# PaullyMac/routest

Measured on AMD Instinct MI355X. Metric: ETA preds/sec (whole node) + p50 /predict latency, 3-layer MLP bf16, higher is better.
Workload: dtype bf16

## Files before the change

csrc/bindings.cpp:

```cpp
#include <torch/extension.h>
#include <ATen/hip/impl/HIPStreamMasqueradingAsCUDA.h>
#include <c10/core/DeviceGuard.h>
#include <hip/hip_runtime.h>

#include <sys/mman.h>

#include <cstring>
#include <mutex>
#include <vector>

#include "ops.h"
#include "common.h"
#include "native_model.h"
#include "route_service.h"

namespace {

#define RT_CHECK_HIP(expr)                                                             \
  do {                                                                                 \
    hipError_t _e = (expr);                                                            \
    TORCH_CHECK(_e == hipSuccess, "HIP error in ", #expr, ": ", hipGetErrorString(_e)); \
  } while (0)

int num_cus(int dev) {
// ... 1342 lines not shown
    c.h_indices = (const int*)tptr("h_indices", false);
    c.h_length = (const float*)tptr("h_length", false);
    c.h_edge_name = (const int32_t*)tptr("h_edge_name", false);
    if (has("names")) c.names = d["names"].cast<std::vector<std::string>>();
    c.N = d["N"].cast<int>();
    c.snap_c = d["snap_c"].cast<double>();
    c.max_path = d["max_path"].cast<int>();
    TORCH_CHECK(c.glat && c.glon && c.h_indptr && c.h_indices && c.h_length && c.N == c.cch->topo().N &&
                    c.max_path > 0,
                "CCH route config incomplete");
  } else if (c.provider == 1) {
    c.glat = (const double*)tptr("glat", false);
    c.glon = (const double*)tptr("glon", false);
    c.h_indptr = (const int*)tptr("h_indptr", false);
    c.h_indices = (const int*)tptr("h_indices", false);
    c.h_cost = (const float*)tptr("h_cost", false);
    c.indptr = (const int*)tptr("indptr", true);
    c.indices = (const int*)tptr("indices", true);
    c.cost = (const float*)tptr("cost", true);
    c.lat32 = (const float*)tptr("lat32", true);
    c.lon32 = (const float*)tptr("lon32", true);
    c.lm = (const float*)tptr("lm", true);
    const torch::Device dev(torch::kCUDA, device);
    ws_from(d.contains("lane_ws") ? py::object(d["lane_ws"]) : py::object(py::none()), c.lane_ws, dev);
    ws_from(d.contains("wave_ws") ? py::object(d["wave_ws"]) : py::object(py::none()), c.wave_ws, dev);
    ws_from(d.contains("big_ws") ? py::object(d["big_ws"]) : py::object(py::none()), c.big_ws, dev);
    if (has("arena")) {
      torch::Tensor ar = d["arena"].cast<torch::Tensor>(), ctr = d["arena_ctr"].cast<torch::Tensor>();
      TORCH_CHECK(ar.is_cuda() && ar.device().index() == device && ar.scalar_type() == torch::kInt64 &&
                      ctr.is_cuda() && ctr.scalar_type() == torch::kInt64, "route config arena");
      c.arena.base = ar.data_ptr();
      c.arena.entries = (unsigned long long)(ar.numel() / 2);
      c.arena.ctr = (unsigned long long*)ctr.data_ptr();
    }
    c.N = d["N"].cast<int>();
    c.K = has("K") ? d["K"].cast<int>() : 0;
    c.snap_c = d["snap_c"].cast<double>();
    c.max_path = d["max_path"].cast<int>();
    c.max_iters = d["max_iters"].cast<int>();
    c.lane_pops = d["lane_pops"].cast<int>();
    if (has("wave_only_below")) c.wave_only_below = d["wave_only_below"].cast<int>();
    c.inv_vmax = d["inv_vmax"].cast<float>();
    c.wave_delta = d["wave_delta"].cast<float>();
    if (has("lane_max_m")) c.lane_max_m = d["lane_max_m"].cast<float>();
    TORCH_CHECK(c.glat && c.glon && c.indptr && c.indices && c.cost && c.lat32 && c.lon32 &&
                    (c.lane_ws.slots > 0 || c.wave_ws.slots > 0) && c.N > 0 && c.max_path > 0,
                "graph route config incomplete");
    TORCH_CHECK(c.lm == nullptr || c.K == 8 || c.K == 16 || c.K == 32, "landmarks K must be 8, 16 or 32");
    TORCH_CHECK((c.lane_ws.slots == 0 || rt::astar_ws_ok(c.lane_ws, false)) &&
                    (c.wave_ws.slots == 0 || rt::astar_ws_ok(c.wave_ws, true)) &&
                    (c.big_ws.slots == 0 || rt::astar_ws_ok(c.big_ws, true)),
                "A* workspace too small");
  }
  return c;
}

static std::vector<float> host_f32(const py::dict& h, const char* k) {
  torch::Tensor t = h[k].cast<torch::Tensor>().to(torch::kCPU).to(torch::kFloat32).contiguous();
  return std::vector<float>(t.data_ptr<float>(), t.data_ptr<float>() + t.numel());
}
static rt::MlpHost mlp_host_from(const py::dict& d) {
  rt::MlpHost m;
  if (!d.contains("host") || d["host"].is_none()) return m;
  py::dict h = d["host"].cast<py::dict>();
  m.w1 = host_f32(h, "w1");
  m.b1 = host_f32(h, "b1");
  m.w2 = host_f32(h, "w2");
  m.b2 = host_f32(h, "b2");
  m.w3 = host_f32(h, "w3");
  m.b3 = h["b3"].cast<float>();
  m.x_mean = host_f32(h, "x_mean");
  m.x_std = host_f32(h, "x_std");
  m.y_mean = h["y_mean"].cast<float>();
  m.y_std = h["y_std"].cast<float>();
  m.H = (int)m.b1.size();
  TORCH_CHECK(m.w1.size() == (size_t)m.H * 12 && m.w2.size() == (size_t)m.H * m.H && m.b2.size() == (size_t)m.H &&
                  m.w3.size() == (size_t)m.H && m.x_mean.size() == 12 && m.x_std.size() == 12,
              "model host weights shapes");
  return m;
}
static rt::NormParams norm_from(const py::dict& d) {
  std::vector<double> norm = d["norm"].cast<std::vector<double>>();
  TORCH_CHECK(norm.size() == 8, "norm must hold 4 scales + 4 shifts");
  rt::NormParams np;
  for (int i = 0; i < 4; ++i) {
    np.scale[i] = (float)norm[i];
    np.shift[i] = (float)norm[4 + i];
  }
  return np;
}
static std::shared_ptr<const rt::NativeModel> model_from(const py::dict& d, int device) {
  const std::string kind = d["kind"].cast<std::string>();
  if (kind == "none") return nullptr;
  std::string err;
  std::shared_ptr<rt::NativeModel> m;
  auto dev_t = [&](const char* k) {
    torch::Tensor t = d[k].cast<torch::Tensor>();
    TORCH_CHECK(t.is_cuda() && t.device().index() == device && t.is_contiguous(), "model tensor ", k,
                " must be contiguous on GPU ", device);
    return t;
  };
  if (kind == "mlp3") {
    const c10::DeviceGuard guard(c10::Device(c10::DeviceType::CUDA, device));
    torch::Tensor blob = dev_t("blob");
    const int H = d["H"].cast<int>();
    TORCH_CHECK(blob.scalar_type() == torch::kUInt8 && (size_t)blob.numel() == rt::eta_mlp3_blob_bytes(H), "mlp3 blob");
    m = rt::make_mlp3_model(device, blob.data_ptr(), (size_t)blob.numel(), H, norm_from(d),
                            d.contains("variant") ? d["variant"].cast<int>() : -1, num_cus(device), mlp_host_from(d),
                            err);
  } else if (kind == "wide") {
    const c10::DeviceGuard guard(c10::Device(c10::DeviceType::CUDA, device));
    torch::Tensor w1q = dev_t("w1q"), w2f = dev_t("w2f"), b2 = dev_t("b2"), w3 = dev_t("w3");
    const int H = d["H"].cast<int>();
    TORCH_CHECK(b2.scalar_type() == torch::kFloat32 && w3.scalar_type() == torch::kFloat32 && b2.numel() == H &&
                    w3.numel() == H, "wide b2/w3 f32 [H]");
    m = rt::make_wide_model(device, H, w1q.data_ptr(), (size_t)w1q.nbytes(), w2f.data_ptr(), (size_t)w2f.nbytes(),
                            b2.data_ptr<float>(), w3.data_ptr<float>(), d["b3"].cast<float>(), norm_from(d),
                            mlp_host_from(d), err);
  } else if (kind == "forest") {
    rt::ForestHost f;
    torch::Tensor v = d["values"].cast<torch::Tensor>().to(torch::kCPU).contiguous();
    torch::Tensor in = d["info"].cast<torch::Tensor>().to(torch::kCPU).contiguous();
    torch::Tensor r = d["roots"].cast<torch::Tensor>().to(torch::kCPU).contiguous();
    TORCH_CHECK(v.scalar_type() == torch::kFloat32 && in.scalar_type() == torch::kInt32 &&
                    r.scalar_type() == torch::kInt32, "forest arrays f32 / int32 / int32");
    f.values.assign(v.data_ptr<float>(), v.data_ptr<float>() + v.numel());
    f.info.assign((const uint32_t*)in.data_ptr<int>(), (const uint32_t*)in.data_ptr<int>() + in.numel());
    f.roots.assign(r.data_ptr<int>(), r.data_ptr<int>() + r.numel());
    f.base = d["base"].cast<float>();
    f.le = d["le"].cast<bool>();
    std::vector<int> fm = d["fmap"].cast<std::vector<int>>();
    TORCH_CHECK(fm.size() == 12, "fmap: 12 entries");
    for (int j = 0; j < 12; ++j) f.fmap[j] = fm[j];
    m = rt::make_forest_model(device, std::move(f), err);
  } else {
    TORCH_CHECK(false, "unknown native model kind ", kind);
  }
  TORCH_CHECK(m != nullptr, "native model: ", err);
  return m;
}

int64_t native_server_start(int64_t port, int64_t threads, std::vector<int64_t> devices, py::list models,
                            int64_t max_batch, std::vector<std::string> cors, bool cors_vercel, bool bind_any,
                            int64_t upstream_port, py::list routes, std::string history_db) {
  TORCH_CHECK(!devices.empty() && models.size() == devices.size(), "one model spec per GPU slot");
  TORCH_CHECK(max_batch >= 1 && max_batch <= (1 << 24), "max_batch out of range");
  TORCH_CHECK(routes.empty() || routes.size() == devices.size(), "one route config per GPU (or none)");
  std::vector<int> devs;
  std::vector<std::shared_ptr<const rt::NativeModel>> ms;
  for (size_t g = 0; g < devices.size(); ++g) {
    devs.push_back((int)devices[g]);
    ms.push_back(model_from(models[g].cast<py::dict>(), (int)devices[g]));
  }
  std::vector<rt::RouteServiceCfg> rcfg;
  for (size_t g = 0; g < routes.size(); ++g) rcfg.push_back(route_cfg_from(routes[g].cast<py::dict>(), devs[g]));
  std::string err;
  const int64_t h = rt::native_server_start((int)port, (int)threads, devs, ms, (int)max_batch, cors, cors_vercel,
                                            bind_any, (int)upstream_port, rcfg, history_db, err);
  TORCH_CHECK(h >= 0, "native server: ", err);
  return h;
}

int64_t native_server_set_models(int64_t h, std::vector<int64_t> devices, py::list models) {
  TORCH_CHECK(models.size() == devices.size(), "one model spec per GPU slot");
  std::vector<std::shared_ptr<const rt::NativeModel>> ms;
  for (size_t g = 0; g < devices.size(); ++g) ms.push_back(model_from(models[g].cast<py::dict>(), (int)devices[g]));
  std::string err;
  int64_t ep;
  {
    py::gil_scoped_release nogil;
    ep = rt::native_server_set_models(h, ms, err);
  }
  TORCH_CHECK(ep >= 0, "native server: ", err);
  return ep;
}

py::dict native_server_health(int64_t h) {
  uint64_t epoch = 0;
  auto rows = rt::native_server_health(h, epoch);
  py::list slots;
  for (auto& r : rows) {
    py::dict d;
    d["device"] = std::stoi(r[0]);
    d["quarantined"] = r[1] == "1";
    d["consecutive_failures"] = std::stoll(r[2]);
    d["failures"] = std::stoll(r[3]);
    d["rounds"] = std::stoll(r[4]);
    d["quarantines"] = std::stoll(r[5]);
    d["fault_injected"] = r[6] == "1";
    d["model"] = r[7];
    d["deadline_timeouts"] = std::stoll(r[8]);
    d["hang_injected"] = r[9] == "1";
    slots.append(d);
  }
  py::dict out;
  out["model_epoch"] = epoch;
  out["slots"] = slots;
  return out;
}

py::bytes comm_unique_id() {
  char id[128];
  TORCH_CHECK(rt::comm_unique_id(id) == 0, "ncclGetUniqueId failed");
  return py::bytes(id, 128);
}

int64_t comm_create(py::bytes uid, int64_t rank, int64_t world, int64_t device, int64_t oneshot_bytes,
                    bool use_rccl) {
  std::string u = uid;
  TORCH_CHECK(!use_rccl || u.size() == 128, "unique id must be 128 bytes");
  u.resize(128);
  std::string err;
  int64_t h;
  {
    py::gil_scoped_release nogil;
    h = rt::comm_create(u.data(), (int)rank, (int)world, (int)device, (size_t)oneshot_bytes, use_rccl, err);
  }
  TORCH_CHECK(h >= 0, "comm_create: ", err);
  return h;
}

py::bytes comm_ipc_handles(int64_t h) {
  std::string out(rt::comm_ipc_handle_bytes(), '\0');
  const int r = rt::comm_ipc_handles(h, out.data());
  TORCH_CHECK(r == 0, "hipIpcGetMemHandle failed (", r, ")");
  return py::bytes(out);
}

void comm_open_peers(int64_t h, std::vector<py::bytes> handles) {
  std::vector<std::string> hs(handles.begin(), handles.end());
  std::string err;
  TORCH_CHECK(rt::comm_open_peers(h, hs, err) == 0, "comm_open_peers: ", err);
}

void comm_all_reduce(int64_t h, torch::Tensor t, int64_t algo) {
  check_dev(t, "all_reduce tensor");
  TORCH_CHECK(t.scalar_type() == torch::kFloat32, "all_reduce: float32 buckets only");
  const c10::DeviceGuard guard(t.device());
  std::string err;
  const hipError_t e = rt::comm_all_reduce_f32(h, t.data_ptr<float>(), (size_t)t.numel(), (int)algo, cur_stream(t), err);
  TORCH_CHECK(e == hipSuccess, "comm_all_reduce: ", err.empty() ? hipGetErrorString(e) : err);
}

void comm_oneshot(int64_t h, int64_t op, torch::Tensor in, torch::Tensor out, int64_t root) {
  check_dev(in, "input");
  check_dev(out, "output");
  TORCH_CHECK(in.is_contiguous() && out.is_contiguous(), "one-shot: contiguous tensors only");
  TORCH_CHECK(in.scalar_type() == out.scalar_type(), "dtype mismatch");
  const c10::DeviceGuard guard(in.device());
  std::string err;
  const size_t bytes = (size_t)in.numel() * in.element_size();
  const int world = rt::comm_world(h);
  TORCH_CHECK(world >= 1, "bad comm handle");
  hipError_t e;
  if (op == 0) {
    TORCH_CHECK(out.numel() == in.numel() * world, "all_gather: out must hold world x input");
    e = rt::comm_all_gather_oneshot(h, in.data_ptr(), out.data_ptr(), bytes, cur_stream(in), err);
  } else {
    TORCH_CHECK(in.data_ptr() == out.data_ptr(), "one-shot broadcast is in place");
    e = rt::comm_broadcast_oneshot(h, in.data_ptr(), bytes, (int)root, cur_stream(in), err);
  }
  TORCH_CHECK(e == hipSuccess, "comm_oneshot: ", err.empty() ? hipGetErrorString(e) : err);
}

int dtype_code(const torch::Tensor& t) {
  if (t.scalar_type() == torch::kFloat32) return 0;
  if (t.scalar_type() == torch::kBFloat16) return 1;
  if (t.scalar_type() == torch::kInt32) return 2;
  TORCH_CHECK(false, "collective dtype must be float32, bfloat16 or int32");
  return -1;
}

void comm_collective(int64_t h, int64_t op, torch::Tensor in, torch::Tensor out, int64_t root) {
  check_dev(in, "input");
  check_dev(out, "output");
  TORCH_CHECK(in.scalar_type() == out.scalar_type(), "dtype mismatch");
  const c10::DeviceGuard guard(in.device());
  std::string err;
  const size_t count = op == 0 ? (size_t)in.numel() : (op == 1 ? (size_t)out.numel() : (size_t)in.numel());
  TORCH_CHECK(rt::comm_nccl_call(h, (int)op, in.data_ptr(), out.data_ptr(), count, dtype_code(in), (int)root,
                                 cur_stream(in), err) == 0, "RCCL collective: ", err);
}

torch::Tensor forest_predict_lds(torch::Tensor records, torch::Tensor nodes2, torch::Tensor roots,
                                 torch::Tensor chunks, double base, bool le, std::vector<int64_t> fmap) {
  for (auto* t : {&records, &nodes2, &roots, &chunks}) check_dev(*t, "forest tensor");
  TORCH_CHECK(records.scalar_type() == torch::kInt32 && records.dim() == 2 && records.size(1) == 4,
              "records must be int32 [B,4]");
  TORCH_CHECK(nodes2.scalar_type() == torch::kInt32 && nodes2.dim() == 2 && nodes2.size(1) == 2, "nodes2 int32 [M,2]");
  TORCH_CHECK(chunks.scalar_type() == torch::kInt32 && chunks.dim() == 2 && chunks.size(1) == 2 &&
              chunks.size(0) >= 2, "chunks int32 [C+1,2]");
  TORCH_CHECK(roots.scalar_type() == torch::kInt32, "roots int32");
  TORCH_CHECK(fmap.size() == 12, "fmap must have 12 entries");
  const c10::DeviceGuard guard(records.device());
  const int B = (int)records.size(0);
  auto out = torch::empty({B}, records.options().dtype(torch::kFloat32));
  int fm[12];
  for (int j = 0; j < 12; ++j) fm[j] = (int)fmap[j];
  RT_CHECK_HIP(rt::launch_forest_lds(records.data_ptr(), nodes2.data_ptr(), roots.data_ptr<int>(),
                                     chunks.data_ptr<int>(), (int)chunks.size(0) - 1, out.data_ptr<float>(), B,
                                     (int)roots.numel(), (int)nodes2.size(0), (float)base, le ? 1 : 0, fm,
                                     num_cus(records.device().index()), cur_stream(records)));
  return out;
}

}

void bind_cch_gpu(py::module& m);

PYBIND11_MODULE(TORCH_EXTENSION_NAME, m) {
  m.doc() = "routest_amd native gfx950 kernels";
  bind_cch_gpu(m);
  m.def("eta_mlp3_forward", &eta_mlp3_forward, "fused featurize + 3-layer MLP forward (bf16 MFMA)");
  m.def("eta_mlp3_forward_hostio", &eta_mlp3_forward_hostio,
        "zero-copy: fused kernel reads records / writes minutes in pinned host memory");
  m.def("pinned_host_empty", &pinned_host_empty, "registered pinned host buffer (optionally THP-backed)",
        py::arg("nbytes"), py::arg("huge") = true);
  m.def("eta_featurize", &eta_featurize,"K1: packed records -> R16 features [B,12] fp32");
  m.def("eta_mlp3_blob_bytes", [](int64_t H) { return (int64_t)rt::eta_mlp3_blob_bytes((int)H); });
  m.def("eta_mlp3_blob16_bytes", [](int64_t H) { return (int64_t)rt::eta_mlp3_blob16_bytes((int)H); });
  m.def("route_haversine_matrix", &route_haversine_matrix, "K5: batched haversine matrices (f64)");
  m.def("route_greedy_cvrp", &route_greedy_cvrp, "K6: batched greedy multi-trip CVRP");
  m.def("route_improve_trips", &route_improve_trips,
        "K6b: intra-trip 2-opt / Or-opt on K6's outputs (visit rewritten in place)");
  m.def("route_tw_trips", &route_tw_trips,
        "K6d: cheapest-insertion trips under time windows and service times for the flagged rows",
        py::arg("D"), py::arg("T"), py::arg("npts"), py::arg("demand"), py::arg("cap"), py::arg("maxd"),
        py::arg("open"), py::arg("close"), py::arg("service"), py::arg("flag"));
  m.def("route_pd_trips", &route_pd_trips,
        "K6f: cheapest insertion of plain stops and pickup -> delivery pairs under time windows for the flagged rows",
        py::arg("D"), py::arg("T"), py::arg("npts"), py::arg("demand"), py::arg("cap"), py::arg("maxd"),
        py::arg("open"), py::arg("close"), py::arg("service"), py::arg("pickup_from"), py::arg("flag"));
  m.def("route_tw_improve", &route_tw_improve,
        "K6e: window-aware relocate / swap on K6d's outputs (rewritten in place); returns stats [R,7]",
        py::arg("D"), py::arg("T"), py::arg("npts"), py::arg("demand"), py::arg("cap"), py::arg("maxd"),
        py::arg("open"), py::arg("close"), py::arg("service"), py::arg("visit"), py::arg("trip_of"),
        py::arg("ntrips"), py::arg("status"), py::arg("arrival"), py::arg("start"), py::arg("flag"));
  m.def("route_pd_improve", &route_pd_improve,
        "K6g: unit relocate on K6f's outputs (rewritten in place); returns stats [R,8]",
        py::arg("D"), py::arg("T"), py::arg("npts"), py::arg("demand"), py::arg("cap"), py::arg("maxd"),
        py::arg("open"), py::arg("close"), py::arg("service"), py::arg("pickup_from"), py::arg("visit"),
        py::arg("trip_of"), py::arg("ntrips"), py::arg("status"), py::arg("arrival"), py::arg("start"),
        py::arg("flag"));
  m.def("route_exchange_trips", &route_exchange_trips,
        "K6c: inter-trip relocate / swap on K6's outputs (visit, trip_of, ntrips rewritten in place)",
        py::arg("D"), py::arg("npts"), py::arg("demand"), py::arg("cap"), py::arg("maxd"), py::arg("visit"),
        py::arg("trip_of"), py::arg("ntrips"), py::arg("status"), py::arg("flag"), py::arg("move_cap") = -1);
  m.def("mm_candidates", &mm_candidates, "K10: map-matching candidates of GPS fixes on the bucket grid",
        py::arg("start"), py::arg("items"), py::arg("nqy"), py::arg("nqx"), py::arg("y0"), py::arg("x0"),
        py::arg("cell"), py::arg("ny"), py::arg("nx"), py::arg("py"), py::arg("px"), py::arg("radius_cm"),
        py::arg("k"));
  m.def("mm_viterbi", &mm_viterbi, "K10: segmenting Viterbi of the map matcher over given costs",
        py::arg("cand_d2"), py::arg("n_cand"), py::arg("route_cm"), py::arg("g"), py::arg("npts"),
        py::arg("beta_cm"), py::arg("sigma_cm"), py::arg("max_detour_cm"));
  m.def("mm_edge_candidates", &mm_edge_candidates, "K10 edge mode: candidates of GPS fixes on the edge grid",
        py::arg("start"), py::arg("items"), py::arg("rec"), py::arg("y0"), py::arg("x0"), py::arg("cell"),
        py::arg("ny"), py::arg("nx"), py::arg("py"), py::arg("px"), py::arg("radius_cm"), py::arg("k"));
  m.def("mm_edge_route_cm", &mm_edge_route_cm, "K10 edge mode: route centimetres between points on edges",
        py::arg("met"), py::arg("e1"), py::arg("off1"), py::arg("lc1"), py::arg("e2"), py::arg("off2"));
  m.def("mm_edge_lds_capacity", []() { return (int64_t)rt::mm_edge_lds_capacity(); },
        "K10 edge mode: survivors of one fix the candidate kernel selects from LDS");
  m.def("big_layer1", &big_layer1, "wide MLP: featurize + layer 1 -> h1 (hperm order)",
        py::arg("records"), py::arg("w1p"), py::arg("H"), py::arg("norm"), py::arg("h1"),
        py::arg("xf") = py::none(), py::arg("mbits") = py::none());
  m.def("big_fused", &big_fused, "wide MLP inference: featurize + layer 1 + layer 2 + relu.w3 partials, one launch");
  m.def("gemm_dgrad_dw1", &gemm_dgrad_dw1, "training dgrad with the dW1 partials in its epilogue (dh1 not stored)");
  m.def("gemm_nt", &gemm_nt, "wide MLP layer GEMM Z^T = W X^T with fused epilogues (0 y-partials, 1 +h2, 2 store)",
        py::arg("epi"), py::arg("W"), py::arg("X"), py::arg("N"), py::arg("M"), py::arg("K"),
        py::arg("b2") = py::none(), py::arg("w3") = py::none(), py::arg("ypart") = py::none(),
        py::arg("out") = py::none());
  m.def("gemm_pipe", [](int64_t set) { return (int64_t)rt::gemm_pipe_mode((int)set); },
        "wide GEMM K loop: 1 phase pipeline, 0 one drain per K-tile; set < 0 only reads", py::arg("set") = -1);
  m.def("big_yreduce", &big_yreduce, "y = sum of partials + b3 (+ dy, dy operand, squared error)",
        py::arg("ypart"), py::arg("nparts"), py::arg("b3"), py::arg("y") = py::none(),
        py::arg("target") = py::none(), py::arg("gscale") = 0.0, py::arg("dy") = py::none(),
        py::arg("dyb") = py::none(), py::arg("sq_err") = py::none(), py::arg("b3_dev") = py::none());
  m.def("adamw_pack_big", &adamw_pack_big, "wide trainer: AdamW + re-pack of w1p / w2k / w2t / b2 / w3 / b3");
  m.def("big_dz2y", &big_dz2y,
        "wide trainer: dy, dyb, squared error, dz2 and the step counter in one launch (+ dW3|db3 slab rows)",
        py::arg("ypart"), py::arg("nparts"), py::arg("b3"), py::arg("target"), py::arg("gscale"), py::arg("dy"),
        py::arg("dyb"), py::arg("sq_err"), py::arg("h2a"), py::arg("w3"), py::arg("H"), py::arg("dz2"),
        py::arg("step_ctr"), py::arg("slab") = py::none());
  m.def("big_dz2", &big_dz2, "dz2 = dy * w3 * relu'(z2) from h2a (hperm order)");
  m.def("eta_mlp3_train_fwd", &eta_mlp3_train_fwd, "K3: fused featurize+MLP forward (one pass over layer 2) + MSE grad + dW3 partial -> dz2 fragments");
  m.def("train_bwd", &train_bwd, "K3: dgrad + relu'(z1) + dW2|db2 and dW1 split-K partials in one kernel (train_bwd_kernel)");
  m.def("train_wgrad_slices", [](int64_t B, int64_t device, int64_t H) {
    return (int64_t)rt::train_wgrad_slices((int)B, num_cus((int)device), (int)H);
  }, py::arg("B"), py::arg("device"), py::arg("H") = 256);
  m.def("adamw_pack", &adamw_pack, "fused AdamW on flat fp32 params + training-blob re-pack");
  m.def("reduce_adamw", &reduce_adamw, "one-rank fused slab reduction + AdamW + blob re-pack");
  m.def("eta_mlp3_train_blob_bytes", [](int64_t H) { return (int64_t)rt::eta_mlp3_train_blob_bytes((int)H); });
  m.def("mlp3_num_params", [](int64_t H) { return (int64_t)rt::mlp3_num_params((int)H); });
  m.def("mlp3_grad_bucket_floats", [](int64_t H) { return (int64_t)rt::mlp3_grad_bucket_floats((int)H); });
  m.def("wgrad", &wgrad, "split-K weight-gradient GEMM (K = batch) into fp32 slabs",
        py::arg("A"), py::arg("M"), py::arg("Mout"), py::arg("Bm"), py::arg("N"), py::arg("slab"),
        py::arg("offset"), py::arg("ldo"), py::arg("mask") = py::none(), py::arg("nout") = -1, py::arg("mask_hperm") = false,
        py::arg("nsplit") = 1);
  m.def("wgrad_dual", &wgrad_dual, "two split-K weight-gradient GEMMs (dW2|db2 and dW1) in one launch");
  m.def("wgrad_reduce", &wgrad_reduce, "deterministic sum of wgrad slabs (optionally a second and third region)",
        py::arg("slab"), py::arg("G"), py::arg("slab1") = py::none(), py::arg("G1") = py::none(),
        py::arg("slab2") = py::none(), py::arg("G2") = py::none(), py::arg("perm_h") = 0, py::arg("fold_ld") = 0,
        py::arg("fold_col") = 0);
  m.def("wgrad256", &wgrad256, "dW2-shaped weight gradient on 256x256 output tiles, split-K over the slab's rows",
        py::arg("A"), py::arg("B"), py::arg("M"), py::arg("N"), py::arg("slab"), py::arg("ldo"), py::arg("db2_col") = -1);
  m.def("train_fwd_grid", [](int64_t B, int64_t dev) { return (int64_t)rt::train_fwd_grid((int)B, num_cus((int)dev)); },
        "workgroups of the training forward = rows of its dW3 slab");
  m.def("num_cus", [](int64_t dev) { return (int64_t)num_cus((int)dev); });
  m.def("gcn_agg_gemm", &gcn_agg_gemm, "K8: fused CSR aggregation + MFMA GEMM + bias/ReLU");
  m.def("gcn_l1_fused", &gcn_l1_fused, "K8: fused aggregation + W1 GEMM + ReLU + W2 transform (H1 stays in LDS)");
  m.def("gcn_spmm_score", &gcn_spmm_score, "K8: layer-2 aggregation + delay head");
  m.def("route_score", &route_score, "K8: per-route delay-weighted length");
  m.def("astar_search", &astar_search, "K9: tiered batched A* (lane -> wave -> big tier) with learned edge costs",
        py::arg("indptr"), py::arg("indices"), py::arg("cost"), py::arg("lat"), py::arg("lon"), py::arg("inv_vmax"),
        py::arg("landmarks"), py::arg("src"), py::arg("dst"), py::arg("lane"), py::arg("wave"), py::arg("big"),
        py::arg("out_cost"), py::arg("out_len"), py::arg("out_status"), py::arg("out_path"), py::arg("out_iters"),
        py::arg("scratch"), py::arg("max_iters"), py::arg("lane_pops"), py::arg("wave_only_below"),
        py::arg("delta"), py::arg("arena") = py::none(), py::arg("arena_ctr") = py::none(),
        py::arg("lane_max_m") = -1.0, py::arg("wave_nw") = 0, py::arg("retry_nw") = 0);
  m.def("forest_predict", &forest_predict, "K4: fused featurize + tree-ensemble inference");
  m.def("forest_predict_lds", &forest_predict_lds, "K4: LDS-staged tree chunks, 2 walks per thread");
  m.def("pscore_create", &pscore_create, "resident single-request scorer kernel on the blob's GPU");
  m.def("pscore_score", &pscore_score, "score n <= cap records on the resident scorer (False: not answered)");
  m.def("pscore_park", [](int64_t h) {
    rt::PersistentScorer* p = ps_get(h);
    py::gil_scoped_release nogil;
    rt::pscore_park(p);
  });
  m.def("pscore_stats", [](int64_t h) {
    long long l, s, f;
    rt::pscore_stats(ps_get(h), &l, &s, &f);
    return std::vector<int64_t>{l, s, f};
  });
  m.def("pscore_destroy", [](int64_t h) {
    rt::PersistentScorer* p = nullptr;
    {
      std::lock_guard<std::mutex> lk(g_ps_mu);
      if (h < 0 || h >= (int64_t)g_ps.size()) return;
      p = g_ps[h];
      g_ps[h] = nullptr;
    }
    py::gil_scoped_release nogil;
    rt::pscore_destroy(p);
  });
  m.def("gcn_train_bwd", &gcn_train_bwd, "GCN scorer backward over a row range -> flat gradient + loss");
  m.def("gcn_grad_numel", []() { return (int64_t)rt::gcn_grad_numel(); });
  m.def("gcn_train_slab2_rows", [](int64_t n) { return (int64_t)rt::gcn_train_slab2_rows((int)n); });
  m.def("native_server_start", &native_server_start, "native HTTP front end (predictions, routes, relay)",
        py::arg("port"), py::arg("threads"), py::arg("devices"), py::arg("models"), py::arg("max_batch"),
        py::arg("cors"), py::arg("cors_vercel"), py::arg("bind_any"), py::arg("upstream_port") = 0,
        py::arg("routes") = py::list(), py::arg("history_db") = "");
  m.def("native_server_set_models", &native_server_set_models,
        "hot-swap the served models (one spec per GPU slot); returns the new epoch");
  m.def("native_server_set_fault", [](int64_t h, int64_t slot, bool on) {
    return rt::native_server_set_fault(h, (int)slot, on);
  });
  m.def("native_server_set_hang", [](int64_t h, int64_t slot, bool on) {
    return rt::native_server_set_hang(h, (int)slot, on);
  }, "latency-watchdog fault hook: launches on the slot first wait on a host flag");
  m.def("native_server_set_scorer", [](int64_t h, std::vector<double> delay, int64_t kind, std::string engine) {
    return rt::native_server_set_scorer(h, std::move(delay), (int)kind, engine);
  }, "publish the GCN scorer's node delays for native \"alternatives\" requests");
  m.def("native_server_health", &native_server_health, "per-GPU-slot health, models and the model epoch");
  m.def("native_server_stop", [](int64_t h) {
    py::gil_scoped_release nogil;
    rt::native_server_stop(h);
  });
  m.def("native_server_stats", [](int64_t h) {
    const auto v = rt::native_server_stats(h);
    return std::vector<int64_t>(v.begin(), v.end());
  });
  m.def("comm_unique_id", &comm_unique_id, "RCCL unique id (128 bytes) for comm_create");
  m.def("comm_create", &comm_create, "own RCCL communicator + one-shot IPC buffers");
  m.def("comm_ipc_handles", &comm_ipc_handles, "IPC handles of this rank's one-shot buffers");
  m.def("comm_open_peers", &comm_open_peers, "map every peer's one-shot buffers (xGMI)");
  m.def("comm_all_reduce", &comm_all_reduce, "in-place SUM all-reduce on the current stream (0=rccl, 1=oneshot)");
  m.def("comm_collective", &comm_collective, "RCCL all_gather(0)/reduce_scatter(1)/broadcast(2)/all_reduce(3)");
  m.def("comm_oneshot", &comm_oneshot, "one-shot IPC all_gather(0)/broadcast(2) on the current stream");
  m.def("comm_error", [](int64_t h) { return (int64_t)rt::comm_error(h); });
  m.def("comm_destroy", [](int64_t h) { rt::comm_destroy(h); });
  m.def("rccl_version", []() { return (int64_t)rt::comm_rccl_version(); });
  m.attr("ARCH") = "gfx950";
}
```

csrc/native_model.h:

```cpp
#pragma once
#include <hip/hip_runtime.h>

#include <cstdint>
#include <memory>
#include <string>
#include <vector>

#include "common.h"
#include "runtime/rt_core.h"

namespace rt {

struct ModelWs {
  void* p = nullptr;
  size_t bytes = 0;
  int device = -1;
  ~ModelWs();
  hipError_t need(int dev, size_t b);
};

struct NativeModel {
  enum Kind { MLP3 = 0, WIDE = 1, FOREST = 2 };
  int kind = MLP3;
  int device = 0;
  int H = 0;
  uint64_t epoch = 0;
  virtual ~NativeModel() = default;
  virtual hipError_t predict(const void* rec, int rec_bytes, float* out, int B, hipStream_t s, ModelWs& ws) const = 0;
  virtual bool takes_wire8() const { return true; }
  virtual const void* mlp3_blob() const { return nullptr; }
  virtual const NormParams* mlp3_norm() const { return nullptr; }
  virtual bool cpu_predict(const rtc::EtaRecord* rec, float* out, int B) const = 0;
  virtual std::string describe() const = 0;
};

struct MlpHost {
  int H = 0;
  std::vector<float> w1, b1, w2, b2, w3, x_mean, x_std;
  float b3 = 0.f, y_mean = 0.f, y_std = 1.f;
};

struct ForestHost {
  std::vector<float> values;
  std::vector<uint32_t> info;
  std::vector<int32_t> roots;
  float base = 0.f;
  bool le = false;
  int fmap[12] = {0, 1, 2, 3, 4, 5, 6, 7, 8, 9, 10, 11};
};

std::shared_ptr<NativeModel> make_mlp3_model(int device, const void* blob, size_t blob_bytes, int H,
                                             const NormParams& np, int variant, int num_cus, MlpHost host,
                                             std::string& err);
std::shared_ptr<NativeModel> make_wide_model(int device, int H, const void* w1q, size_t w1q_bytes, const void* w2f,
                                             size_t w2f_bytes, const float* b2, const float* w3, float b3,
                                             const NormParams& np, MlpHost host, std::string& err);
std::shared_ptr<NativeModel> make_forest_model(int device, ForestHost host, std::string& err);

float mlp_cpu_forward(const MlpHost& m, const rtc::EtaRecord& r);

}
```

csrc/native_model.hip:

```cpp
#include <cmath>
#include <cstring>

#include "native_model.h"
#include "ops.h"

namespace rt {

ModelWs::~ModelWs() {
  if (p) {
    int cur = 0;
    (void)hipGetDevice(&cur);
    (void)hipSetDevice(device);
    (void)hipFree(p);
    (void)hipSetDevice(cur);
  }
}

hipError_t ModelWs::need(int dev, size_t b) {
  if (p && device == dev && bytes >= b) return hipSuccess;
  if (p) {
    int cur = 0;
    (void)hipGetDevice(&cur);
    (void)hipSetDevice(device);
    (void)hipFree(p);
    (void)hipSetDevice(cur);
    p = nullptr;
  }
  bytes = 0;
  device = dev;
  const size_t m = b < 4096 ? 4096 : b;
  hipError_t e = hipMalloc(&p, m);
  if (e == hipSuccess) bytes = m;
  return e;
}

namespace {

struct DevOwned {
  void* p = nullptr;
  int device = 0;
  DevOwned() = default;
  DevOwned(const DevOwned&) = delete;
  ~DevOwned() {
    if (p) {
      int cur = 0;
      (void)hipGetDevice(&cur);
      (void)hipSetDevice(device);
      (void)hipFree(p);
      (void)hipSetDevice(cur);
    }
  }
  hipError_t copy_from(int dev, const void* src, size_t bytes, hipMemcpyKind kind) {
    device = dev;
    int cur = 0;
    (void)hipGetDevice(&cur);
    (void)hipSetDevice(dev);
    hipError_t e = hipMalloc(&p, bytes ? bytes : 4);
    if (e == hipSuccess && bytes) e = hipMemcpy(p, src, bytes, kind);
    (void)hipSetDevice(cur);
    return e;
  }
};

inline void featurize(const rtc::EtaRecord& r, float x[12]) {
  for (int i = 0; i < 8; ++i) x[i] = 0.f;
  if (r.weather < 4) x[r.weather] = 1.f;
  if (r.traffic < 4) x[4 + r.traffic] = 1.f;
  const int64_t secs = r.wallclock_s;
  const int64_t days = secs >= 0 ? secs / 86400 : -((-secs + 86399) / 86400);
  const int64_t sod = secs - days * 86400;
  x[8] = (float)(((days + 2) % 7 + 7) % 7);
  x[9] = (float)(sod / 3600);
  x[10] = r.distance_m / 1000.0f;
  x[11] = r.driver_age;
}

bool mlp_cpu_batch(const MlpHost& m, const rtc::EtaRecord* rec, float* out, int B) {
  if (m.H <= 0) return false;
  for (int i = 0; i < B; ++i) out[i] = mlp_cpu_forward(m, rec[i]);
  return true;
}

struct Mlp3Model : NativeModel {
  DevOwned blob;
  NormParams np{};
  int variant = -1, cus = 256;
  MlpHost host;
  hipError_t predict(const void* rec, int rec_bytes, float* out, int B, hipStream_t s, ModelWs&) const override {
    return launch_eta_mlp3_fwd(rec, out, B, blob.p, H, np, variant, cus, s, rec_bytes);
  }
  const void* mlp3_blob() const override { return blob.p; }
  const NormParams* mlp3_norm() const override { return &np; }
  bool cpu_predict(const rtc::EtaRecord* rec, float* out, int B) const override { return mlp_cpu_batch(host, rec, out, B); }
  std::string describe() const override { return "mlp3 H=" + std::to_string(H); }
};

struct WideModel : NativeModel {
  DevOwned w1q, w2f, b2, w3;
  float b3 = 0.f;
  NormParams np{};
  MlpHost host;
  hipError_t predict(const void* rec, int rec_bytes, float* out, int B, hipStream_t s, ModelWs& ws) const override {
    const int parts = H / 64;
    hipError_t e = ws.need(device, (size_t)B * parts * sizeof(float));
    if (e != hipSuccess) return e;
    float* yp = (float*)ws.p;
    e = launch_big_fused(rec, rec_bytes, B, w1q.p, w2f.p, H, np, (const float*)b2.p, (const float*)w3.p, yp, s);
    if (e != hipSuccess) return e;
    return launch_big_yreduce(yp, parts, B, b3, nullptr, out, nullptr, 0.f, nullptr, nullptr, nullptr, s);
  }
  bool cpu_predict(const rtc::EtaRecord* rec, float* out, int B) const override { return mlp_cpu_batch(host, rec, out, B); }
  std::string describe() const override { return "mlp3-wide H=" + std::to_string(H); }
};

struct ForestModelN : NativeModel {
  DevOwned values, info, roots;
  ForestHost host;
  int fm[12];
  hipError_t predict(const void* rec, int rec_bytes, float* out, int B, hipStream_t s, ModelWs&) const override {
    if (rec_bytes != 16) return hipErrorInvalidValue;
    return launch_forest(rec, (const float*)values.p, (const unsigned*)info.p, (const int*)roots.p, out, B,
                         (int)host.roots.size(), (int)host.values.size(), host.base, host.le ? 1 : 0, fm, s);
  }
  bool takes_wire8() const override { return false; }
  bool cpu_predict(const rtc::EtaRecord* rec, float* out, int B) const override {
    const int T = (int)host.roots.size();
    for (int i = 0; i < B; ++i) {
      float x[12], xm[12];
      featurize(rec[i], x);
      for (int j = 0; j < 12; ++j) xm[j] = x[host.fmap[j]];
      double acc = host.base;
      for (int t = 0; t < T; ++t) {
        const int root = host.roots[t];
        int n = root;
        while (!(host.info[n] >> 31)) {
          const uint32_t inf = host.info[n];
          const float v = xm[(inf >> 24) & 63];
          const float thr = host.values[n];
          const bool left = std::isnan(v) ? ((inf >> 30) & 1) != 0 : (host.le ? v <= thr : v < thr);
          n = root + (int)(inf & 0xFFFFFF) + (left ? 0 : 1);
        }
        acc += host.values[n];
      }
      out[i] = (float)acc;
    }
    return true;
  }
  std::string describe() const override { return "forest trees=" + std::to_string(host.roots.size()); }
};

}

float mlp_cpu_forward(const MlpHost& m, const rtc::EtaRecord& r) {
  float x[12];
  featurize(r, x);
  for (int j = 0; j < 12; ++j) x[j] = (x[j] - m.x_mean[j]) / m.x_std[j];
  const int H = m.H;
  std::vector<float> h1(H), h2(H);
  for (int u = 0; u < H; ++u) {
    float a = m.b1[u];
    const float* w = m.w1.data() + (size_t)u * 12;
    for (int j = 0; j < 12; ++j) a += w[j] * x[j];
    h1[u] = a > 0.f ? a : 0.f;
  }
  for (int u = 0; u < H; ++u) {
    float a = m.b2[u];
    const float* w = m.w2.data() + (size_t)u * H;
    for (int j = 0; j < H; ++j) a += w[j] * h1[j];
    h2[u] = a > 0.f ? a : 0.f;
  }
  float y = m.b3;
  for (int j = 0; j < H; ++j) y += m.w3[j] * h2[j];
  return y * m.y_std + m.y_mean;
}

std::shared_ptr<NativeModel> make_mlp3_model(int device, const void* blob, size_t blob_bytes, int H,
                                             const NormParams& np, int variant, int num_cus, MlpHost host,
                                             std::string& err) {
  auto m = std::make_shared<Mlp3Model>();
  m->kind = NativeModel::MLP3;
  m->device = device;
  m->H = H;
  m->np = np;
  m->variant = variant;
  m->cus = num_cus;
  m->host = std::move(host);
  if (m->blob.copy_from(device, blob, blob_bytes, hipMemcpyDeviceToDevice) != hipSuccess) {
    err = "mlp3 blob copy failed";
    return nullptr;
  }
  return m;
}

std::shared_ptr<NativeModel> make_wide_model(int device, int H, const void* w1q, size_t w1q_bytes, const void* w2f,
                                             size_t w2f_bytes, const float* b2, const float* w3, float b3,
                                             const NormParams& np, MlpHost host, std::string& err) {
  if (H != 512 && H != 1024) {
    err = "wide model: H must be 512 or 1024";
    return nullptr;
  }
  auto m = std::make_shared<WideModel>();
  m->kind = NativeModel::WIDE;
  m->device = device;
  m->H = H;
  m->np = np;
  m->b3 = b3;
  m->host = std::move(host);
  if (m->w1q.copy_from(device, w1q, w1q_bytes, hipMemcpyDeviceToDevice) != hipSuccess ||
      m->w2f.copy_from(device, w2f, w2f_bytes, hipMemcpyDeviceToDevice) != hipSuccess ||
      m->b2.copy_from(device, b2, (size_t)H * 4, hipMemcpyDeviceToDevice) != hipSuccess ||
      m->w3.copy_from(device, w3, (size_t)H * 4, hipMemcpyDeviceToDevice) != hipSuccess) {
    err = "wide model weight copy failed";
    return nullptr;
  }
  return m;
}

constexpr int FOREST_MAX_DEPTH = 64;

std::shared_ptr<NativeModel> make_forest_model(int device, ForestHost host, std::string& err) {
  const size_t M = host.values.size();
  if (M == 0 || host.info.size() != M || host.roots.empty() || host.roots[0] != 0) {
    err = "forest: malformed arrays";
    return nullptr;
  }
  for (size_t i = 1; i < host.roots.size(); ++i)
    if (host.roots[i] <= host.roots[i - 1] || (size_t)host.roots[i] >= M) {
      err = "forest: roots not increasing";
      return nullptr;
    }
  for (size_t t = 0; t < host.roots.size(); ++t) {
    const size_t b = (size_t)host.roots[t], e = t + 1 < host.roots.size() ? (size_t)host.roots[t + 1] : M;
    for (size_t n = b; n < e; ++n) {
      const uint32_t inf = host.info[n];
      if (inf >> 31) continue;
      if (((inf >> 24) & 63) >= 12 || b + (inf & 0xFFFFFF) + 1 >= e) {
        err = "forest: node reference out of range";
        return nullptr;
      }
    }
  }
  {
    std::vector<int> seen(M, -1);
    std::vector<uint32_t> cur, nxt;
    for (size_t t = 0; t < host.roots.size(); ++t) {
      const uint32_t b = (uint32_t)host.roots[t];
      cur.assign(1, b);
      for (int level = 0; !cur.empty(); ++level) {
        nxt.clear();
        for (uint32_t n : cur) {
          const uint32_t inf = host.info[n];
          if (inf >> 31) continue;
          if (level == FOREST_MAX_DEPTH) {
            err = "forest: tree " + std::to_string(t) + " is deeper than the kernels' depth limit of " +
                  std::to_string(FOREST_MAX_DEPTH) + " inner nodes on a root-to-leaf path";
            return nullptr;
          }
          for (uint32_t c = b + (inf & 0xFFFFFF), e = c + 2; c < e; ++c)
            if (seen[c] != level) {
              seen[c] = level;
              nxt.push_back(c);
            }
        }
        cur.swap(nxt);
      }
    }
  }
  for (int j = 0; j < 12; ++j)
    if (host.fmap[j] < 0 || host.fmap[j] >= 12) {
      err = "forest: feature map out of range";
      return nullptr;
    }
  auto m = std::make_shared<ForestModelN>();
  m->kind = NativeModel::FOREST;
  m->device = device;
  m->H = 0;
  for (int j = 0; j < 12; ++j) m->fm[j] = host.fmap[j];
  if (m->values.copy_from(device, host.values.data(), M * 4, hipMemcpyHostToDevice) != hipSuccess ||
      m->info.copy_from(device, host.info.data(), M * 4, hipMemcpyHostToDevice) != hipSuccess ||
      m->roots.copy_from(device, host.roots.data(), host.roots.size() * 4, hipMemcpyHostToDevice) != hipSuccess) {
    err = "forest copy failed";
    return nullptr;
  }
  m->host = std::move(host);
  return m;
}

}
```

csrc/native_server.hip:

```cpp
#include <arpa/inet.h>
#include <errno.h>
#include <fcntl.h>
#include <netinet/in.h>
#include <netinet/tcp.h>
#include <sys/epoll.h>
#include <sys/eventfd.h>
#include <sys/socket.h>
#include <sys/time.h>
#include <time.h>
#include <unistd.h>

#include <atomic>
#include <cstdlib>
#include <cstring>
#include <memory>
#include <mutex>
#include <shared_mutex>
#include <string>
#include <thread>
#include <unordered_map>
#include <vector>

#include "common.h"
#include "native_model.h"
// ... 1197 lines not shown
    }
    c.out.clear();
    c.out_off = 0;
    epoll_event e{};
    e.events = EPOLLIN;
    e.data.fd = c.fd;
    epoll_ctl(ep_, EPOLL_CTL_MOD, c.fd, &e);
    if (c.close_after && !c.async) to_close_.push_back(c.fd);
  }
};

struct Server {
  ServerCfg cfg;
  Stats stats;
  Shared sh;
  std::atomic<bool> stop{false};
  std::vector<std::unique_ptr<Reactor>> reactors;
  std::vector<std::thread> threads;
  std::vector<std::unique_ptr<RouteService>> routes;
  std::shared_mutex routes_mu;
  bool routes_open = false;
  std::shared_ptr<AltScorerState> alt = std::make_shared<AltScorerState>();
  ~Server() {
    if (sh.hang_release) *(volatile int*)sh.hang_release = 1;
    {
      std::unique_lock<std::shared_mutex> lk(routes_mu);
      routes_open = false;
    }
    routes.clear();
    for (PersistentScorer* p : sh.scorers)
      if (p) pscore_destroy(p);
    if (sh.hang_release) (void)hipHostFree(sh.hang_release);
  }
};

void stop_scorer(Server* s, int g) {
  Shared& sh = s->sh;
  if (sh.scorers[g] != nullptr) pscore_destroy(sh.scorers[g]);
  sh.scorers[g] = nullptr;
  sh.scorer_models[g] = nullptr;
}

void restart_scorer(Server* s, int g) {
  Shared& sh = s->sh;
  stop_scorer(s, g);
  if (!(s->cfg.persist_idle_ms > 0 && s->cfg.persist_cap > 0)) return;
  auto m = sh.model(g);
  if (m == nullptr || m->mlp3_blob() == nullptr) return;
  hipError_t e = hipSuccess;
  sh.scorers[g] = pscore_create(sh.devices[g], m->mlp3_blob(), m->H, *m->mlp3_norm(), s->cfg.persist_cap,
                                s->cfg.persist_idle_ms, s->cfg.persist_life_ms, &e);
  if (sh.scorers[g] != nullptr) sh.scorer_models[g] = m;
}

std::mutex g_srv_mu;
std::vector<Server*> g_servers;

}

int64_t native_server_start(int port, int threads, const std::vector<int>& devices,
                            const std::vector<std::shared_ptr<const NativeModel>>& models, int max_batch,
                            const std::vector<std::string>& cors, bool cors_vercel, bool bind_any, int upstream_port,
                            const std::vector<RouteServiceCfg>& routes, const std::string& history_db,
                            std::string& err) {
  if (devices.empty() || devices.size() != models.size() || (!routes.empty() && routes.size() != devices.size())) {
    err = "devices/models/routes mismatch";
    return -1;
  }
  auto* s = new Server();
  s->cfg.port = port;
  s->cfg.threads = threads < 1 ? 1 : threads;
  s->cfg.max_batch = max_batch;
  s->cfg.cors_exact = cors;
  s->cfg.cors_vercel = cors_vercel;
  s->cfg.upstream_port = upstream_port;
  s->cfg.sh = &s->sh;
  s->cfg.history_db = history_db;
  if (const char* v = std::getenv("ROUTEST_PERSIST_IDLE_MS")) s->cfg.persist_idle_ms = std::atof(v);
  if (const char* v = std::getenv("ROUTEST_PERSIST_CAP")) s->cfg.persist_cap = std::atoi(v);
  if (const char* v = std::getenv("ROUTEST_PERSIST_LIFE_MS")) s->cfg.persist_life_ms = std::atof(v);
  Shared& sh = s->sh;
  if (const char* v = std::getenv("ROUTEST_QUARANTINE_AFTER")) sh.quarantine_after = std::max(1, std::atoi(v));
  if (const char* v = std::getenv("ROUTEST_QUARANTINE_PROBE_MS")) sh.probe_ms = std::max(1ll, std::atoll(v));
  if (const char* v = std::getenv("ROUTEST_FRONT_CACHE_MS")) sh.rc_ttl_ms = std::max(0ll, std::atoll(v));
  sh.devices = devices;
  sh.models = models;
  sh.epoch = 1;
  for (size_t g = 0; g < devices.size(); ++g) {
    sh.health.push_back(std::make_unique<SlotHealth>());
    sh.scorers.push_back(nullptr);
    sh.scorer_models.push_back(nullptr);
    sh.scorer_mus.push_back(std::make_unique<std::mutex>());
  }
  if (const char* v = std::getenv("ROUTEST_GPU_DEADLINE_MS")) sh.deadline_ms = std::atof(v);
  if (const char* v = std::getenv("ROUTEST_ROUTE_TRACE_MS")) sh.trace_ms = std::atof(v);
  if (hipHostMalloc((void**)&sh.hang_release, sizeof(int), hipHostMallocMapped | hipHostMallocPortable) == hipSuccess) {
    *(volatile int*)sh.hang_release = 1;
    if (hipHostGetDevicePointer((void**)&sh.hang_release_d, sh.hang_release, 0) != hipSuccess) sh.hang_release_d = nullptr;
  } else {
    sh.hang_release = nullptr;
  }
  if (const char* v = std::getenv("ROUTEST_FAULT")) {
    std::string f = v;
    size_t b = 0;
    while (b <= f.size()) {
      size_t e = f.find(',', b);
      if (e == std::string::npos) e = f.size();
      std::string t = f.substr(b, e - b);
      while (!t.empty() && t.front() == ' ') t.erase(t.begin());
      while (!t.empty() && t.back() == ' ') t.pop_back();
      if (t == "gpu_fail") {
        for (auto& h : sh.health) h->fault = true;
      } else if (t.rfind("gpu_fail@", 0) == 0) {
        const int g = std::atoi(t.c_str() + 9);
        if (g >= 0 && g < (int)sh.health.size()) sh.health[g]->fault = true;
      } else if (t.rfind("gpu_hang@", 0) == 0 && sh.hang_release_d) {
        const int g = std::atoi(t.c_str() + 9);
        if (g >= 0 && g < (int)sh.health.size()) {
          sh.health[g]->hang = true;
          *(volatile int*)sh.hang_release = 0;
        }
      }
      b = e + 1;
    }
  }
  for (size_t g = 0; g < devices.size(); ++g) {
    std::lock_guard<std::mutex> lk(*sh.scorer_mus[g]);
    restart_scorer(s, (int)g);
  }
  if (!routes.empty() && routes[0].provider == 1 && routes[0].h_length != nullptr && routes[0].glat != nullptr) {
    auto rg = std::make_shared<rrec::RecordGraph>();
    const RouteServiceCfg& r0 = routes[0];
    rg->own_names = r0.names;
    rg->build(r0.N, r0.glat, r0.glon, r0.h_indptr, r0.h_indices, r0.h_length, r0.h_edge_name, &rg->own_names);
    if (rg->ok()) s->cfg.record_graph = rg;
  }
  for (int i = 0; i < s->cfg.threads; ++i) {
    ServerCfg rc = s->cfg;
    const size_t g = (size_t)i % devices.size();
    rc.device = devices[g];
    rc.slot = (int)g;
    auto r = std::make_unique<Reactor>(rc, s->stats, s->stop);
    r->set_bind_any(bind_any);
    if (!r->init(err)) {
      delete s;
      return -1;
    }
    s->reactors.push_back(std::move(r));
  }
  s->routes.reserve(routes.size());
  for (size_t g = 0; g < routes.size(); ++g) {
    RouteServiceCfg rc = routes[g];
    rc.record_graph = s->cfg.record_graph;
    Shared* shp = &s->sh;
    const int slot = (int)g;
    rc.eta_model = [shp, slot]() { return shp->model(slot); };
    rc.park_scorer = [shp, slot]() { shp->park(slot); };
    rc.alt = s->alt;
    rc.on_timeout = [shp, slot]() { shp->timed_out(slot); };
    rc.slot = slot;
    rc.failover = [s, slot](RouteJob* j) {
      std::shared_lock<std::shared_mutex> lk(s->routes_mu);
      if (!s->routes_open) return false;
      const int n = (int)s->routes.size();
      if (j->hops >= n - 1) return false;
      for (int k = 1; k < n; ++k) {
        RouteService* r = s->routes[(size_t)((slot + k) % n)].get();
        if (r != nullptr && !r->broken()) {
          ++j->hops;
          if (r->submit(j)) return true;
          --j->hops;
        }
      }
      return false;
    };
    rc.hang_fault = [shp, slot]() { return shp->health[slot]->hang.load(std::memory_order_relaxed); };
    rc.hang_release_d = shp->hang_release_d;
    s->routes.push_back(std::make_unique<RouteService>(rc, [](RouteJob* j) {
      static_cast<JobTag*>(j->tag)->reactor->job_done(j);
    }));
    s->routes.back()->set_done_batch([](std::vector<RouteJob*>& js) {
      std::vector<std::pair<Reactor*, std::vector<RouteJob*>>> by;
      for (RouteJob* j : js) {
        Reactor* r = static_cast<JobTag*>(j->tag)->reactor;
        auto it = std::find_if(by.begin(), by.end(), [r](const auto& p) { return p.first == r; });
        if (it == by.end()) by.push_back({r, {j}});
        else it->second.push_back(j);
      }
      for (auto& [r, v] : by) r->jobs_done(v);
    });
  }
  {
    std::unique_lock<std::shared_mutex> lk(s->routes_mu);
    s->routes_open = true;
  }
  if (!s->routes.empty())
    for (int i = 0; i < s->cfg.threads; ++i) s->reactors[i]->set_routes(s->routes[(size_t)i % devices.size()].get());
  for (auto& r : s->reactors) s->threads.emplace_back([rp = r.get()]() { rp->run(); });
  std::lock_guard<std::mutex> lk(g_srv_mu);
  g_servers.push_back(s);
  return (int64_t)g_servers.size() - 1;
}

int64_t native_server_set_models(int64_t h, const std::vector<std::shared_ptr<const NativeModel>>& models,
                                 std::string& err) {
  std::lock_guard<std::mutex> lk(g_srv_mu);
  if (h < 0 || h >= (int64_t)g_servers.size() || !g_servers[h]) {
    err = "no such server";
    return -1;
  }
  Server* s = g_servers[h];
  if (models.size() != s->sh.devices.size()) {
    err = "one model per GPU slot";
    return -1;
  }
  for (size_t g = 0; g < models.size(); ++g) {
    std::lock_guard<std::mutex> sl(*s->sh.scorer_mus[g]);
    stop_scorer(s, (int)g);
  }
  uint64_t ep;
  {
    std::lock_guard<std::mutex> ml(s->sh.model_mu);
    s->sh.models = models;
    ep = s->sh.epoch.fetch_add(1) + 1;
  }
  for (size_t g = 0; g < models.size(); ++g) {
    std::lock_guard<std::mutex> sl(*s->sh.scorer_mus[g]);
    restart_scorer(s, (int)g);
  }
  return (int64_t)ep;
}

bool native_server_set_fault(int64_t h, int slot, bool on) {
  std::lock_guard<std::mutex> lk(g_srv_mu);
  if (h < 0 || h >= (int64_t)g_servers.size() || !g_servers[h]) return false;
  Server* s = g_servers[h];
  if (slot < 0 || slot >= (int)s->sh.health.size()) return false;
  s->sh.health[slot]->fault = on;
  return true;
}

bool native_server_set_hang(int64_t h, int slot, bool on) {
  std::lock_guard<std::mutex> lk(g_srv_mu);
  if (h < 0 || h >= (int64_t)g_servers.size() || !g_servers[h]) return false;
  Server* s = g_servers[h];
  if (slot < 0 || slot >= (int)s->sh.health.size() || !s->sh.hang_release) return false;
  s->sh.health[slot]->hang = on;
  bool any = false;
  for (auto& x : s->sh.health) any |= x->hang.load();
  *(volatile int*)s->sh.hang_release = any ? 0 : 1;
  return true;
}

bool native_server_set_scorer(int64_t h, std::vector<double> delay, int kind, const std::string& engine) {
  std::lock_guard<std::mutex> lk(g_srv_mu);
  if (h < 0 || h >= (int64_t)g_servers.size() || !g_servers[h]) return false;
  Server* s = g_servers[h];
  std::lock_guard<std::mutex> lk2(s->alt->mu);
  s->alt->delay = delay.empty() ? nullptr : std::make_shared<const std::vector<double>>(std::move(delay));
  s->alt->kind = kind;
  s->alt->engine = engine;
  return true;
}

std::vector<std::vector<std::string>> native_server_health(int64_t h, uint64_t& epoch) {
  std::vector<std::vector<std::string>> out;
  std::lock_guard<std::mutex> lk(g_srv_mu);
  if (h < 0 || h >= (int64_t)g_servers.size() || !g_servers[h]) return out;
  Server* s = g_servers[h];
  epoch = s->sh.epoch.load();
  auto models = s->sh.snapshot();
  for (size_t g = 0; g < s->sh.devices.size(); ++g) {
    const SlotHealth& x = *s->sh.health[g];
    out.push_back({std::to_string(s->sh.devices[g]), x.quarantined.load() ? "1" : "0", std::to_string(x.consec.load()),
                   std::to_string(x.failures.load()), std::to_string(x.rounds.load()),
                   std::to_string(x.quarantines.load()), x.fault.load() ? "1" : "0",
                   models[g] ? models[g]->describe() : std::string("none"), std::to_string(x.timeouts.load()),
                   x.hang.load() ? "1" : "0"});
  }
  return out;
}

void native_server_stop(int64_t h) {
  Server* s = nullptr;
  {
    std::lock_guard<std::mutex> lk(g_srv_mu);
    if (h < 0 || h >= (int64_t)g_servers.size()) return;
    s = g_servers[h];
    g_servers[h] = nullptr;
  }
  if (!s) return;
  if (s->sh.hang_release) *(volatile int*)s->sh.hang_release = 1;
  s->stop.store(true);
  for (auto& r : s->reactors) {
    uint64_t one = 1;
    (void)!write(r->wake_fd(), &one, 8);
  }
  for (auto& t : s->threads) t.join();
  delete s;
}

std::vector<long long> native_server_stats(int64_t h) {
  std::lock_guard<std::mutex> lk(g_srv_mu);
  if (h < 0 || h >= (int64_t)g_servers.size() || !g_servers[h]) return std::vector<long long>(41, 0);
  Server* s = g_servers[h];
  std::vector<long long> v = {s->stats.requests.load(), s->stats.predictions.load(), s->stats.launches.load(),
                              s->stats.errors.load(), s->stats.resident.load(), s->stats.fallbacks.load(),
                              s->stats.wire8.load(), s->stats.route_requests.load(),
                              s->stats.route_fallbacks.load(), s->stats.relayed.load()};
  std::vector<long long> rs(18, 0);
  for (auto& r : s->routes) {
    const auto x = r->stats();
    for (size_t i = 0; i < rs.size() && i < x.size(); ++i) rs[i] += x[i];
  }
  v.insert(v.end(), rs.begin(), rs.end());
  v.push_back(s->stats.failovers.load());
  v.push_back(s->stats.cpu_rounds.load());
  v.push_back(s->stats.history.load());
  v.push_back(s->stats.cached.load());
  std::vector<long long> rx(4, 0);
  for (auto& r : s->routes) {
    const auto x = r->stats();
    for (size_t i = 0; i < rx.size() && 18 + i < x.size(); ++i) rx[i] += x[18 + i];
  }
  v.insert(v.end(), rx.begin(), rx.end());
  v.push_back(s->stats.timeouts.load());
  std::vector<long long> rr(4, 0);
  for (auto& r : s->routes) {
    const auto x = r->stats();
    for (size_t i = 0; i < rr.size() && 22 + i < x.size(); ++i) rr[i] += x[22 + i];
  }
  v.insert(v.end(), rr.begin(), rr.end());
  return v;
}

}
```

csrc/route_service.h:

```cpp
#pragma once
#include <cmath>
#include <functional>
#include <memory>
#include <string>
#include <vector>

#include "cch_gpu.h"
#include "common.h"
#include "native_model.h"
#include "ops.h"
#include "runtime/route_core.h"
#include "runtime/route_record.h"
#include "runtime/route_store.h"

#include <mutex>

namespace rt {

struct PersistentScorer;
struct RouteJob;

inline hipError_t isolated_stream(int device, hipStream_t* s) {
  int cus = 0;
  if (hipDeviceGetAttribute(&cus, hipDeviceAttributeMultiprocessorCount, device) != hipSuccess || cus <= 0) cus = 256;
  std::vector<uint32_t> mask((size_t)(cus + 31) / 32, 0xFFFFFFFFu);
  return hipExtStreamCreateWithCUMask(s, (uint32_t)mask.size(), mask.data());
}

struct AltScorerState {
  std::mutex mu;
  std::shared_ptr<const std::vector<double>> delay;
  int kind = 0;
  std::string engine = "gcn-hip";
  std::shared_ptr<const std::vector<double>> get(int& k, std::string& e) {
    std::lock_guard<std::mutex> lk(mu);
    k = kind;
    e = engine;
    return delay;
  }
};

struct RouteServiceCfg {
  int device = 0;
  int provider = 0;
  CchGpu* cch = nullptr;
  bool cch_contexts = true;
  uint64_t cch_fixed_key = 0;
  const float* h_length = nullptr;
  const int32_t* h_edge_name = nullptr;
  std::vector<std::string> names;
  double circuity = 1.3, step_m = 150.0;
  std::string engine = "backend:mi355x";
  bool compat200 = true;
  int batch_max = 1024;
  double timeout_us = 500.0;
  int chunk_threads = 16;
  const double* glat = nullptr;
  const double* glon = nullptr;
  int N = 0;
  double snap_c = 1.0;
  const int* h_indptr = nullptr;
  const int* h_indices = nullptr;
  const float* h_cost = nullptr;
  const int* indptr = nullptr;
  const int* indices = nullptr;
  const float* cost = nullptr;
  const float* lat32 = nullptr;
  const float* lon32 = nullptr;
  const float* lm = nullptr;
  int K = 0;
  AstarWs lane_ws, wave_ws, big_ws;
  AstarArenaBuf arena;
  int max_path = 4096, max_iters = 2000000, lane_pops = 500;
  int wave_only_below = 32768;
  float inv_vmax = 0.f, wave_delta = 10.f, lane_max_m = -1.f;
  std::function<std::shared_ptr<const NativeModel>()> eta_model;
  std::string sqlite_path;
  std::function<void()> park_scorer;
  std::shared_ptr<AltScorerState> alt;
  std::function<bool(RouteJob*)> failover;
  std::shared_ptr<const rrec::RecordGraph> record_graph;
  std::function<void()> on_timeout;
  int slot = -1;
  std::function<bool()> hang_fault;
  const int* hang_release_d = nullptr;
};

struct RouteJob {
  std::string body;
  bool json_ok = true;
  bool request_route = false;
  void* tag = nullptr;
  bool fallback = false;
  int status = 0;
  std::string out;
  rtj::Value root;
  rtr::RouteReq req;
  rtr::Plan plan;
  std::vector<std::vector<std::pair<double, double>>> calls;
  std::vector<int32_t> nodes;
  int group = 0;
  bool parsed = false;
  double defer_t0 = 0.0;
  bool sync_ctx = false;
  int hops = 0;
  double t_enq_us = 0.0;
  std::vector<std::pair<int, int>> alt_pairs;
  std::vector<std::vector<int>> alt_vias;
  std::vector<rtr::Leg> alt_legs;
  std::vector<std::vector<int32_t>> alt_paths, alt_edges;
  std::string alt_json;
  rts::StoreRow row;
  rtc::Stamp now;
};

class RouteService {
 public:
  RouteService(const RouteServiceCfg& cfg, std::function<void(RouteJob*)> done);
  ~RouteService();
  bool submit(RouteJob* j);
  void set_done_batch(std::function<void(std::vector<RouteJob*>&)> done_many);
  std::vector<long long> stats() const;
  bool broken() const;

 private:
  struct Impl;
  Impl* p_;
};

}
```

csrc/route_service.hip:

```cpp
#include <fcntl.h>
#include <unistd.h>

#include <algorithm>
#include <cstdlib>
#include <cstring>

#include "route_service_impl.h"

namespace rt {

namespace {

__global__ __launch_bounds__(64) void route_hang_kernel(const int* release, long long max_ticks) {
  const long long t0 = wall_clock64();
  for (int it = 0; it < 2000000 && __hip_atomic_load(release, __ATOMIC_RELAXED, __HIP_MEMORY_SCOPE_SYSTEM) == 0 &&
                   wall_clock64() - t0 < max_ticks;
       ++it)
    __builtin_amdgcn_s_sleep(127);
}

}

hipError_t RouteService::Impl::sync(hipStream_t s, hipEvent_t ev, const char* what) {
  hipError_t e = hipEventRecord(ev, s);
  if (e != hipSuccess) return e;
  const auto t0 = std::chrono::steady_clock::now();
  auto waited = [&] { return std::chrono::duration<double, std::milli>(std::chrono::steady_clock::now() - t0).count(); };
  for (int i = 0;; ++i) {
    e = hipEventQuery(ev);
    if (e != hipErrorNotReady) {
      if (trace_ms >= 0 && waited() > trace_ms) trace("wait %s %.1f ms", what, waited());
      return e;
    }
    const double dl = flush_deadline_ms.load(std::memory_order_relaxed);
    if (dl > 0 && (i & 15) == 15 && waited() > dl) {
      trace("DEADLINE in %s after %.1f ms", what, waited());
      if (!broken.exchange(true) && cfg.on_timeout) cfg.on_timeout();
      return hipErrorLaunchTimeOut;
    }
    if (i > 4096) std::this_thread::sleep_for(std::chrono::microseconds(20));
  }
}

void RouteService::Impl::hand_off(std::vector<RouteJob*>& jobs) {
  for (RouteJob* j : jobs) {
    if (!j->fallback && !j->status && cfg.failover) {
      j->plan = rtr::Plan();
      j->calls.clear();
      j->nodes.clear();
      j->group = 0;
      j->alt_pairs.clear();
      j->alt_vias.clear();
      j->alt_legs.clear();
      j->alt_paths.clear();
      j->alt_edges.clear();
      j->alt_json.clear();
      j->row.asmb = rtr::Assembled();
      if (cfg.failover(j)) {
        n_failed_over.fetch_add(1, std::memory_order_relaxed);
        continue;
      }
      trace("no other route service takes the job (hops %d): relayed to the app", j->hops);
    }
    if (!j->status) j->fallback = true;
    finish(j);
    done(j);
  }
  jobs.clear();
}

void RouteService::Impl::run() {
  if (hipSetDevice(cfg.device) != hipSuccess) return;
  int least = 0, greatest = 0;
  if (hipDeviceGetStreamPriorityRange(&least, &greatest) != hipSuccess ||
      hipStreamCreateWithPriority(&stream, hipStreamNonBlocking, greatest) != hipSuccess) {
    (void)hipGetLastError();
    if (hipStreamCreateWithFlags(&stream, hipStreamNonBlocking) != hipSuccess) return;
  }
  if (const char* v = std::getenv("ROUTEST_CCH_ASYNC")) async_ctx = std::string(v) != "0";
  if (const char* v = std::getenv("ROUTEST_ROUTE_DEADLINE_MS")) deadline_ms = std::atof(v);
  flush_deadline_ms.store(deadline_ms);
  if (const char* v = std::getenv("ROUTEST_ROUTE_TRACE_MS")) trace_ms = std::atof(v);
  if (const char* v = std::getenv("ROUTEST_FAULT")) fail_fault = std::string(v).find("route_fail") != std::string::npos;
  if (hipEventCreateWithFlags(&ev_gpu, hipEventDisableTiming) != hipSuccess) ev_gpu = nullptr;
  if (const char* v = std::getenv("ROUTEST_CCH_PREFETCH_MIN")) prefetch_min = std::atoi(v);
  if (const char* v = std::getenv("ROUTEST_ROUTE_CLOCK_SKEW_S")) clock_skew_s = std::atoll(v);
  if (cfg.cch != nullptr && cfg.cch_contexts && async_ctx) {
    listener = cfg.cch->add_build_listener([this](uint64_t key, bool ok) { on_built(key, ok); });
    cfg.cch->start_builders();
  }
  if (std::getenv("ROUTEST_ROUTE_PREWARM") == nullptr || std::string(std::getenv("ROUTEST_ROUTE_PREWARM")) != "0")
    prewarm();
  if (const char* v = std::getenv("ROUTEST_HANG_ARM"))
    if (std::string(v) == "1" && isolated_stream(cfg.device, &hang_stream) != hipSuccess) hang_stream = nullptr;
  th_asm = std::thread([this] { asm_loop(); });
  while (true) {
    auto* b = new Batch();
    {
      std::unique_lock<std::mutex> lk(mu);
      cv.wait(lk, [&] { return stop || !q.empty(); });
      if (stop && q.empty()) { delete b; break; }
      const double t_wake = now_us();
      static const bool from_wake = [] {
        const char* v = std::getenv("ROUTEST_ROUTE_COLLECT");
        return v && std::string(v) == "wake";
      }();
      const double t_open = from_wake ? t_wake : q.front()->t_enq_us;
      const auto deadline = std::chrono::steady_clock::time_point(std::chrono::duration_cast<std::chrono::steady_clock::duration>(
          std::chrono::duration<double, std::micro>(t_open + cfg.timeout_us)));
      while ((int)q.size() < cfg.batch_max && !stop && std::chrono::steady_clock::now() < deadline) {
        if (cv.wait_until(lk, deadline) == std::cv_status::timeout) break;
      }
      t_collect_us.fetch_add((long long)(now_us() - t_wake), std::memory_order_relaxed);
      const size_t take = std::min<size_t>(q.size(), (size_t)cfg.batch_max);
      b->jobs.assign(q.begin(), q.begin() + take);
      q.erase(q.begin(), q.begin() + take);
    }
    if (broken.load()) {
      if (drained()) {
        trace("drained: serving again");
        broken.store(false);
      } else {
        trace("broken: handing %zu jobs off", b->jobs.size());
        hand_off(b->jobs);
        delete b;
        continue;
      }
    }
    hipStream_t main_stream = stream;
    if (cfg.hang_fault && cfg.hang_release_d && cfg.hang_fault()) {
      if (!hang_stream && isolated_stream(cfg.device, &hang_stream) != hipSuccess) hang_stream = nullptr;
      if (hang_stream) {
        stream = hang_stream;
        hipLaunchKernelGGL(route_hang_kernel, dim3(1), dim3(64), 0, stream, cfg.hang_release_d, 500000000ll);
      }
    }
    gpu_stage(*b);
    stream = main_stream;
    if (fail_fault && !b->jobs.empty()) b->failed = true;
    if (b->failed) {
      trace("flush of %zu jobs failed: handing off", b->jobs.size());
      hand_off(b->jobs);
      delete b;
      continue;
    }
    if (b->jobs.empty()) {
      delete b;
      continue;
    }
    const double t_h = now_us();
    std::unique_lock<std::mutex> lk(amu);
    acv.wait(lk, [&] { return aq.size() < 2; });
    t_handoff_us.fetch_add((long long)(now_us() - t_h), std::memory_order_relaxed);
    aq.push_back(b);
    acv.notify_all();
  }
  if (listener) cfg.cch->remove_build_listener(listener);
  std::vector<RouteJob*> left;
  {
    std::lock_guard<std::mutex> lk(wmu);
    for (auto& kv : waiting) left.insert(left.end(), kv.second.begin(), kv.second.end());
    waiting.clear();
  }
  {
    std::lock_guard<std::mutex> lk(mu);
    left.insert(left.end(), q.begin(), q.end());
    q.clear();
  }
  for (RouteJob* j : left) {
    j->fallback = true;
    finish(j);
    done(j);
  }
  {
    std::lock_guard<std::mutex> lk(amu);
    gpu_done = true;
  }
  acv.notify_all();
  th_asm.join();
  (void)hipStreamDestroy(stream);
  if (ev_gpu) (void)hipEventDestroy(ev_gpu);
}

void RouteService::Impl::asm_loop() {
  if (hipSetDevice(cfg.device) != hipSuccess) return;
  if (hipStreamCreateWithFlags(&stream_asm, hipStreamNonBlocking) != hipSuccess) return;
  if (hipEventCreateWithFlags(&ev_asm, hipEventDisableTiming) != hipSuccess) ev_asm = nullptr;
  store.open(cfg.sqlite_path);
  th_persist = std::thread([this] { persist_loop(); });
  while (true) {
    Batch* b = nullptr;
    {
      std::unique_lock<std::mutex> lk(amu);
      acv.wait(lk, [&] { return gpu_done || !aq.empty(); });
      if (aq.empty()) break;
      b = aq.front();
      aq.pop_front();
      acv.notify_all();
    }
    asm_stage(*b);
    n_flushes.fetch_add(1, std::memory_order_relaxed);
    std::vector<RouteJob*> save = std::move(b->save);
    std::vector<RouteJob*> now_done;
    {
      const std::unordered_set<RouteJob*> saving(save.begin(), save.end());
      for (RouteJob* j : b->jobs)
        if (!saving.count(j)) {
          finish(j);
          now_done.push_back(j);
        }
    }
    done_all(now_done);
    delete b;
    if (!save.empty()) {
      std::unique_lock<std::mutex> lk(pmu);
      pcv.wait(lk, [&] { return pq.size() < 8; });
      pq.push_back(std::move(save));
      pcv.notify_all();
    }
  }
  {
    std::lock_guard<std::mutex> lk(pmu);
    asm_done = true;
  }
  pcv.notify_all();
  th_persist.join();
  (void)hipStreamDestroy(stream_asm);
  if (ev_asm) (void)hipEventDestroy(ev_asm);
}

void RouteService::Impl::prewarm() {
  const size_t R = (size_t)std::max(1, cfg.batch_max), NM = 11, RN = R * NM, Q = RN;
  const size_t MP = (size_t)std::max(1, cfg.max_path);
  bool ok = tb.reserve(R, NM, false) && lb.reserve(Q, Q, MP, cfg.cch != nullptr) && lb.reserve_flat(Q * 256) &&
            eb.reserve(R);
  if (cfg.cch != nullptr) {
    ok = ok && tb.reserve(R, NM, true) && lb.reserve_flat_e(Q * 256) && cb.reserve(R) &&
         cb.h_hcost.need((size_t)cfg.cch->topo().E) == hipSuccess;
    const int S = cfg.cch->stride();
    msc.device = cfg.device;
    ok = ok && msc.ensure(RN * 2, std::max(Q, (RN * NM * 2 + CchGpu::MAX_ARCS - 1) / CchGpu::MAX_ARCS + 1), S,
                              CchGpu::MAX_ARCS) == hipSuccess;
  }
  if (!ok) (void)hipGetLastError();
}

void RouteService::Impl::on_built(uint64_t key, bool ok) {
  std::vector<RouteJob*> js;
  {
    std::lock_guard<std::mutex> lk(wmu);
    auto it = waiting.find(key);
    if (it == waiting.end()) return;
    js.swap(it->second);
    waiting.erase(it);
  }
  if (!ok)
    for (RouteJob* j : js) j->sync_ctx = true;
  {
    std::lock_guard<std::mutex> lk(mu);
    for (auto it = js.rbegin(); it != js.rend(); ++it) q.push_front(*it);
  }
  cv.notify_one();
}

void RouteService::Impl::assemble_all(Batch& b) {
  std::vector<RouteJob*>& jobs = b.jobs;
  const std::vector<rtr::Leg>& legs = b.legs;
  const std::unordered_map<uint64_t, int>& leg_index = b.leg_index;
  rtc::parallel_chunks(jobs.size(), 8, chunk_threads(), [&](size_t lo, size_t hi) {
    for (size_t i = lo; i < hi; ++i) {
      RouteJob* j = jobs[i];
      if (j->fallback || j->status) continue;
      if (j->req.alt_k > 0) choose_alternatives(b, j);
      std::vector<rtr::Dir> dirs(j->calls.size());
      std::string perr;
      size_t off = 0;
      bool want_rec = rg != nullptr && store.opened() && !j->request_route && j->req.alt_k == 0 &&
                      cfg.provider == 1 && !j->calls.empty();
      rrec::Writer rw;
      std::vector<uint64_t> durs;
      std::vector<uint32_t> per_leg;
      j->row.rec.clear();
      for (size_t k = 0; k < j->calls.size() && perr.empty(); ++k) {
        if (cfg.provider == 0) {
          rtr::haversine_directions(j->calls[k], j->req.profile, cfg.circuity, cfg.step_m, dirs[k]);
        } else {
          std::vector<const rtr::Leg*> lp;
          for (size_t t = 0; t + 1 < j->calls[k].size(); ++t) {
            const int s0 = j->nodes[off + t], s1 = j->nodes[off + t + 1];
            if (j->req.alt_k > 0) {
              size_t a = 0;
              while (j->alt_pairs[a].first != s0 || j->alt_pairs[a].second != s1) ++a;
              lp.push_back(&j->alt_legs[a]);
              continue;
            }
            const uint64_t key = cfg.cch ? leg_key(j->group, s0, s1)
                                         : (((uint64_t)(uint32_t)s0 << 32) | (uint32_t)s1);
            lp.push_back(&legs[leg_index.at(key)]);
          }
          rtr::GraphHost gh;
          const rtr::GraphHost* ghp = nullptr;
          if (cfg.cch && cfg.h_length != nullptr) {
            gh.indptr = cfg.h_indptr;
            gh.indices = cfg.h_indices;
            gh.length = cfg.h_length;
            gh.cost = b.host_cost[j->group]->data();
            gh.edge_name = cfg.h_edge_name;
            gh.names = &cfg.names;
            gh.edge_heading = headings();
            ghp = &gh;
          }
          if (k == 0 && want_rec) rrec::begin(rw, *rg, ghp != nullptr, j->req.profile, j->calls.size());
          durs.clear();
          per_leg.clear();
          rtr::StepDurs sd;
          sd.out = &durs;
          sd.per_leg = &per_leg;
          perr = rtr::graph_directions(j->calls[k], j->nodes.data() + off, lp, j->req.profile, cfg.glat, cfg.glon,
                                       dirs[k], ghp, want_rec && ghp ? &sd : nullptr);
          off += j->calls[k].size();
          if (want_rec && perr.empty())
            want_rec = !sd.bad && rrec::add_call(rw, *rg, ghp, j->calls[k], lp, durs, per_leg);
        }
      }
      if (!perr.empty()) j->req.error = perr;
      if (want_rec && perr.empty()) {
        j->row.rec = std::move(rw.b);
        n_records.fetch_add(1, std::memory_order_relaxed);
        n_record_bytes.fetch_add((long long)j->row.rec.size(), std::memory_order_relaxed);
      }
      if (!rtr::assemble(j->req, j->plan, dirs, cfg.engine, j->row.asmb, ccache()))
        j->fallback = true;
      else if (j->req.alt_k > 0 && j->row.asmb.ok) j->row.asmb.body += j->alt_json;
    }
  });
}

bool RouteService::Impl::run_eta(std::vector<RouteJob*>& jobs) {
  std::vector<RouteJob*> m;
  for (RouteJob* j : jobs)
    if (!j->fallback && !j->status && j->row.asmb.ok && j->req.use_ml_eta && j->req.eta_ok) m.push_back(j);
  if (m.empty()) return true;
  std::shared_ptr<const NativeModel> model = cfg.eta_model ? cfg.eta_model() : nullptr;
  if (model == nullptr) {
    for (RouteJob* j : m) j->fallback = true;
    return true;
  }
  const int n = (int)m.size();
  if (!eb.reserve((size_t)n)) return false;
  const rtc::Stamp now = local_now();
  for (int k = 0; k < n; ++k) {
    RouteJob* j = m[k];
    j->now = now;
    rtc::EtaRecord& r = eb.h_rec.h[k];
    r.distance_m = (float)j->row.asmb.dist;
    r.driver_age = (float)j->req.eta_age;
    r.wallclock_s = (int32_t)(now.secs - rtc::EPOCH2020_DAYS * 86400);
    r.weather = j->req.eta_weather;
    r.traffic = j->req.eta_traffic;
    r.pad = 0;
  }
  hipError_t e = qcopy(eb.d_rec.d, eb.h_rec.h, (size_t)n * 16, stream_asm);
  if (e == hipSuccess) e = model->predict(eb.d_rec.d, 16, eb.d_eta.d, n, stream_asm, eta_ws);
  if (e == hipSuccess) e = qcopy(eb.h_eta.h, eb.d_eta.d, (size_t)n * 4, stream_asm);
  if (e == hipSuccess) e = sync(stream_asm, ev_asm, "eta");
  std::vector<float> cpu_eta;
  const float* eta = eb.h_eta.h;
  if (e != hipSuccess) {
    cpu_eta.resize((size_t)n);
    std::vector<rtc::EtaRecord> rec(eb.h_rec.h, eb.h_rec.h + n);
    if (!model->cpu_predict(rec.data(), cpu_eta.data(), n)) return false;
    eta = cpu_eta.data();
  }
  for (int k = 0; k < n; ++k) {
    RouteJob* j = m[k];
    const double mins = (double)eta[k];
    if (!std::isfinite(mins) || std::fabs(mins) > 1.4e9) continue;
    std::string tmp;
    rtc::format_one(tmp, mins, now.secs, now.us, false, 0, "");
    const size_t a = tmp.find("\"eta_completion_time_ml\":\"");
    if (a == std::string::npos) continue;
    const size_t b0 = a + 26;
    j->row.eta_iso = tmp.substr(b0, tmp.size() - 2 - b0);
    j->row.eta_min = eta[k];
  }
  return true;
}

void RouteService::Impl::parse_job(RouteJob* j) {
  if (j->parsed) return;
  j->parsed = true;
  bool parsed = false;
  if (j->json_ok && !j->body.empty()) {
    try {
      j->root = rtj::Parser(j->body.data(), j->body.size()).parse();
      parsed = true;
    } catch (const std::exception&) {
    }
  }
  if (j->request_route && (!j->json_ok || (!parsed && !j->body.empty()))) {
    j->fallback = true;
    return;
  }
  static const rtj::Value empty = [] { rtj::Value v; v.kind = rtj::Value::Obj; return v; }();
  const rtj::Value* rootp = parsed ? &j->root : (j->request_route ? nullptr : &empty);
  if (!j->request_route && parsed && j->root.kind != rtj::Value::Obj) rootp = &empty;
  j->req = rtr::parse_route_request(rootp);
  if (j->req.fallback) j->fallback = true;
}

void RouteService::Impl::gpu_stage(Batch& b) {
  std::vector<RouteJob*>& jobs = b.jobs;
  long long fresh_jobs = 0;
  for (RouteJob* j : jobs) fresh_jobs += !j->parsed;
  n_jobs.fetch_add(fresh_jobs, std::memory_order_relaxed);
  double t0 = now_us();
  rtc::parallel_chunks(jobs.size(), 32, chunk_threads(), [&](size_t lo, size_t hi) {
    for (size_t i = lo; i < hi; ++i) parse_job(jobs[i]);
  });
  bool any_alt = false;
  for (RouteJob* j : jobs) any_alt |= !j->fallback && j->req.alt_k > 0;
  if (any_alt) {
    if (cfg.alt && cfg.provider == 1 && cfg.cch != nullptr) b.alt_delay = cfg.alt->get(b.alt_kind, b.alt_engine);
    const bool ok = b.alt_delay != nullptr && (int)b.alt_delay->size() == cfg.N;
    for (RouteJob* j : jobs)
      if (!j->fallback && j->req.alt_k > 0 && (!ok || !j->req.error.empty())) j->fallback = !ok || j->fallback;
  }
  add_t(0, t0);
  {
    double pairs = 0.0;
    bool sync_build = false;
    for (RouteJob* j : jobs) {
      if (j->fallback) continue;
      const double n = (double)j->req.dst.size() + 1.0;
      pairs += n * n;
      sync_build |= j->sync_ctx;
    }
    flush_deadline_ms.store(deadline_ms <= 0 ? deadline_ms
                                             : deadline_ms * (1.0 + pairs / 2.0e6) + (sync_build ? 30000.0 : 0.0));
  }
  if (cfg.park_scorer) cfg.park_scorer();
  t0 = now_us();
  if (cfg.provider == 1 && cfg.cch != nullptr) {
    if (!cch_groups(b) || !plan_multi_road(b)) {
      b.failed = true;
      return;
    }
    add_t(1, t0);
    for (RouteJob* j : jobs)
      if (!j->fallback) rtr::directions_calls(j->req, j->plan, j->calls);
    if (!search_legs_cch(b)) b.failed = true;
    return;
  }
  if (!plan_multi(jobs)) { b.failed = true; return; }
  add_t(1, t0);
  for (RouteJob* j : jobs)
    if (!j->fallback) rtr::directions_calls(j->req, j->plan, j->calls);
  if (cfg.provider == 1 && !search_legs(b)) b.failed = true;
}

void RouteService::Impl::asm_stage(Batch& b) {
  std::vector<RouteJob*>& jobs = b.jobs;
  if (b.failed) return;
  double t0 = now_us();
  assemble_all(b);
  add_t(5, t0);
  t0 = now_us();
  if (!run_eta(jobs)) {
    for (RouteJob* j : jobs) j->row.eta_iso.clear();
  }
  add_t(6, t0);
  for (RouteJob* j : jobs)
    if (store.opened() && !j->fallback && !j->status && j->row.asmb.ok && !j->request_route) b.save.push_back(j);
  t0 = now_us();
  rtc::parallel_chunks(b.save.size(), 16, chunk_threads(), [&](size_t lo, size_t hi) {
    for (size_t i = lo; i < hi; ++i) {
      b.save[i]->row.root = b.save[i]->req.root;
      rts::RouteStore::prepare(b.save[i]->row);
    }
  });
  add_t(7, t0);
}

void RouteService::Impl::finish(RouteJob* j) {
  if (j->fallback) { n_fallback.fetch_add(1, std::memory_order_relaxed); return; }
  if (j->status) return;
  if (!j->row.asmb.ok) {
    j->status = (j->request_route && cfg.compat200) ? 200 : 400;
    j->out = rtr::error_body(j->row.asmb.error.empty() ? j->req.error : j->row.asmb.error);
    return;
  }
  j->status = 200;
  j->out = std::move(j->row.asmb.body);
  if (!j->row.eta_iso.empty()) {
    j->out += ",\"eta_minutes_ml\":";
    rtr::put_float(j->out, (double)j->row.eta_min);
    j->out += ",\"eta_completion_time_ml\":";
    rtr::put_str(j->out, j->row.eta_iso);
  }
  if (!j->row.request_id.empty()) {
    j->out += ",\"request_id\":";
    rtr::put_str(j->out, j->row.request_id);
    j->out += ",\"saved\":true";
  }
  j->out += "}}";
}

void RouteService::Impl::persist_loop() {
  while (true) {
    std::vector<std::vector<RouteJob*>> groups;
    {
      std::unique_lock<std::mutex> lk(pmu);
      pcv.wait(lk, [&] { return asm_done || !pq.empty(); });
      if (pq.empty()) break;
      groups.assign(std::make_move_iterator(pq.begin()), std::make_move_iterator(pq.end()));
      pq.clear();
      pcv.notify_all();
    }
    std::vector<RouteJob*> fin;
    std::vector<rts::StoreRow*> rows;
    for (auto& g : groups)
      for (RouteJob* j : g) {
        fin.push_back(j);
        rows.push_back(&j->row);
      }
    const double t0 = now_us();
    store.commit_group(rows);
    add_t(7, t0);
    for (RouteJob* j : fin) finish(j);
    done_all(fin);
  }
}

RouteService::RouteService(const RouteServiceCfg& cfg, std::function<void(RouteJob*)> done) : p_(new Impl) {
  p_->cfg = cfg;
  p_->done = std::move(done);
  if (cfg.provider == 1 && cfg.glat != nullptr) {
    p_->grid.build(cfg.glat, cfg.glon, (size_t)cfg.N, cfg.snap_c);
    const auto& shared = cfg.record_graph;
    if (shared && shared->ok() && shared->N == cfg.N && shared->glat == cfg.glat && shared->indptr == cfg.h_indptr &&
        shared->length == cfg.h_length) {
      p_->rg = shared;
    } else {
      p_->coord_cache.build(cfg.glat, cfg.glon, (size_t)cfg.N);
      if (cfg.h_indptr != nullptr && cfg.h_indices != nullptr) {
        const int64_t E = cfg.h_indptr[cfg.N];
        p_->edge_heading.resize((size_t)E);
        for (int u = 0; u < cfg.N; ++u)
          for (int32_t e = cfg.h_indptr[u]; e < cfg.h_indptr[u + 1]; ++e)
            p_->edge_heading[(size_t)e] = rtr::hop_heading(cfg.glat, cfg.glon, u, cfg.h_indices[e]);
      }
      if (cfg.h_length != nullptr && cfg.h_indptr != nullptr && cfg.h_indices != nullptr) {
        auto g = std::make_shared<rrec::RecordGraph>();
        const Impl* ip = p_;
        g->build(cfg.N, cfg.glat, cfg.glon, cfg.h_indptr, cfg.h_indices, cfg.h_length, cfg.h_edge_name,
                 &ip->cfg.names, &ip->coord_cache, ip->edge_heading.empty() ? nullptr : ip->edge_heading.data());
        if (g->ok()) p_->rg = g;
      }
    }
  }
  p_->th = std::thread([this] { p_->run(); });
}

RouteService::~RouteService() {
  {
    std::lock_guard<std::mutex> lk(p_->mu);
    p_->stop = true;
  }
  p_->cv.notify_all();
  if (p_->th.joinable()) p_->th.join();
  delete p_;
}

void RouteService::set_done_batch(std::function<void(std::vector<RouteJob*>&)> done_many) {
  p_->done_many = std::move(done_many);
}

bool RouteService::submit(RouteJob* j) {
  if (!j->parsed) {
    p_->n_jobs.fetch_add(1, std::memory_order_relaxed);
    Impl::parse_job(j);
  }
  if (j->req.avoid || j->req.time_windows) return false;
  {
    std::lock_guard<std::mutex> lk(p_->mu);
    if (p_->stop) return false;
    j->t_enq_us = now_us();
    p_->q.push_back(j);
  }
  p_->cv.notify_one();
  return true;
}

std::vector<long long> RouteService::stats() const {
  std::vector<long long> v = {p_->n_jobs.load(), p_->n_flushes.load(), p_->n_fallback.load(), p_->n_legs.load(),
                              p_->n_host_legs.load(), p_->store.rows_persisted()};
  for (int k = 0; k < 8; ++k) v.push_back(p_->t_stage[k].load());
  v.push_back(p_->n_escalated.load());
  v.push_back(p_->n_ctx_built.load());
  v.push_back(p_->t_ctx_us.load());
  v.push_back(p_->n_legs_reused.load());
  v.push_back(p_->n_deferred.load());
  v.push_back(p_->t_wait_us.load());
  v.push_back(p_->n_prefetch.load());
  v.push_back(p_->n_failed_over.load());
  v.push_back(p_->n_records.load());
  v.push_back(p_->n_record_bytes.load());
  v.push_back(p_->t_collect_us.load());
  v.push_back(p_->t_handoff_us.load());
  return v;
}

bool RouteService::broken() const { return p_->broken.load();
}

}
```

csrc/route_service_bufs.h:

```cpp
#pragma once
#include <algorithm>
#include <atomic>
#include <cstdint>
#include <vector>

#include "common.h"

namespace rt {

static __global__ __launch_bounds__(256) void route_copy_kernel(unsigned char* __restrict__ dst,
                                                                const unsigned char* __restrict__ src, size_t bytes) {
  const size_t nv = (((uintptr_t)dst | (uintptr_t)src) & 15) == 0 ? bytes / 16 : 0;
  const size_t stride = (size_t)gridDim.x * blockDim.x;
  for (size_t i = (size_t)blockIdx.x * blockDim.x + threadIdx.x; i < nv; i += stride)
    reinterpret_cast<int4*>(dst)[i] = reinterpret_cast<const int4*>(src)[i];
  for (size_t i = nv * 16 + (size_t)blockIdx.x * blockDim.x + threadIdx.x; i < bytes; i += stride) dst[i] = src[i];
}
static __global__ __launch_bounds__(256) void route_copy2d_kernel(unsigned char* __restrict__ dst, size_t dpitch,
                                                                  const unsigned char* __restrict__ src, size_t spitch,
                                                                  size_t width, size_t height) {
  const size_t stride = (size_t)gridDim.x * blockDim.x;
  for (size_t i = (size_t)blockIdx.x * blockDim.x + threadIdx.x; i < width * height; i += stride) {
    const size_t r = i / width, c = i - r * width;
    dst[r * dpitch + c] = src[r * spitch + c];
  }
}
inline std::atomic<bool>& qcopy_same_va() {
  static std::atomic<bool> ok{true};
  return ok;
}
inline hipError_t qcopy(void* dst, const void* src, size_t bytes, hipStream_t s) {
  if (bytes == 0) return hipSuccess;
  if (!qcopy_same_va().load(std::memory_order_relaxed)) return hipMemcpyAsync(dst, src, bytes, hipMemcpyDefault, s);
  const size_t blocks = std::min<size_t>(1024, (bytes / 16 + 255) / 256 + 1);
  hipLaunchKernelGGL(route_copy_kernel, dim3((unsigned)blocks), dim3(256), 0, s, (unsigned char*)dst,
                     (const unsigned char*)src, bytes);
  return hipGetLastError();
}
inline hipError_t qcopy2d(void* dst, size_t dpitch, const void* src, size_t spitch, size_t width, size_t height,
                          hipStream_t s) {
  if (width == 0 || height == 0) return hipSuccess;
  if (!qcopy_same_va().load(std::memory_order_relaxed))
    return hipMemcpy2DAsync(dst, dpitch, src, spitch, width, height, hipMemcpyDefault, s);
  const size_t blocks = std::min<size_t>(1024, (width * height + 255) / 256);
  hipLaunchKernelGGL(route_copy2d_kernel, dim3((unsigned)blocks), dim3(256), 0, s, (unsigned char*)dst, dpitch,
                     (const unsigned char*)src, spitch, width, height);
  return hipGetLastError();
}

template <class T>
struct DevBuf {
  T* d = nullptr;
  size_t n = 0;
  std::vector<T*> old;
  hipError_t need(size_t k) {
    if (k <= n) return hipSuccess;
    const size_t m = std::max(k, n * 3 / 2);
    if (d) old.push_back(d);
    d = nullptr;
    n = 0;
    hipError_t e = hipMalloc((void**)&d, m * sizeof(T));
    if (e == hipSuccess) n = m;
    return e;
  }
  ~DevBuf() {
    if (d) (void)hipFree(d);
    for (T* p : old) (void)hipFree(p);
  }
};
template <class T>
struct HostBuf {
  T* h = nullptr;
  size_t n = 0;
  std::vector<T*> old;
  hipError_t need(size_t k) {
    if (k <= n) return hipSuccess;
    const size_t m = std::max(k, n * 3 / 2);
    if (h) old.push_back(h);
    h = nullptr;
    n = 0;
    hipError_t e = hipHostMalloc((void**)&h, m * sizeof(T), hipHostMallocMapped | hipHostMallocPortable);
    if (e == hipSuccess) {
      n = m;
      void* dp = nullptr;
      if (hipHostGetDevicePointer(&dp, h, 0) != hipSuccess || dp != (void*)h) qcopy_same_va().store(false);
    }
    return e;
  }
  ~HostBuf() {
    if (h) (void)hipHostFree(h);
    for (T* p : old) (void)hipHostFree(p);
  }
};

struct ImproveBufs {
  HostBuf<unsigned char> h_flag;
  DevBuf<unsigned char> d_flag;
  HostBuf<int> h_moves, h_changed;
  DevBuf<int> d_moves, d_changed;
  HostBuf<long long> h_before, h_after;
  DevBuf<long long> d_before, d_after;
  HostBuf<unsigned char> h_xflag;
  DevBuf<unsigned char> d_xflag;
  HostBuf<int> h_xmoves, h_xtb, h_xta, h_moves2;
  DevBuf<int> d_xmoves, d_xrej, d_xtb, d_xta, d_moves2, d_changed2;
  HostBuf<long long> h_after2;
  DevBuf<long long> d_xbefore, d_xafter, d_before2, d_after2;
  bool reserve(size_t R) {
    return !(h_flag.need(R) || d_flag.need(R) || h_moves.need(R) || h_changed.need(R) || d_moves.need(R) ||
             d_changed.need(R) || h_before.need(R) || h_after.need(R) || d_before.need(R) || d_after.need(R) ||
             h_xflag.need(R) || d_xflag.need(R) || h_xmoves.need(R) || h_xtb.need(R) || h_xta.need(R) ||
             h_moves2.need(R) || d_xmoves.need(R) || d_xrej.need(R) || d_xtb.need(R) || d_xta.need(R) ||
             d_moves2.need(R) || d_changed2.need(R) || h_after2.need(R) || d_xbefore.need(R) || d_xafter.need(R) ||
             d_before2.need(R) || d_after2.need(R));
  }
};

}
```

csrc/route_service_impl.h:

```cpp
#pragma once
#include <array>
#include <atomic>
#include <chrono>
#include <condition_variable>
#include <cstdarg>
#include <cstdio>
#include <deque>
#include <functional>
#include <list>
#include <memory>
#include <mutex>
#include <thread>
#include <unordered_map>
#include <unordered_set>

#include "common.h"
#include "ops.h"
#include "route_service.h"
#include "route_service_bufs.h"

namespace rt {

struct Batch {
  std::vector<RouteJob*> jobs;
  std::vector<std::shared_ptr<CchMetricDev>> metrics;
  std::vector<std::shared_ptr<const std::vector<float>>> host_cost;
  std::vector<rtr::Leg> legs;
  std::vector<std::vector<int32_t>> host_paths;
  std::vector<int32_t> flat;
  std::vector<int32_t> flat_e;
  std::unordered_map<uint64_t, int> leg_index;
  bool failed = false;
  std::shared_ptr<const std::vector<double>> alt_delay;
  int alt_kind = 0;
  std::string alt_engine;
  std::vector<RouteJob*> save;
};

inline double now_us() {
  return std::chrono::duration<double, std::micro>(std::chrono::steady_clock::now().time_since_epoch()).count();
}

inline rtc::Stamp local_now(int64_t skew_s = 0) {
  struct timespec ts;
  clock_gettime(CLOCK_REALTIME, &ts);
  struct tm lt;
  time_t t = ts.tv_sec + (time_t)skew_s;
  localtime_r(&t, &lt);
  rtc::Stamp s;
  s.secs = rtc::days_from_civil(lt.tm_year + 1900, (unsigned)lt.tm_mon + 1, (unsigned)lt.tm_mday) * 86400 +
           lt.tm_hour * 3600 + lt.tm_min * 60 + lt.tm_sec;
  s.us = (int32_t)(ts.tv_nsec / 1000);
  return s;
}

struct TripBufs {
  HostBuf<double> h_lat, h_lon, h_dem, h_cap, h_maxd, h_row0;
  HostBuf<int> h_npts, h_visit, h_trip, h_ntrips, h_status;
  DevBuf<double> d_lat, d_lon, d_dem, d_cap, d_maxd, d_D;
  DevBuf<int> d_npts, d_visit, d_trip, d_ntrips, d_status;
  HostBuf<int> h_pts, h_npts2, h_rowg;
  DevBuf<int> d_pts, d_npts2, d_rowg;
  DevBuf<float> d_msec, d_mmet;
  ImproveBufs imp;
  bool reserve(size_t R, size_t NM, bool road) {
    const size_t RN = R * NM;
    if (!imp.reserve(R)) return false;
    if (road)
      return !(h_pts.need(RN) || h_npts2.need(R) || h_dem.need(RN) || h_cap.need(R) || h_maxd.need(R) ||
               h_visit.need(RN) || h_trip.need(RN) || h_ntrips.need(R) || h_status.need(R) || h_row0.need(RN) ||
               d_pts.need(RN) || d_npts2.need(R) || d_dem.need(RN) || d_cap.need(R) || d_maxd.need(R) ||
               d_D.need(RN * NM) || d_msec.need(RN * NM) || d_mmet.need(RN * NM) || d_visit.need(RN) ||
               d_trip.need(RN) || d_ntrips.need(R) || d_status.need(R) || h_rowg.need(R) || d_rowg.need(R));
    return !(h_lat.need(RN) || h_lon.need(RN) || h_dem.need(RN) || h_npts.need(R) || h_cap.need(R) || h_maxd.need(R) ||
             h_visit.need(RN) || h_trip.need(RN) || h_ntrips.need(R) || h_status.need(R) || h_row0.need(RN) ||
             d_lat.need(RN) || d_lon.need(RN) || d_dem.need(RN) || d_npts.need(R) || d_cap.need(R) || d_maxd.need(R) ||
             d_D.need(RN * NM) || d_visit.need(RN) || d_trip.need(RN) || d_ntrips.need(R) || d_status.need(R));
  }
};

struct LegBufs {
  HostBuf<int> h_src, h_dst, h_len, h_st, h_qidx, h_flat, h_flat_e;
  HostBuf<float> h_cost, h_met;
  HostBuf<long long> h_off;
  DevBuf<int> d_src, d_dst, d_len, d_st, d_path, d_qidx, d_flat, d_iters, d_edge, d_flat_e;
  DevBuf<float> d_cost, d_met;
  DevBuf<long long> d_off;
  HostBuf<int> h_lgrp, h_lr, h_li, h_lj;
  DevBuf<int> d_lgrp, d_lr, d_li, d_lj;
  bool reserve(size_t Q, size_t QA, size_t MP, bool cch) {
    if (!cch)
      return !(h_src.need(Q) || h_dst.need(Q) || h_len.need(Q) || h_st.need(Q) || h_cost.need(Q) || h_off.need(Q) ||
               h_qidx.need(Q) || d_src.need(Q) || d_dst.need(Q) || d_len.need(Q) || d_st.need(Q) || d_cost.need(Q) ||
               d_off.need(Q) || d_qidx.need(Q + 1) || d_iters.need(Q) || d_path.need(Q * MP));
    if (h_src.need(Q) || h_dst.need(Q) || h_len.need(Q) || h_st.need(Q) || h_cost.need(Q) || h_met.need(Q) ||
        h_off.need(Q) || d_src.need(Q) || d_dst.need(Q) || d_len.need(Q) || d_st.need(Q) || d_cost.need(Q) ||
        d_met.need(Q) || d_off.need(Q) || d_path.need(Q * MP) || d_edge.need(Q * MP) || h_lgrp.need(Q) ||
        d_lgrp.need(Q))
      return false;
    return QA == 0 ||
           !(h_lr.need(QA) || h_li.need(QA) || h_lj.need(QA) || d_lr.need(QA) || d_li.need(QA) || d_lj.need(QA));
  }
  bool reserve_flat(size_t total) { return !(h_flat.need(total) || d_flat.need(total)); }
  bool reserve_flat_e(size_t total) { return !(h_flat_e.need(total) || d_flat_e.need(total)); }
};

struct CchBufs {
  HostBuf<CchMView> h_mv;
  DevBuf<CchMView> d_mv;
  HostBuf<float> h_hcost;
  bool reserve(size_t G) { return !(h_mv.need(G) || d_mv.need(G)); }
};

struct EtaBufs {
  HostBuf<rtc::EtaRecord> h_rec;
  HostBuf<float> h_eta;
  DevBuf<rtc::EtaRecord> d_rec;
  DevBuf<float> d_eta;
  bool reserve(size_t n) { return !(h_rec.need(n) || h_eta.need(n) || d_rec.need(n) || d_eta.need(n)); }
};

struct RouteService::Impl {
  RouteServiceCfg cfg;
  std::function<void(RouteJob*)> done;
  unsigned chunk_threads() const { return (unsigned)(cfg.chunk_threads < 1 ? 1 : cfg.chunk_threads); }
  std::function<void(std::vector<RouteJob*>&)> done_many;
  void done_all(std::vector<RouteJob*>& js) {
    if (js.empty()) return;
    if (done_many) {
      done_many(js);
    } else {
      for (RouteJob* j : js) done(j);
    }
  }
  std::mutex mu;
  std::condition_variable cv;
  std::deque<RouteJob*> q;
  bool stop = false;
  std::thread th, th_asm;
  hipStream_t stream{}, stream_asm{};
  rtr::NodeGrid grid;
  std::mutex amu;
  std::condition_variable acv;
  std::deque<Batch*> aq;
  bool gpu_done = false;
  std::atomic<long long> n_legs_reused{0};
  std::atomic<long long> n_jobs{0}, n_flushes{0}, n_fallback{0}, n_legs{0}, n_host_legs{0}, n_escalated{0};
  std::atomic<long long> t_stage[8] = {};
  std::atomic<long long> t_collect_us{0}, t_handoff_us{0};
  void add_t(int k, double t0) {
    const long long dt = (long long)(now_us() - t0);
    t_stage[k].fetch_add(dt, std::memory_order_relaxed);
    if (trace_ms >= 0 && dt > trace_ms * 1e3) {
      static const char* const names[8] = {"parse", "trips", "snap", "astar", "copyout", "assemble", "eta", "persist"};
      trace("stage %s took %.1f ms", names[k], dt * 1e-3);
    }
  }
  TripBufs tb;
  LegBufs lb;
  CchBufs cb;
  EtaBufs eb;
  ModelWs eta_ws;
  void cp(hipError_t& e, void* dst, const void* src, size_t bytes) {
    if (e == hipSuccess) e = qcopy(dst, src, bytes, stream);
  }
  CchScratch csc;
  CchScratch msc;
  uint64_t mtag = 0;
  std::unordered_map<const RouteJob*, int> jrow;
  std::mutex hc_mu;
  std::list<std::pair<uint64_t, std::shared_ptr<const std::vector<float>>>> hc_lru;
  std::unordered_map<uint64_t, decltype(hc_lru)::iterator> hc_index;
  static constexpr size_t HC_MAX = 64;
  std::atomic<long long> n_ctx_built{0};
  std::atomic<long long> t_ctx_us{0};
  bool async_ctx = true;
  int listener = 0;
  std::mutex wmu;
  std::unordered_map<uint64_t, std::vector<RouteJob*>> waiting;
  std::atomic<long long> n_deferred{0}, t_wait_us{0}, n_prefetch{0};
  double deadline_ms = 2000.0;
  std::atomic<double> flush_deadline_ms{2000.0};
  std::atomic<bool> broken{false};
  hipEvent_t ev_gpu{}, ev_asm{};
  hipStream_t hang_stream{};
  std::atomic<long long> n_failed_over{0};
  std::atomic<long long> n_records{0}, n_record_bytes{0};
  bool fail_fault = false;

  double trace_ms = -1.0;
  void trace(const char* fmt, ...) __attribute__((format(printf, 2, 3))) {
    if (trace_ms < 0) return;
    char buf[512];
    va_list ap;
    va_start(ap, fmt);
    std::vsnprintf(buf, sizeof buf, fmt, ap);
    va_end(ap);
    std::fprintf(stderr, "[route slot %d t=%.3f] %s\n", cfg.slot,
                 std::chrono::duration<double>(std::chrono::steady_clock::now().time_since_epoch()).count(), buf);
  }
  hipError_t sync(hipStream_t s, hipEvent_t ev, const char* what = "");
  bool drained() {
    return (!ev_gpu || hipEventQuery(ev_gpu) != hipErrorNotReady) && (!ev_asm || hipEventQuery(ev_asm) != hipErrorNotReady);
  }
  void hand_off(std::vector<RouteJob*>& jobs);
  std::unordered_map<int, double> seen_now;
  int prefetched_wh = -1;
  int64_t clock_skew_s = 0;
  std::unordered_set<int> prefetched;
  int prefetch_min = 10;
  rts::RouteStore store;
  std::thread th_persist;
  std::mutex pmu;
  std::condition_variable pcv;
  std::deque<std::vector<RouteJob*>> pq;
  bool asm_done = false;

  rtr::CoordCache coord_cache;
  std::vector<double> edge_heading;
  std::shared_ptr<const rrec::RecordGraph> rg;
  const rtr::CoordCache* ccache() const {
    if (rg) return rg->cc;
    return coord_cache.ofs.empty() ? nullptr : &coord_cache;
  }
  const double* headings() const {
    if (rg) return rg->heading;
    return edge_heading.empty() ? nullptr : edge_heading.data();
  }
  static uint64_t leg_key(int group, int s, int t) {
    return ((uint64_t)(uint32_t)group << 48) ^ ((uint64_t)(uint32_t)s << 24) ^ (uint64_t)(uint32_t)t;
  }

  void run();
  void asm_loop();
  void persist_loop();
  void prewarm();
  void on_built(uint64_t key, bool ok);
  static void parse_job(RouteJob* j);
  void gpu_stage(Batch& b);
  void asm_stage(Batch& b);
  void assemble_all(Batch& b);
  bool run_eta(std::vector<RouteJob*>& jobs);
  void finish(RouteJob* j);
  std::shared_ptr<const std::vector<float>> host_costs(const std::shared_ptr<CchMetricDev>& m);
  bool cch_groups(Batch& b);
  bool plan_multi(std::vector<RouteJob*>& jobs);
  bool plan_multi_road(Batch& b);
  hipError_t improve_rows(bool any, const int* d_npts, int R, int NM);
  void unpack_plan(RouteJob* j, int n, int NM, int k, bool improved);
  std::vector<RouteJob*> snap_jobs(Batch& b);
  bool compact_out(Batch& b, int Q, bool edges, const char* what);
  bool search_legs_cch(Batch& b);
  bool search_legs(Batch& b);
  void choose_alternatives(Batch& b, RouteJob* j);
};

}
```

csrc/route_service_legs.hip:

```cpp
#include <algorithm>
#include <cmath>
#include <queue>

#include "route_service_impl.h"
#include "runtime/alternatives.h"

namespace rt {

namespace {

__global__ void compact_paths_kernel(const int* __restrict__ rows, int max_path, const int* __restrict__ len,
                                     const int* __restrict__ status, const long long* __restrict__ off, int Q,
                                     int* __restrict__ flat) {
  const int q = blockIdx.x;
  if (q >= Q || status[q] != 0) return;
  const int n = min(len[q], max_path);
  const long long o = off[q];
  for (int i = threadIdx.x; i < n; i += blockDim.x) flat[o + i] = rows[(size_t)q * max_path + i];
}

bool host_dijkstra(const int* indptr, const int* indices, const float* cost, int N, int s, int t, int max_path,
                   float& out_cost, std::vector<int32_t>& path) {
  std::vector<double> dist((size_t)N, INFINITY);
  std::vector<int32_t> par((size_t)N, -1);
  using QE = std::pair<double, int>;
  std::priority_queue<QE, std::vector<QE>, std::greater<QE>> pq;
  dist[s] = 0.0;
  pq.push({0.0, s});
  while (!pq.empty()) {
    auto [d, v] = pq.top();
    pq.pop();
    if (d > dist[v]) continue;
    if (v == t) break;
    for (int e = indptr[v]; e < indptr[v + 1]; ++e) {
      const int w = indices[e];
      const double nd = d + (double)cost[e];
      if (nd < dist[w]) {
        dist[w] = nd;
        par[w] = v;
        pq.push({nd, w});
      }
    }
  }
  if (!std::isfinite(dist[t])) return false;
  path.clear();
  for (int v = t; v != -1; v = par[v]) {
    path.push_back(v);
    if ((int)path.size() > max_path) return false;
    if (v == s) break;
  }
  std::reverse(path.begin(), path.end());
  out_cost = (float)dist[t];
  return true;
}

}

std::vector<RouteJob*> RouteService::Impl::snap_jobs(Batch& b) {
  const double t0 = now_us();
  std::vector<RouteJob*> g;
  for (RouteJob* j : b.jobs)
    if (!j->fallback && !j->calls.empty()) g.push_back(j);
  rtc::parallel_chunks(g.size(), 64, chunk_threads(), [&](size_t lo, size_t hi) {
    for (size_t i = lo; i < hi; ++i) {
      RouteJob* j = g[i];
      j->nodes.clear();
      for (const auto& c : j->calls)
        for (const auto& pt : c) j->nodes.push_back(grid.nearest(pt.second, pt.first, cfg.snap_c));
    }
  });
  add_t(2, t0);
  return g;
}

bool RouteService::Impl::compact_out(Batch& b, int Q, bool edges, const char* what) {
  const int MP = cfg.max_path;
  long long total = 0;
  for (int i = 0; i < Q; ++i) {
    lb.h_off.h[i] = total;
    if (lb.h_st.h[i] == 0) total += std::min(lb.h_len.h[i], MP);
  }
  if (total == 0) return true;
  if (!lb.reserve_flat((size_t)total)) return false;
  hipError_t e = qcopy(lb.d_off.d, lb.h_off.h, (size_t)Q * 8, stream);
  if (e == hipSuccess) {
    hipLaunchKernelGGL(compact_paths_kernel, dim3(Q), dim3(256), 0, stream, lb.d_path.d, MP, lb.d_len.d, lb.d_st.d,
                       lb.d_off.d, Q, lb.d_flat.d);
    e = hipGetLastError();
  }
  if (edges) {
    if (e == hipSuccess && !lb.reserve_flat_e((size_t)total)) e = hipErrorOutOfMemory;
    if (e == hipSuccess) {
      hipLaunchKernelGGL(compact_paths_kernel, dim3(Q), dim3(256), 0, stream, lb.d_edge.d, MP, lb.d_len.d, lb.d_st.d,
                         lb.d_off.d, Q, lb.d_flat_e.d);
      e = hipGetLastError();
    }
  }
  if (e == hipSuccess) e = qcopy(lb.h_flat.h, lb.d_flat.d, (size_t)total * 4, stream);
  if (edges && e == hipSuccess) e = qcopy(lb.h_flat_e.h, lb.d_flat_e.d, (size_t)total * 4, stream);
  if (e == hipSuccess) e = sync(stream, ev_gpu, what);
  if (e != hipSuccess) return false;
  b.flat.assign(lb.h_flat.h, lb.h_flat.h + total);
  if (edges) b.flat_e.assign(lb.h_flat_e.h, lb.h_flat_e.h + total);
  return true;
}

bool RouteService::Impl::search_legs_cch(Batch& b) {
  std::vector<rtr::Leg>& legs = b.legs;
  std::unordered_map<uint64_t, int>& leg_index = b.leg_index;
  const std::vector<RouteJob*> g = snap_jobs(b);
  double t0 = now_us();
  const int G = (int)b.metrics.size();
  std::vector<std::vector<std::pair<int, int>>> pairs(G);
  std::vector<int> order;
  std::vector<std::vector<std::array<int, 3>>> tri(G);
  std::vector<std::vector<std::pair<int, int>>> rest(G);
  auto want = [&](int grp, int s, int t, int row, int i, int jj) {
    if (!leg_index.emplace(leg_key(grp, s, t), -1 - grp).second) return;
    if (row >= 0) {
      pairs[grp].emplace_back(s, t);
      tri[grp].push_back({row, i, jj});
    } else {
      rest[grp].emplace_back(s, t);
    }
  };
  for (RouteJob* j : g) {
    int row = -1;
    if (mtag != 0 && !j->plan.trips.empty()) {
      auto it = jrow.find(j);
      if (it != jrow.end()) row = it->second;
    }
    size_t off = 0;
    for (size_t ci = 0; ci < j->calls.size(); ++ci) {
      const auto& c = j->calls[ci];
      const bool from_trip = row >= 0 && ci < j->plan.trips.size() && j->plan.trips[ci].size() == c.size();
      for (size_t i = 0; i + 1 < c.size(); ++i)
        want(j->group, j->nodes[off + i], j->nodes[off + i + 1], from_trip ? row : -1,
             from_trip ? j->plan.trips[ci][i] : 0, from_trip ? j->plan.trips[ci][i + 1] : 0);
      off += c.size();
    }
  }
  std::vector<RouteJob*> alt_jobs;
  for (RouteJob* j : g)
    if (j->req.alt_k > 0) alt_jobs.push_back(j);
  rtc::parallel_chunks(alt_jobs.size(), 1, chunk_threads(), [&](size_t lo, size_t hi) {
    for (size_t i = lo; i < hi; ++i) {
      RouteJob* j = alt_jobs[i];
      j->alt_pairs.clear();
      std::unordered_map<uint64_t, int> seen;
      size_t off = 0;
      for (const auto& c : j->calls) {
        for (size_t k = 0; k + 1 < c.size(); ++k) {
          const int s = j->nodes[off + k], t = j->nodes[off + k + 1];
          if (seen.emplace(((uint64_t)(uint32_t)s << 32) | (uint32_t)t, 0).second) j->alt_pairs.emplace_back(s, t);
        }
        off += c.size();
      }
      j->alt_vias.assign(j->alt_pairs.size(), {});
      for (size_t k = 0; k < j->alt_pairs.size(); ++k)
        j->alt_vias[k] = ralt::via_nodes(cfg.glat, cfg.glon, cfg.N, j->alt_pairs[k].first, j->alt_pairs[k].second,
                                         j->req.alt_k - 1);
    }
  });
  for (RouteJob* j : alt_jobs)
    for (size_t k = 0; k < j->alt_pairs.size(); ++k)
      for (int w : j->alt_vias[k]) {
        want(j->group, j->alt_pairs[k].first, w, -1, 0, 0);
        want(j->group, w, j->alt_pairs[k].second, -1, 0, 0);
      }
  int QA = 0, QR = 0;
  for (int gi = 0; gi < G; ++gi) {
    QA += (int)pairs[gi].size();
    QR += (int)rest[gi].size();
  }
  const int Q = QA + QR;
  {
    int a = 0, r = QA;
    for (int gi = 0; gi < G; ++gi) {
      for (const auto& pr : pairs[gi]) leg_index[leg_key(gi, pr.first, pr.second)] = a++;
      for (const auto& pr : rest[gi]) leg_index[leg_key(gi, pr.first, pr.second)] = r++;
    }
  }
  legs.assign(Q, rtr::Leg());
  if (Q == 0) return true;
  n_legs.fetch_add(Q, std::memory_order_relaxed);
  const int MP = cfg.max_path;
  if (!lb.reserve((size_t)Q, (size_t)QA, (size_t)MP, true)) return false;
  {
    int a = 0, r = QA;
    for (int gi = 0; gi < G; ++gi) {
      for (size_t k = 0; k < pairs[gi].size(); ++k, ++a) {
        lb.h_src.h[a] = pairs[gi][k].first;
        lb.h_dst.h[a] = pairs[gi][k].second;
        lb.h_lgrp.h[a] = gi;
        lb.h_lr.h[a] = tri[gi][k][0];
        lb.h_li.h[a] = tri[gi][k][1];
        lb.h_lj.h[a] = tri[gi][k][2];
      }
      for (const auto& pr : rest[gi]) {
        lb.h_src.h[r] = pr.first;
        lb.h_dst.h[r] = pr.second;
        lb.h_lgrp.h[r] = gi;
        ++r;
      }
    }
  }
  hipError_t e = qcopy(lb.d_src.d, lb.h_src.h, (size_t)Q * 4, stream);
  if (e == hipSuccess) e = qcopy(lb.d_dst.d, lb.h_dst.h, (size_t)Q * 4, stream);
  if (e == hipSuccess) e = qcopy(lb.d_lgrp.d, lb.h_lgrp.h, (size_t)Q * 4, stream);
  if (QA > 0) {
    if (e == hipSuccess) e = qcopy(lb.d_lr.d, lb.h_lr.h, (size_t)QA * 4, stream);
    if (e == hipSuccess) e = qcopy(lb.d_li.d, lb.h_li.h, (size_t)QA * 4, stream);
    if (e == hipSuccess) e = qcopy(lb.d_lj.d, lb.h_lj.h, (size_t)QA * 4, stream);
  }
  auto out_at = [&](int q) {
    CchRouteOut o;
    o.sec = lb.d_cost.d + q;
    o.metres = lb.d_met.d + q;
    o.status = lb.d_st.d + q;
    o.len = lb.d_len.d + q;
    o.path = lb.d_path.d + (size_t)q * MP;
    o.edges = lb.d_edge.d + (size_t)q * MP;
    o.max_path = MP;
    return o;
  };
  if (e == hipSuccess && QA > 0)
    e = cfg.cch->legs_from_matrix_multi(cb.d_mv.d, lb.d_lgrp.d, lb.d_src.d, lb.d_lr.d, lb.d_li.d, lb.d_lj.d, QA, mtag, out_at(0), msc,
                                        stream);
  if (e == hipSuccess && QR > 0)
    e = cfg.cch->route_multi(cb.d_mv.d, lb.d_lgrp.d + QA, lb.d_src.d + QA, lb.d_dst.d + QA, QR, out_at(QA), csc, stream);
  n_legs_reused.fetch_add(QA, std::memory_order_relaxed);
  if (e == hipSuccess) e = qcopy(lb.h_st.h, lb.d_st.d, (size_t)Q * 4, stream);
  if (e == hipSuccess) e = qcopy(lb.h_len.h, lb.d_len.d, (size_t)Q * 4, stream);
  if (e == hipSuccess) e = qcopy(lb.h_cost.h, lb.d_cost.d, (size_t)Q * 4, stream);
  if (e == hipSuccess) e = qcopy(lb.h_met.h, lb.d_met.d, (size_t)Q * 4, stream);
  if (e == hipSuccess) e = sync(stream, ev_gpu, "cch-legs");
  add_t(3, t0);
  t0 = now_us();
  if (e != hipSuccess) return false;
  if (!compact_out(b, Q, true, "cch-paths")) return false;
  add_t(4, t0);
  int nbad = 0;
  for (int i = 0; i < Q; ++i) nbad += lb.h_st.h[i] == 4;
  b.host_paths.resize(Q);
  for (int i = 0; i < Q; ++i) {
      const int gi = lb.h_lgrp.h[i];
      rtr::Leg& L = legs[i];
      if (lb.h_st.h[i] == 0) {
        L.sec = lb.h_cost.h[i];
        L.metres = lb.h_met.h[i];
        L.len = std::min(lb.h_len.h[i], MP);
        L.path = b.flat.data() + lb.h_off.h[i];
        L.edges = b.flat_e.data() + lb.h_off.h[i];
      } else if (lb.h_st.h[i] == 4 && nbad <= 1024 && cfg.h_indptr != nullptr) {
        const std::vector<float>& hc = *b.host_cost[gi];
        float c;
        if (host_dijkstra(cfg.h_indptr, cfg.h_indices, hc.data(), cfg.N, lb.h_src.h[i], lb.h_dst.h[i], 1 << 22, c,
                          b.host_paths[i])) {
          L.sec = c;
          float met = 0.f;
          const auto& p = b.host_paths[i];
          for (size_t k = 0; k + 1 < p.size(); ++k) {
            int32_t best = -1;
            for (int32_t ee = cfg.h_indptr[p[k]]; ee < cfg.h_indptr[p[k] + 1]; ++ee)
              if (cfg.h_indices[ee] == p[k + 1] && (best < 0 || hc[ee] < hc[best])) best = ee;
            if (best >= 0) met += cfg.h_length[best];
          }
          L.metres = met;
          L.len = (int)p.size();
          L.path = p.data();
          n_host_legs.fetch_add(1, std::memory_order_relaxed);
        }
      }
    }
  return true;
}

bool RouteService::Impl::search_legs(Batch& b) {
  std::vector<rtr::Leg>& legs = b.legs;
  std::vector<std::vector<int32_t>>& host_paths = b.host_paths;
  std::unordered_map<uint64_t, int>& leg_index = b.leg_index;
  const std::vector<RouteJob*> g = snap_jobs(b);
  double t0 = now_us();
  std::vector<std::pair<int, int>> pairs;
  for (RouteJob* j : g) {
    size_t off = 0;
    for (const auto& c : j->calls) {
      for (size_t i = 0; i + 1 < c.size(); ++i) {
        const uint64_t key = ((uint64_t)(uint32_t)j->nodes[off + i] << 32) | (uint32_t)j->nodes[off + i + 1];
        if (leg_index.emplace(key, (int)pairs.size()).second) pairs.emplace_back(j->nodes[off + i], j->nodes[off + i + 1]);
      }
      off += c.size();
    }
  }
  const int Q = (int)pairs.size();
  legs.assign(Q, rtr::Leg());
  if (Q == 0) return true;
  n_legs.fetch_add(Q, std::memory_order_relaxed);
  const int MP = cfg.max_path;
  if (!lb.reserve((size_t)Q, 0, (size_t)MP, false)) return false;
  for (int i = 0; i < Q; ++i) {
    lb.h_src.h[i] = pairs[i].first;
    lb.h_dst.h[i] = pairs[i].second;
  }
  hipError_t e = qcopy(lb.d_src.d, lb.h_src.h, (size_t)Q * 4, stream);
  if (e == hipSuccess) e = qcopy(lb.d_dst.d, lb.h_dst.h, (size_t)Q * 4, stream);
  AstarGraphDev gd;
  gd.indptr = cfg.indptr;
  gd.indices = cfg.indices;
  gd.cost = cfg.cost;
  gd.lat = cfg.lat32;
  gd.lon = cfg.lon32;
  gd.N = cfg.N;
  gd.inv_vmax = cfg.inv_vmax;
  gd.lm = cfg.lm;
  gd.K = cfg.K;
  AstarOut ao;
  ao.cost = lb.d_cost.d;
  ao.len = lb.d_len.d;
  ao.status = lb.d_st.d;
  ao.path = lb.d_path.d;
  ao.max_path = MP;
  ao.iters = lb.d_iters.d;
  AstarPlan pl;
  pl.max_iters = cfg.max_iters;
  pl.lane_pops = cfg.lane_pops;
  pl.wave_only_below = cfg.wave_only_below;
  pl.delta = cfg.wave_delta;
  pl.lane_max_m = cfg.lane_max_m;
  AstarRunStats rs;
  if (e == hipSuccess)
    e = astar_search(gd, lb.d_src.d, lb.d_dst.d, Q, cfg.lane_ws.slots > 0 ? &cfg.lane_ws : nullptr,
                     cfg.wave_ws.slots > 0 ? &cfg.wave_ws : nullptr, cfg.big_ws.slots > 0 ? &cfg.big_ws : nullptr,
                     ao, pl, lb.d_qidx.d, stream, &rs, cfg.arena.base ? &cfg.arena : nullptr);
  n_escalated.fetch_add(rs.escalated, std::memory_order_relaxed);
  if (e == hipSuccess) e = qcopy(lb.h_st.h, lb.d_st.d, (size_t)Q * 4, stream);
  if (e == hipSuccess) e = sync(stream, ev_gpu, "astar");
  add_t(3, t0);
  t0 = now_us();
  if (e == hipSuccess) e = qcopy(lb.h_len.h, lb.d_len.d, (size_t)Q * 4, stream);
  if (e == hipSuccess) e = qcopy(lb.h_cost.h, lb.d_cost.d, (size_t)Q * 4, stream);
  if (e == hipSuccess) e = sync(stream, ev_gpu, "astar-escalate");
  if (e != hipSuccess) return false;
  if (!compact_out(b, Q, false, "astar-paths")) return false;
  add_t(4, t0);
  int nbad = 0;
  for (int i = 0; i < Q; ++i) nbad += (lb.h_st.h[i] == 2 || lb.h_st.h[i] == 3);
  host_paths.resize(Q);
  for (int i = 0; i < Q; ++i) {
    rtr::Leg& L = legs[i];
    if (lb.h_st.h[i] == 0) {
      L.sec = lb.h_cost.h[i];
      L.len = std::min(lb.h_len.h[i], MP);
      L.path = b.flat.data() + lb.h_off.h[i];
    } else if ((lb.h_st.h[i] == 2 || lb.h_st.h[i] == 3) && nbad <= 1024 && cfg.h_indptr != nullptr) {
      float c;
      if (host_dijkstra(cfg.h_indptr, cfg.h_indices, cfg.h_cost, cfg.N, pairs[i].first, pairs[i].second, MP, c,
                        host_paths[i])) {
        L.sec = c;
        L.len = (int)host_paths[i].size();
        L.path = host_paths[i].data();
        n_host_legs.fetch_add(1, std::memory_order_relaxed);
      }
    }
  }
  return true;
}

void RouteService::Impl::choose_alternatives(Batch& b, RouteJob* j) {
  const std::vector<rtr::Leg>& legs = b.legs;
  const double* delay = b.alt_delay->data();
  const size_t P = j->alt_pairs.size();
  struct Cand {
    double sec, met;
    const int32_t* p1;
    int n1;
    const int32_t* p2;
    int n2;
    const int32_t* e1;
    const int32_t* e2;
  };
  auto leg = [&](int s, int t) -> const rtr::Leg* {
    auto it = b.leg_index.find(leg_key(j->group, s, t));
    return it == b.leg_index.end() || it->second < 0 ? nullptr : &legs[it->second];
  };
  std::vector<std::vector<Cand>> cands(P);
  size_t total = 0;
  for (size_t k = 0; k < P; ++k) {
    const int s = j->alt_pairs[k].first, t = j->alt_pairs[k].second;
    const rtr::Leg* d = leg(s, t);
    if (d && d->len > 0) cands[k].push_back({d->sec, d->metres, d->path, d->len, nullptr, 0, d->edges, nullptr});
    for (int w : j->alt_vias[k]) {
      const rtr::Leg* a = leg(s, w);
      const rtr::Leg* c = leg(w, t);
      if (a && c && a->len > 0 && c->len > 0)
        cands[k].push_back({a->sec + c->sec, a->metres + c->metres, a->path, a->len, c->path + 1, c->len - 1,
                            a->edges, c->edges});
    }
    total += cands[k].size();
  }
  (void)total;
  j->alt_legs.assign(P, rtr::Leg());
  j->alt_paths.assign(P, {});
  j->alt_edges.assign(P, {});
  std::string o = ",\"alternatives\":{\"k\":";
  rtr::put_int(o, j->req.alt_k);
  o += ",\"scorer\":";
  rtr::put_str(o, b.alt_engine);
  o += ",\"legs\":[";
  std::vector<int32_t> tmp;
  for (size_t k = 0; k < P; ++k) {
    if (k) o += ',';
    o += "{\"from_node\":";
    rtr::put_int(o, j->alt_pairs[k].first);
    o += ",\"to_node\":";
    rtr::put_int(o, j->alt_pairs[k].second);
    o += ",\"candidates\":";
    rtr::put_int(o, (long long)cands[k].size());
    if (cands[k].empty()) {
      o += '}';
      continue;
    }
    std::vector<double> sc(cands[k].size());
    for (size_t c = 0; c < cands[k].size(); ++c) {
      const Cand& x = cands[k][c];
      tmp.assign(x.p1, x.p1 + x.n1);
      if (x.p2) tmp.insert(tmp.end(), x.p2, x.p2 + x.n2);
      sc[c] = ralt::candidate_score(cfg.glat, cfg.glon, delay, tmp.data(), tmp.size(), x.sec, b.alt_kind);
    }
    const int best = ralt::argmin_score(sc);
    const Cand& x = cands[k][best];
    std::vector<int32_t>& own = j->alt_paths[k];
    own.assign(x.p1, x.p1 + x.n1);
    if (x.p2) own.insert(own.end(), x.p2, x.p2 + x.n2);
    rtr::Leg& L = j->alt_legs[k];
    L.sec = x.sec;
    L.metres = x.met;
    L.path = own.data();
    L.len = (int)own.size();
    if (x.e1 && (x.p2 == nullptr || x.e2)) {
      std::vector<int32_t>& oe = j->alt_edges[k];
      oe.assign(x.e1, x.e1 + (x.n1 - 1));
      if (x.p2) oe.insert(oe.end(), x.e2, x.e2 + x.n2);
      L.edges = oe.data();
    }
    o += ",\"chosen\":";
    rtr::put_int(o, best);
    o += ",\"scores\":[";
    for (size_t c = 0; c < sc.size(); ++c) {
      if (c) o += ',';
      rtr::put_float(o, sc[c]);
    }
    o += "],\"seconds\":[";
    for (size_t c = 0; c < cands[k].size(); ++c) {
      if (c) o += ',';
      rtr::put_float(o, cands[k][c].sec);
    }
    o += "]}";
  }
  o += "]}";
  j->alt_json = std::move(o);
}

}
```

csrc/route_service_plan.hip:

```cpp
#include <algorithm>
#include <cmath>
#include <cstring>

#include "route_service_impl.h"

namespace rt {

std::shared_ptr<const std::vector<float>> RouteService::Impl::host_costs(const std::shared_ptr<CchMetricDev>& m) {
  if (m->host_cost.size() == (size_t)cfg.cch->topo().E) return {m, &m->host_cost};
  {
    std::lock_guard<std::mutex> lk(hc_mu);
    auto it = hc_index.find(m->key);
    if (it != hc_index.end()) {
      hc_lru.splice(hc_lru.begin(), hc_lru, it->second);
      return it->second->second;
    }
  }
  auto v = std::make_shared<std::vector<float>>((size_t)cfg.cch->topo().E);
  if (cb.h_hcost.need(v->size()) != hipSuccess || qcopy(cb.h_hcost.h, m->cost, v->size() * 4, stream) != hipSuccess ||
      sync(stream, ev_gpu, "host-costs") != hipSuccess)
    return nullptr;
  std::memcpy(v->data(), cb.h_hcost.h, v->size() * 4);
  std::lock_guard<std::mutex> lk(hc_mu);
  if (hc_index.count(m->key)) return v;
  hc_lru.emplace_front(m->key, v);
  hc_index[m->key] = hc_lru.begin();
  while (hc_lru.size() > HC_MAX) {
    hc_index.erase(hc_lru.back().first);
    hc_lru.pop_back();
  }
  return v;
}

bool RouteService::Impl::cch_groups(Batch& b) {
  if (cfg.cch != nullptr) cfg.cch->note_queries();
  const rtc::Stamp now = local_now(clock_skew_s);
  const int64_t days = (int64_t)std::floor((double)now.secs / 86400.0);
  const int64_t sec_of_day = now.secs - days * 86400;
  const int now_wh = (int)(((days + 3) % 7 + 7) % 7) * 24 + (int)(sec_of_day / 3600);
  const double t_now = now_us();
  std::unordered_map<uint64_t, int> gidx;
  std::vector<CchContext> ctxs;
  std::vector<char> sync;
  for (RouteJob* j : b.jobs) {
    if (j->fallback || !j->req.error.empty()) continue;
    CchContext c;
    uint64_t key = cfg.cch_fixed_key;
    if (cfg.cch_contexts) {
      c.weather = j->req.route_weather;
      c.congestion = j->req.route_congestion;
      c.weekhour = j->req.route_weekhour >= 0 ? j->req.route_weekhour : now_wh;
      key = c.key();
      if (j->req.route_weekhour < 0) seen_now[(c.weather & 0xFF) | (c.congestion << 8)] = t_now;
    }
    auto it = gidx.find(key);
    if (it == gidx.end()) {
      it = gidx.emplace(key, (int)ctxs.size()).first;
      ctxs.push_back(c);
      sync.push_back(0);
    }
    j->group = it->second;
    if (j->sync_ctx) sync[j->group] = 1;
  }
  std::vector<std::shared_ptr<CchMetricDev>> met(ctxs.size());
  std::vector<char> ready(ctxs.size(), 1);
  for (size_t g = 0; g < ctxs.size(); ++g) {
    if (!cfg.cch_contexts) {
      if (!cfg.cch->cached_metric(cfg.cch_fixed_key, met[g])) return false;
    } else if (async_ctx && !sync[g]) {
      ready[g] = cfg.cch->cached_metric(ctxs[g].key(), met[g]) ? 1 : 0;
    } else {
      const double t0 = now_us();
      bool fresh = false;
      if (cfg.cch->metric_for(ctxs[g], stream, met[g], &fresh) != hipSuccess) return false;
      if (fresh) {
        n_ctx_built.fetch_add(1, std::memory_order_relaxed);
        t_ctx_us.fetch_add((long long)(now_us() - t0), std::memory_order_relaxed);
      }
    }
  }
  std::vector<int> remap(ctxs.size(), -1);
  for (size_t g = 0; g < ctxs.size(); ++g)
    if (ready[g]) {
      remap[g] = (int)b.metrics.size();
      b.metrics.push_back(met[g]);
    }
  std::vector<CchContext> to_build;
  if (b.metrics.size() < ctxs.size()) {
    std::vector<RouteJob*> keep;
    keep.reserve(b.jobs.size());
    {
      std::lock_guard<std::mutex> lk(wmu);
      for (RouteJob* j : b.jobs) {
        if (j->fallback || !j->req.error.empty() || ready[j->group]) {
          keep.push_back(j);
          continue;
        }
        if (j->defer_t0 == 0.0) {
          j->defer_t0 = t_now;
          n_deferred.fetch_add(1, std::memory_order_relaxed);
        }
        waiting[ctxs[j->group].key()].push_back(j);
      }
    }
    b.jobs.swap(keep);
    for (size_t g = 0; g < ctxs.size(); ++g)
      if (!ready[g]) to_build.push_back(ctxs[g]);
  }
  for (RouteJob* j : b.jobs) {
    if (j->fallback || !j->req.error.empty()) continue;
    j->group = remap[j->group];
    if (j->defer_t0 > 0.0) {
      t_wait_us.fetch_add((long long)(t_now - j->defer_t0), std::memory_order_relaxed);
      j->defer_t0 = -1.0;
    }
  }
  for (const CchContext& c : to_build) cfg.cch->request_build(c, true);
  const int min_in_hour = (int)((sec_of_day % 3600) / 60);
  const int next_wh = (now_wh + 1) % 168;
  if (cfg.cch_contexts && async_ctx && prefetch_min > 0 && min_in_hour >= 60 - prefetch_min) {
    if (prefetched_wh != next_wh) {
      prefetched_wh = next_wh;
      prefetched.clear();
    }
    for (auto it = seen_now.begin(); it != seen_now.end();) {
      if (t_now - it->second > 3600e6) { it = seen_now.erase(it); continue; }
      if (!prefetched.insert(it->first).second) { ++it; continue; }
      CchContext c;
      c.weather = it->first & 0xFF;
      c.congestion = it->first >> 8;
      c.weekhour = next_wh;
      cfg.cch->request_build(c, false);
      n_prefetch.fetch_add(1, std::memory_order_relaxed);
      ++it;
    }
  }
  b.host_cost.assign(b.metrics.size(), nullptr);
  for (size_t g = 0; g < b.metrics.size(); ++g) {
    b.host_cost[g] = host_costs(b.metrics[g]);
    if (!b.host_cost[g]) return false;
  }
  const size_t G = b.metrics.size();
  if (G > 0) {
    if (!cb.reserve(G)) return false;
    for (size_t g = 0; g < G; ++g) cb.h_mv.h[g] = CchGpu::view(*b.metrics[g]);
    if (qcopy(cb.d_mv.d, cb.h_mv.h, G * sizeof(CchMView), stream) != hipSuccess) return false;
  }
  return true;
}

bool RouteService::Impl::plan_multi(std::vector<RouteJob*>& jobs) {
  std::vector<RouteJob*> m;
  for (RouteJob* j : jobs)
    if (!j->fallback && j->req.error.empty() && j->req.dst.size() > 1) m.push_back(j);
  if (m.empty()) return true;
  const int R = (int)m.size();
  int NM = 1;
  for (RouteJob* j : m) NM = std::max(NM, (int)j->req.dst.size() + 1);
  if (NM > 4096) {
    for (RouteJob* j : m) j->fallback = true;
    return true;
  }
  const size_t RN = (size_t)R * NM;
  if (!tb.reserve((size_t)R, (size_t)NM, false)) return false;
  for (int k = 0; k < R; ++k) {
    const rtr::RouteReq& r = m[k]->req;
    const int n = (int)r.dst.size() + 1;
    double* la = tb.h_lat.h + (size_t)k * NM;
    double* lo = tb.h_lon.h + (size_t)k * NM;
    double* de = tb.h_dem.h + (size_t)k * NM;
    std::fill(la, la + NM, 0.0);
    std::fill(lo, lo + NM, 0.0);
    std::fill(de, de + NM, 0.0);
    la[0] = r.src.lat;
    lo[0] = r.src.lon;
    for (int i = 1; i < n; ++i) {
      la[i] = r.dst[i - 1].lat;
      lo[i] = r.dst[i - 1].lon;
      de[i] = r.dst[i - 1].demand;
    }
    tb.h_npts.h[k] = n;
    tb.h_cap.h[k] = r.cap;
    tb.h_maxd.h[k] = r.maxd;
    tb.imp.h_flag.h[k] = r.improve || r.exchange ? 1 : 0;
    tb.imp.h_xflag.h[k] = r.exchange ? 1 : 0;
  }
  const bool any_imp = std::any_of(m.begin(), m.end(), [](const RouteJob* j) { return j->req.improve || j->req.exchange; });
  hipError_t e = hipSuccess;
  cp(e, tb.d_lat.d, tb.h_lat.h, RN * 8);
  cp(e, tb.d_lon.d, tb.h_lon.h, RN * 8);
  cp(e, tb.d_dem.d, tb.h_dem.h, RN * 8);
  cp(e, tb.d_npts.d, tb.h_npts.h, (size_t)R * 4);
  cp(e, tb.d_cap.d, tb.h_cap.h, (size_t)R * 8);
  cp(e, tb.d_maxd.d, tb.h_maxd.h, (size_t)R * 8);
  if (e == hipSuccess) e = launch_haversine_matrix(tb.d_lat.d, tb.d_lon.d, tb.d_npts.d, R, NM, cfg.circuity, tb.d_D.d, stream);
  if (e == hipSuccess)
    e = launch_greedy_cvrp(tb.d_D.d, tb.d_npts.d, tb.d_dem.d, tb.d_cap.d, tb.d_maxd.d, R, NM, tb.d_visit.d, tb.d_trip.d, tb.d_ntrips.d,
                           tb.d_status.d, stream);
  if (e == hipSuccess) e = improve_rows(any_imp, tb.d_npts.d, R, NM);
  cp(e, tb.h_visit.h, tb.d_visit.d, RN * 4);
  cp(e, tb.h_trip.h, tb.d_trip.d, RN * 4);
  cp(e, tb.h_ntrips.h, tb.d_ntrips.d, (size_t)R * 4);
  cp(e, tb.h_status.h, tb.d_status.d, (size_t)R * 4);
  if (e == hipSuccess)
    e = qcopy2d(tb.h_row0.h, (size_t)NM * 8, tb.d_D.d, (size_t)NM * NM * 8, (size_t)NM * 8, (size_t)R, stream);
  if (e == hipSuccess) e = sync(stream, ev_gpu, "k5k6-matrix");
  if (e != hipSuccess) return false;
  for (int k = 0; k < R; ++k) unpack_plan(m[k], tb.h_npts.h[k], NM, k, any_imp);
  return true;
}

bool RouteService::Impl::plan_multi_road(Batch& b) {
  jrow.clear();
  mtag = 0;
  const int G = (int)b.metrics.size();
  std::vector<std::vector<RouteJob*>> byg(G);
  int NM = 1;
  for (RouteJob* j : b.jobs)
    if (!j->fallback && j->req.error.empty() && j->req.dst.size() > 1 && j->group >= 0 && j->group < G) {
      if ((int)j->req.dst.size() + 1 > 4096) {
        j->fallback = true;
        continue;
      }
      byg[j->group].push_back(j);
      NM = std::max(NM, (int)j->req.dst.size() + 1);
    }
  std::vector<RouteJob*> m;
  std::vector<int> r0(G + 1, 0);
  for (int g = 0; g < G; ++g) {
    r0[g] = (int)m.size();
    m.insert(m.end(), byg[g].begin(), byg[g].end());
  }
  r0[G] = (int)m.size();
  if (m.empty()) return true;
  const int R = (int)m.size();
  const size_t RN = (size_t)R * NM;
  if (!tb.reserve((size_t)R, (size_t)NM, true)) return false;
  for (int g = 0; g < G; ++g)
    for (int k = r0[g]; k < r0[g + 1]; ++k) tb.h_rowg.h[k] = g;
  rtc::parallel_chunks((size_t)R, 64, chunk_threads(), [&](size_t lo, size_t hi) {
    for (size_t k = lo; k < hi; ++k) {
      const rtr::RouteReq& r = m[k]->req;
      const int n = (int)r.dst.size() + 1;
      int* pt = tb.h_pts.h + k * NM;
      double* de = tb.h_dem.h + k * NM;
      std::fill(pt, pt + NM, 0);
      std::fill(de, de + NM, 0.0);
      pt[0] = grid.nearest(r.src.lat, r.src.lon, cfg.snap_c);
      for (int i = 1; i < n; ++i) {
        pt[i] = grid.nearest(r.dst[i - 1].lat, r.dst[i - 1].lon, cfg.snap_c);
        de[i] = r.dst[i - 1].demand;
      }
      tb.h_npts2.h[k] = n;
      tb.h_cap.h[k] = r.cap;
      tb.h_maxd.h[k] = r.maxd;
      tb.imp.h_flag.h[k] = r.improve || r.exchange ? 1 : 0;
    tb.imp.h_xflag.h[k] = r.exchange ? 1 : 0;
    }
  });
  const bool any_imp = std::any_of(m.begin(), m.end(), [](const RouteJob* j) { return j->req.improve || j->req.exchange; });
  hipError_t e = hipSuccess;
  cp(e, tb.d_pts.d, tb.h_pts.h, RN * 4);
  cp(e, tb.d_npts2.d, tb.h_npts2.h, (size_t)R * 4);
  cp(e, tb.d_dem.d, tb.h_dem.h, RN * 8);
  cp(e, tb.d_cap.d, tb.h_cap.h, (size_t)R * 8);
  cp(e, tb.d_maxd.d, tb.h_maxd.h, (size_t)R * 8);
  cp(e, tb.d_rowg.d, tb.h_rowg.h, (size_t)R * 4);
  if (e == hipSuccess)
    e = cfg.cch->matrix_multi(cb.d_mv.d, tb.d_rowg.d, tb.d_pts.d, tb.d_npts2.d, R, NM, tb.d_msec.d, tb.d_mmet.d, tb.d_D.d, msc, stream);
  mtag = e == hipSuccess ? msc.chain_tag : 0;
  for (int k = 0; k < R; ++k) jrow[m[k]] = k;
  if (e == hipSuccess)
    e = launch_greedy_cvrp(tb.d_D.d, tb.d_npts2.d, tb.d_dem.d, tb.d_cap.d, tb.d_maxd.d, R, NM, tb.d_visit.d, tb.d_trip.d, tb.d_ntrips.d,
                           tb.d_status.d, stream);
  if (e == hipSuccess) e = improve_rows(any_imp, tb.d_npts2.d, R, NM);
  cp(e, tb.h_visit.h, tb.d_visit.d, RN * 4);
  cp(e, tb.h_trip.h, tb.d_trip.d, RN * 4);
  cp(e, tb.h_ntrips.h, tb.d_ntrips.d, (size_t)R * 4);
  cp(e, tb.h_status.h, tb.d_status.d, (size_t)R * 4);
  if (e == hipSuccess)
    e = qcopy2d(tb.h_row0.h, (size_t)NM * 8, tb.d_D.d, (size_t)NM * NM * 8, (size_t)NM * 8, (size_t)R, stream);
  if (e == hipSuccess) e = sync(stream, ev_gpu, "cch-matrix+greedy");
  if (e != hipSuccess) return false;
  for (int k = 0; k < R; ++k) unpack_plan(m[k], tb.h_npts2.h[k], NM, k, any_imp);
  return true;
}

hipError_t RouteService::Impl::improve_rows(bool any, const int* d_npts, int R, int NM) {
  if (!any) return hipSuccess;
  hipError_t e = hipSuccess;
  cp(e, tb.imp.d_flag.d, tb.imp.h_flag.h, (size_t)R);
  if (e == hipSuccess)
    e = launch_improve_trips(tb.d_D.d, d_npts, tb.d_maxd.d, tb.imp.d_flag.d, tb.d_status.d, R, NM, tb.d_visit.d, tb.d_trip.d,
                             tb.imp.d_moves.d, tb.imp.d_changed.d, tb.imp.d_before.d, tb.imp.d_after.d, stream);
  cp(e, tb.imp.h_moves.h, tb.imp.d_moves.d, (size_t)R * 4);
  cp(e, tb.imp.h_changed.h, tb.imp.d_changed.d, (size_t)R * 4);
  cp(e, tb.imp.h_before.h, tb.imp.d_before.d, (size_t)R * 8);
  cp(e, tb.imp.h_after.h, tb.imp.d_after.d, (size_t)R * 8);
  if (!std::any_of(tb.imp.h_xflag.h, tb.imp.h_xflag.h + R, [](unsigned char f) { return f != 0; })) return e;
  cp(e, tb.imp.d_xflag.d, tb.imp.h_xflag.h, (size_t)R);
  if (e == hipSuccess)
    e = launch_exchange_trips(tb.d_D.d, d_npts, tb.d_dem.d, tb.d_cap.d, tb.d_maxd.d, tb.imp.d_xflag.d, tb.d_status.d, R, NM, -1,
                              tb.d_visit.d, tb.d_trip.d, tb.d_ntrips.d, tb.imp.d_xmoves.d, tb.imp.d_xrej.d, tb.imp.d_xtb.d,
                              tb.imp.d_xta.d, tb.imp.d_xbefore.d, tb.imp.d_xafter.d, stream);
  if (e == hipSuccess)
    e = launch_improve_trips(tb.d_D.d, d_npts, tb.d_maxd.d, tb.imp.d_xflag.d, tb.d_status.d, R, NM, tb.d_visit.d, tb.d_trip.d,
                             tb.imp.d_moves2.d, tb.imp.d_changed2.d, tb.imp.d_before2.d, tb.imp.d_after2.d, stream);
  cp(e, tb.imp.h_xmoves.h, tb.imp.d_xmoves.d, (size_t)R * 4);
  cp(e, tb.imp.h_xtb.h, tb.imp.d_xtb.d, (size_t)R * 4);
  cp(e, tb.imp.h_xta.h, tb.imp.d_xta.d, (size_t)R * 4);
  cp(e, tb.imp.h_moves2.h, tb.imp.d_moves2.d, (size_t)R * 4);
  cp(e, tb.imp.h_after2.h, tb.imp.d_after2.d, (size_t)R * 8);
  return e;
}

void RouteService::Impl::unpack_plan(RouteJob* j, int n, int NM, int k, bool improved) {
  rtr::Plan& p = j->plan;
  const int* vis = tb.h_visit.h + (size_t)k * NM;
  const int* tof = tb.h_trip.h + (size_t)k * NM;
  if (tb.h_status.h[k] != 0) {
    std::vector<char> placed(n, 0);
    for (int i = 0; i < NM && vis[i] >= 0; ++i) placed[vis[i]] = 1;
    std::vector<int> rest;
    for (int i = 1; i < n; ++i)
      if (!placed[i]) rest.push_back(i);
    const double* d0 = tb.h_row0.h + (size_t)k * NM;
    std::stable_sort(rest.begin(), rest.end(), [&](int a, int c) { return d0[a] < d0[c]; });
    p.infeasible = true;
    for (int i : rest) p.infeasible_stops.push_back(i - 1);
    return;
  }
  p.trips.assign(tb.h_ntrips.h[k], std::vector<int>{0});
  for (int i = 0; i < NM && vis[i] >= 0; ++i) p.trips[tof[i]].push_back(vis[i]);
  for (auto& t : p.trips) t.push_back(0);
  if (improved && j->req.exchange) {
    p.improved = true;
    p.imp.exchange = true;
    p.imp.moves = (long long)tb.imp.h_moves.h[k] + tb.imp.h_moves2.h[k];
    p.imp.exchange_moves = tb.imp.h_xmoves.h[k];
    p.imp.trips_before = tb.imp.h_xtb.h[k];
    p.imp.trips_after = tb.imp.h_xta.h[k];
    p.imp.len_before_q = tb.imp.h_before.h[k];
    p.imp.len_after_q = tb.imp.h_after2.h[k];
  } else if (improved && j->req.improve) {
    p.improved = true;
    p.imp.moves = tb.imp.h_moves.h[k];
    p.imp.trips_changed = tb.imp.h_changed.h[k];
    p.imp.len_before_q = tb.imp.h_before.h[k];
    p.imp.len_after_q = tb.imp.h_after.h[k];
  }
}

}
```

routest_amd/serve/native_server.py:

```python
from __future__ import annotations

import socket
from typing import Dict, List, Optional, Sequence

import torch

from ..ops._ext import native
from ..ops.eta_mlp import EtaMlpKernel


def free_port() -> int:
    s = socket.socket()
    s.bind(("127.0.0.1", 0))
    p = s.getsockname()[1]
    s.close()
    return p


def _mlp_host(model) -> dict:
    m = model.float().cpu()
    return {"w1": m.l1.weight.detach().contiguous(), "b1": m.l1.bias.detach().contiguous(),
            "w2": m.l2.weight.detach().contiguous(), "b2": m.l2.bias.detach().contiguous(),
            "w3": m.l3.weight.detach().reshape(-1).contiguous(), "b3": float(m.l3.bias.detach()[0]),
            "x_mean": m.x_mean.detach().contiguous(), "x_std": m.x_std.detach().contiguous(),
            "y_mean": float(m.y_mean), "y_std": float(m.y_std)}


def native_supported(model) -> bool:
    from ..models.forest import ForestModel
    from ..models.mlp3 import EtaMLP
    return (isinstance(model, EtaMLP) and model.hidden in (64, 128, 256, 512, 1024)) or isinstance(model, ForestModel)


def native_model_spec(model, device: int, variant: int = -1) -> dict:
    from ..models.forest import ForestModel
    from ..models.mlp3 import EtaMLP
    dev = torch.device("cuda", device)
    if isinstance(model, EtaMLP) and model.hidden in (64, 128, 256):
        k = EtaMlpKernel(model, dev, variant=variant)
        return {"kind": "mlp3", "blob": k.packed.blob, "H": k.hidden, "norm": list(k.packed.norm),
                "variant": int(variant), "host": _mlp_host(model)}
    if isinstance(model, EtaMLP) and model.hidden in (512, 1024):
        from ..ops.mlp_big import PackedBig
        p = PackedBig(model.float().cpu(), dev)
        return {"kind": "wide", "H": p.hidden, "w1q": p.w1q, "w2f": p.w2f, "b2": p.b2, "w3": p.w3, "b3": p.b3,
                "norm": list(p.norm), "host": _mlp_host(model)}
    if isinstance(model, ForestModel):
        import numpy as np
        model.validate()
        return {"kind": "forest", "values": torch.from_numpy(np.ascontiguousarray(model.values)),
                "info": torch.from_numpy(np.ascontiguousarray(model.info.view(np.int32))),
                "roots": torch.from_numpy(np.ascontiguousarray(model.roots)), "base": float(model.base_score),
                "le": bool(model.le), "fmap": [int(x) for x in model.feature_map]}
    raise ValueError(f"the native front end does not serve {type(model).__name__} models")


class NativePredictServer:

    def __init__(self, model, device=0, port: int = 0, threads: int = 2, max_batch: int = 1 << 18,
                 cors_origins: Sequence[str] = ("http://localhost:3000", "http://127.0.0.1:3000"),
                 cors_vercel: bool = True, bind_any: bool = False, variant: int = -1,
                 upstream_port: int = 0, routes: Optional[List[dict]] = None, history_db: str = ""):
        self.C = native(required=True)
        self.devices = [device] if isinstance(device, int) else list(device)
        self.routes = list(routes or [])
        self.variant = variant
        threads = max(threads, len(self.devices))
        self.port = port or free_port()
        specs = [native_model_spec(model, d, variant) for d in self.devices]
        self.model_epoch = 1
        self.h: Optional[int] = self.C.native_server_start(
            self.port, threads, self.devices, specs, max_batch, list(cors_origins), cors_vercel, bind_any,
            int(upstream_port), self.routes, history_db)
        self.history_db = history_db

    def set_model(self, model) -> int:
        specs = [native_model_spec(model, d, self.variant) if model is not None else {"kind": "none"}
                 for d in self.devices]
        self.model_epoch = int(self.C.native_server_set_models(self.h, self.devices, specs))
        return self.model_epoch

    def set_fault(self, slot: int, on: bool = True, kind: str = "fail") -> bool:
        if kind == "hang":
            return bool(self.C.native_server_set_hang(self.h, slot, on))
        return bool(self.C.native_server_set_fault(self.h, slot, on))

    def set_scorer(self, scorer) -> bool:
        if self.h is None:
            return False
        if scorer is None:
            return bool(self.C.native_server_set_scorer(self.h, [], 0, ""))
        import numpy as np
        from ..routing.alternatives import KINDS
        delay = np.ascontiguousarray(scorer.node_delays(), dtype=np.float64)
        return bool(self.C.native_server_set_scorer(self.h, delay.tolist(), KINDS[getattr(scorer, "kind", "edge")],
                                                    str(getattr(scorer, "engine", "gcn"))))

    def health(self) -> Dict:
        if self.h is None:
            return {}
        h = dict(self.C.native_server_health(self.h))
        st = self.stats()
        h["stats"] = {k: st.get(k) for k in ("requests", "predictions", "launches", "errors", "resident",
                                             "fallbacks", "failovers", "cpu_rounds", "route_jobs",
                                             "route_flushes", "route_service_fallbacks", "route_legs",
                                             "route_contexts_built", "route_failed_over", "timeouts")}
        h["degraded"] = any(s["quarantined"] for s in h["slots"])
        return h

    def stats(self) -> Dict[str, int]:
        if self.h is None:
            return {}
        v = self.C.native_server_stats(self.h)
        names = ("requests", "predictions", "launches", "errors", "resident", "fallbacks", "wire8",
                 "route_requests", "route_fallbacks", "relayed", "route_jobs", "route_flushes",
                 "route_service_fallbacks", "route_legs", "route_host_legs", "route_persisted",
                 "route_us_parse", "route_us_trips", "route_us_snap", "route_us_astar", "route_us_copyout",
                 "route_us_assemble", "route_us_eta", "route_us_persist",
                 "route_astar_escalated",
                 "route_contexts_built", "route_us_context",
                 "route_legs_reused",
                 "failovers", "cpu_rounds",
                 "history_native",
                 "cached",
                 "route_ctx_deferred", "route_us_ctx_wait", "route_ctx_prefetched",
                 "route_failed_over", "timeouts",
                 "route_records", "route_record_bytes",
                 "route_us_collect", "route_us_handoff")
        return dict(zip(names, v))

    def close(self) -> None:
        if self.h is not None:
            self.C.native_server_stop(self.h)
            self.h = None

    def __enter__(self):
        return self

    def __exit__(self, *exc):
        self.close()
        return False


def route_config(provider, device, *, engine: str = "backend:mi355x", compat200: bool = True,
                 batch_max: int = 1024, timeout_us: int = 500, store=None, astar=None,
                 chunk_threads: int = 16) -> dict:
    name = getattr(provider, "name", "")
    cfg = {"provider": "graph" if name == "graph" else "haversine", "engine": engine,
           "compat200": bool(compat200), "batch_max": int(batch_max), "timeout_us": float(timeout_us),
           "chunk_threads": max(1, int(chunk_threads)),
           "circuity": float(getattr(provider, "circuity", 1.3)), "step_m": float(getattr(provider, "step_m", 150.0)),
           "sqlite_path": getattr(store, "sqlite_uri", "") if store is not None else ""}
    if name == "graph" and getattr(provider, "engine", "astar") != "astar":
        import numpy as np
        g = provider.g
        dev = torch.device("cuda", device) if isinstance(device, int) else torch.device(device)
        router = provider.router(dev)
        if router.gpu is None:
            raise ValueError("the native route service needs the GPU router")
        cfg.update({
            "router": "cch", "cch_ptr": int(router.gpu.ptr()), "cch_contexts": bool(provider.uses_context),
            "cch_fixed_key": int(provider.FIXED_KEY),
            "glat": torch.from_numpy(np.ascontiguousarray(g.lat, dtype=np.float64)),
            "glon": torch.from_numpy(np.ascontiguousarray(g.lon, dtype=np.float64)),
            "h_indptr": torch.from_numpy(np.ascontiguousarray(g.indptr, dtype=np.int32)),
            "h_indices": torch.from_numpy(np.ascontiguousarray(g.indices, dtype=np.int32)),
            "h_length": torch.from_numpy(np.ascontiguousarray(g.length_m, dtype=np.float32)),
            "h_edge_name": (torch.from_numpy(np.ascontiguousarray(g.edge_name, dtype=np.int32))
                            if g.edge_name is not None else None),
            "names": list(g.names or []),
            "N": int(g.num_nodes), "snap_c": float(g.SNAP_C), "max_path": int(router.max_path),
            "_router": router})
        return cfg
    if name == "graph":
        import numpy as np
        a = astar
        if a is None or a.perm is not None:
            raise ValueError("graph routes need a BatchedAstar without node reordering")
        g = a.g
        cfg.update({
            "glat": torch.from_numpy(np.ascontiguousarray(g.lat, dtype=np.float64)),
            "glon": torch.from_numpy(np.ascontiguousarray(g.lon, dtype=np.float64)),
            "h_indptr": torch.from_numpy(np.ascontiguousarray(g.indptr, dtype=np.int32)),
            "h_indices": torch.from_numpy(np.ascontiguousarray(g.indices, dtype=np.int32)),
            "h_cost": a.cost.detach().cpu().contiguous(),
            "indptr": a.indptr, "indices": a.indices, "cost": a.cost, "lat32": a.lat, "lon32": a.lon,
            "lm": a.lm, "K": (a.lm.shape[1] // 2) if a.lm is not None else 0,
            "lane_ws": a.lane_tier.ws(), "wave_ws": a.wave_tier.ws() if a.wave_tier else None,
            "big_ws": a.big_tier.ws() if a.big_tier else None,
            "arena": a.arena, "arena_ctr": a.arena_ctr if a.arena is not None else None,
            "N": int(g.num_nodes), "snap_c": float(g.SNAP_C),
            "max_path": int(a.max_path), "max_iters": int(a.max_iters), "lane_pops": int(a.lane_pops),
            "wave_only_below": int(a.wave_only_below),
            "inv_vmax": float(a.inv_vmax), "wave_delta": float(a.wave_delta),
            "lane_max_m": float(a.lane_max_m),
            "_astar": a})
    return cfg


NativeFrontEnd = NativePredictServer
```

Before: 6.569 billion.

## Batch route host/device copies into one segment-list kernel launch per flush

```diff
diff --git a/csrc/bindings.cpp b/csrc/bindings.cpp
--- a/csrc/bindings.cpp
+++ b/csrc/bindings.cpp
@@ -1668,6 +1668,50 @@
                                      (int)roots.numel(), (int)nodes2.size(0), (float)base, le ? 1 : 0, fm,
                                      num_cus(records.device().index()), cur_stream(records)));
   return out;
+}
+
+int64_t route_copy_list(std::vector<std::tuple<torch::Tensor, int64_t, torch::Tensor, int64_t, int64_t, int64_t, int64_t,
+                                               int64_t>> segs) {
+  std::vector<std::array<long long, 6>> v;
+  hipStream_t s = nullptr;
+  for (auto& g : segs) {
+    const torch::Tensor& dst = std::get<0>(g);
+    const torch::Tensor& src = std::get<2>(g);
+    const int64_t doff = std::get<1>(g), soff = std::get<3>(g), width = std::get<4>(g), rows = std::get<5>(g);
+    const int64_t dpitch = std::get<6>(g), spitch = std::get<7>(g);
+    TORCH_CHECK(dst.scalar_type() == torch::kUInt8 && src.scalar_type() == torch::kUInt8, "segments are uint8 tensors");
+    TORCH_CHECK(doff >= 0 && soff >= 0 && width >= 0 && rows >= 0 && dpitch >= width && spitch >= width, "bad segment");
+    if (rows > 0 && width > 0) {
+      TORCH_CHECK(doff + (rows - 1) * dpitch + width <= dst.numel(), "segment past the end of dst");
+      TORCH_CHECK(soff + (rows - 1) * spitch + width <= src.numel(), "segment past the end of src");
+    }
+    if (dst.is_cuda()) s = cur_stream(dst);
+    if (src.is_cuda()) s = cur_stream(src);
+    v.push_back({(long long)(uintptr_t)((unsigned char*)kernel_ptr(dst, "dst") + doff),
+                 (long long)(uintptr_t)((const unsigned char*)kernel_ptr(src, "src") + soff), (long long)width,
+                 (long long)rows, (long long)dpitch, (long long)spitch});
+  }
+  long long launches = 0;
+  RT_CHECK_HIP(rt::route_copy_list_run(v, s, &launches));
+  return (int64_t)launches;
+}
+
+void route_leg_offsets_compact(torch::Tensor rows, torch::Tensor len, torch::Tensor status, torch::Tensor off,
+                               torch::Tensor flat, int64_t capacity) {
+  check_dev(rows, "rows");
+  check_dev(len, "len");
+  check_dev(status, "status");
+  check_dev(off, "off");
+  const int64_t Q = len.numel();
+  TORCH_CHECK(rows.scalar_type() == torch::kInt32 && len.scalar_type() == torch::kInt32 &&
+              status.scalar_type() == torch::kInt32 && flat.scalar_type() == torch::kInt32 &&
+              off.scalar_type() == torch::kInt64, "int32 rows / len / status / flat, int64 off");
+  TORCH_CHECK(Q >= 1 && rows.dim() == 2 && rows.size(0) == Q && status.numel() == Q && off.numel() == Q + 1, "bad shapes");
+  TORCH_CHECK(capacity >= 0 && capacity <= flat.numel(), "capacity exceeds flat");
+  const c10::DeviceGuard guard(rows.device());
+  RT_CHECK_HIP(rt::route_leg_offsets_compact(rows.data_ptr<int>(), (int)rows.size(1), len.data_ptr<int>(),
+                                             status.data_ptr<int>(), (int)Q, (long long*)off.data_ptr<int64_t>(),
+                                             (int*)kernel_ptr(flat, "flat"), capacity, cur_stream(rows)));
 }
 
 }
@@ -1831,6 +1875,9 @@
     py::gil_scoped_release nogil;
     rt::native_server_stop(h);
   });
+  m.def("route_copy_list", &route_copy_list, "test hook: the route flushes' segment-list copy; returns its launches");
+  m.def("route_leg_offsets_compact", &route_leg_offsets_compact,
+        "test hook: found paths' offsets (off[Q] = total) + compaction into flat (GPU or pinned)");
   m.def("native_server_stats", [](int64_t h) {
     const auto v = rt::native_server_stats(h);
     return std::vector<int64_t>(v.begin(), v.end());
diff --git a/csrc/native_model.h b/csrc/native_model.h
--- a/csrc/native_model.h
+++ b/csrc/native_model.h
@@ -28,6 +28,7 @@
   virtual ~NativeModel() = default;
   virtual hipError_t predict(const void* rec, int rec_bytes, float* out, int B, hipStream_t s, ModelWs& ws) const = 0;
   virtual bool takes_wire8() const { return true; }
+  virtual bool streams_host_io() const { return false; }
   virtual const void* mlp3_blob() const { return nullptr; }
   virtual const NormParams* mlp3_norm() const { return nullptr; }
   virtual bool cpu_predict(const rtc::EtaRecord* rec, float* out, int B) const = 0;
diff --git a/csrc/native_model.hip b/csrc/native_model.hip
--- a/csrc/native_model.hip
+++ b/csrc/native_model.hip
@@ -89,6 +89,7 @@
   hipError_t predict(const void* rec, int rec_bytes, float* out, int B, hipStream_t s, ModelWs&) const override {
     return launch_eta_mlp3_fwd(rec, out, B, blob.p, H, np, variant, cus, s, rec_bytes);
   }
+  bool streams_host_io() const override { return true; }
   const void* mlp3_blob() const override { return blob.p; }
   const NormParams* mlp3_norm() const override { return &np; }
   bool cpu_predict(const rtc::EtaRecord* rec, float* out, int B) const override { return mlp_cpu_batch(host, rec, out, B); }
diff --git a/csrc/native_server.hip b/csrc/native_server.hip
--- a/csrc/native_server.hip
+++ b/csrc/native_server.hip
@@ -1523,7 +1523,7 @@
 
 std::vector<long long> native_server_stats(int64_t h) {
   std::lock_guard<std::mutex> lk(g_srv_mu);
-  if (h < 0 || h >= (int64_t)g_servers.size() || !g_servers[h]) return std::vector<long long>(41, 0);
+  if (h < 0 || h >= (int64_t)g_servers.size() || !g_servers[h]) return std::vector<long long>(44, 0);
   Server* s = g_servers[h];
   std::vector<long long> v = {s->stats.requests.load(), s->stats.predictions.load(), s->stats.launches.load(),
                               s->stats.errors.load(), s->stats.resident.load(), s->stats.fallbacks.load(),
@@ -1552,6 +1552,12 @@
     for (size_t i = 0; i < rr.size() && 22 + i < x.size(); ++i) rr[i] += x[22 + i];
   }
   v.insert(v.end(), rr.begin(), rr.end());
+  std::vector<long long> rc(3, 0);
+  for (auto& r : s->routes) {
+    const auto x = r->stats();
+    for (size_t i = 0; i < rc.size() && 26 + i < x.size(); ++i) rc[i] += x[26 + i];
+  }
+  v.insert(v.end(), rc.begin(), rc.end());
   return v;
 }
 
diff --git a/csrc/route_service.h b/csrc/route_service.h
--- a/csrc/route_service.h
+++ b/csrc/route_service.h
@@ -1,4 +1,5 @@
 #pragma once
+#include <array>
 #include <cmath>
 #include <functional>
 #include <memory>
@@ -128,4 +129,8 @@
   Impl* p_;
 };
 
+hipError_t route_copy_list_run(const std::vector<std::array<long long, 6>>& segs, hipStream_t s, long long* launches);
+hipError_t route_leg_offsets_compact(const int* rows, int max_path, const int* len, const int* status, int Q,
+                                     long long* off, int* flat, long long capacity, hipStream_t s);
+
 }
diff --git a/csrc/route_service.hip b/csrc/route_service.hip
--- a/csrc/route_service.hip
+++ b/csrc/route_service.hip
@@ -24,6 +24,7 @@
 hipError_t RouteService::Impl::sync(hipStream_t s, hipEvent_t ev, const char* what) {
   hipError_t e = hipEventRecord(ev, s);
   if (e != hipSuccess) return e;
+  n_gpu_syncs.fetch_add(1, std::memory_order_relaxed);
   const auto t0 = std::chrono::steady_clock::now();
   auto waited = [&] { return std::chrono::duration<double, std::milli>(std::chrono::steady_clock::now() - t0).count(); };
   for (int i = 0;; ++i) {
@@ -232,10 +233,11 @@
 void RouteService::Impl::prewarm() {
   const size_t R = (size_t)std::max(1, cfg.batch_max), NM = 11, RN = R * NM, Q = RN;
   const size_t MP = (size_t)std::max(1, cfg.max_path);
-  bool ok = tb.reserve(R, NM, false) && lb.reserve(Q, Q, MP, cfg.cch != nullptr) && lb.reserve_flat(Q * 256) &&
+  bool ok = tb.reserve(R, NM, false) && lb.reserve(Q, Q, MP, cfg.cch != nullptr) &&
+            lb.reserve_flat(Q * 256, !qcopy_same_va().load()) &&
             eb.reserve(R);
   if (cfg.cch != nullptr) {
-    ok = ok && tb.reserve(R, NM, true) && lb.reserve_flat_e(Q * 256) && cb.reserve(R) &&
+    ok = ok && tb.reserve(R, NM, true) && lb.reserve_flat_e(Q * 256, !qcopy_same_va().load()) && cb.reserve(R) &&
          cb.h_hcost.need((size_t)cfg.cch->topo().E) == hipSuccess;
     const int S = cfg.cch->stride();
     msc.device = cfg.device;
@@ -360,9 +362,17 @@
     r.traffic = j->req.eta_traffic;
     r.pad = 0;
   }
-  hipError_t e = qcopy(eb.d_rec.d, eb.h_rec.h, (size_t)n * 16, stream_asm);
-  if (e == hipSuccess) e = model->predict(eb.d_rec.d, 16, eb.d_eta.d, n, stream_asm, eta_ws);
-  if (e == hipSuccess) e = qcopy(eb.h_eta.h, eb.d_eta.d, (size_t)n * 4, stream_asm);
+  hipError_t e = hipSuccess;
+  if (model->streams_host_io() && qcopy_same_va().load(std::memory_order_relaxed)) {
+    e = model->predict(eb.h_rec.h, 16, eb.h_eta.h, n, stream_asm, eta_ws);
+  } else {
+    QCopyList io(stream_asm, &n_copy_launches);
+    io.add(eb.d_rec.d, eb.h_rec.h, (size_t)n * 16);
+    e = io.flush(stream_asm);
+    if (e == hipSuccess) e = model->predict(eb.d_rec.d, 16, eb.d_eta.d, n, stream_asm, eta_ws);
+    io.add(eb.h_eta.h, eb.d_eta.d, (size_t)n * 4);
+    if (e == hipSuccess) e = io.flush(stream_asm);
+  }
   if (e == hipSuccess) e = sync(stream_asm, ev_asm, "eta");
   std::vector<float> cpu_eta;
   const float* eta = eb.h_eta.h;
@@ -608,6 +618,9 @@
   v.push_back(p_->n_record_bytes.load());
   v.push_back(p_->t_collect_us.load());
   v.push_back(p_->t_handoff_us.load());
+  v.push_back(p_->n_copy_launches.load());
+  v.push_back(p_->n_gpu_syncs.load());
+  v.push_back(p_->n_flat_regrows.load());
   return v;
 }
 
diff --git a/csrc/route_service_bufs.h b/csrc/route_service_bufs.h
--- a/csrc/route_service_bufs.h
+++ b/csrc/route_service_bufs.h
@@ -8,45 +8,101 @@
 
 namespace rt {
 
-static __global__ __launch_bounds__(256) void route_copy_kernel(unsigned char* __restrict__ dst,
-                                                                const unsigned char* __restrict__ src, size_t bytes) {
-  const size_t nv = (((uintptr_t)dst | (uintptr_t)src) & 15) == 0 ? bytes / 16 : 0;
-  const size_t stride = (size_t)gridDim.x * blockDim.x;
-  for (size_t i = (size_t)blockIdx.x * blockDim.x + threadIdx.x; i < nv; i += stride)
-    reinterpret_cast<int4*>(dst)[i] = reinterpret_cast<const int4*>(src)[i];
-  for (size_t i = nv * 16 + (size_t)blockIdx.x * blockDim.x + threadIdx.x; i < bytes; i += stride) dst[i] = src[i];
+struct QCopySeg {
+  unsigned char* dst;
+  const unsigned char* src;
+  unsigned long long width, dpitch, spitch;
+  unsigned rows, pad;
+};
+constexpr int QCOPY_CAP = 16;
+struct QCopyArgs {
+  QCopySeg s[QCOPY_CAP];
+};
+
+template <class V>
+__device__ __forceinline__ void qcopy_body(const QCopySeg& g, size_t t0, size_t stride) {
+  const size_t nv = g.width / sizeof(V), nt = g.width - nv * sizeof(V);
+  if (g.rows == 1) {
+    for (size_t i = t0; i < nv; i += stride) reinterpret_cast<V*>(g.dst)[i] = reinterpret_cast<const V*>(g.src)[i];
+    for (size_t i = t0; i < nt; i += stride) g.dst[nv * sizeof(V) + i] = g.src[nv * sizeof(V) + i];
+    return;
+  }
+  for (size_t i = t0; i < nv * g.rows; i += stride) {
+    const size_t r = i / nv, c = (i - r * nv) * sizeof(V);
+    *reinterpret_cast<V*>(g.dst + r * g.dpitch + c) = *reinterpret_cast<const V*>(g.src + r * g.spitch + c);
+  }
+  for (size_t i = t0; i < nt * g.rows; i += stride) {
+    const size_t r = i / nt, c = nv * sizeof(V) + (i - r * nt);
+    g.dst[r * g.dpitch + c] = g.src[r * g.spitch + c];
+  }
 }
-static __global__ __launch_bounds__(256) void route_copy2d_kernel(unsigned char* __restrict__ dst, size_t dpitch,
-                                                                  const unsigned char* __restrict__ src, size_t spitch,
-                                                                  size_t width, size_t height) {
-  const size_t stride = (size_t)gridDim.x * blockDim.x;
-  for (size_t i = (size_t)blockIdx.x * blockDim.x + threadIdx.x; i < width * height; i += stride) {
-    const size_t r = i / width, c = i - r * width;
-    dst[r * dpitch + c] = src[r * spitch + c];
-  }
+static __global__ __launch_bounds__(256) void route_copy_list_kernel(const QCopyArgs a) {
+  const QCopySeg& g = a.s[blockIdx.y];
+  const size_t t0 = (size_t)blockIdx.x * blockDim.x + threadIdx.x, stride = (size_t)gridDim.x * blockDim.x;
+  uintptr_t al = (uintptr_t)g.dst | (uintptr_t)g.src;
+  if (g.rows > 1) al |= g.dpitch | g.spitch;
+  if ((al & 15) == 0) qcopy_body<int4>(g, t0, stride);
+  else if ((al & 7) == 0) qcopy_body<int2>(g, t0, stride);
+  else if ((al & 3) == 0) qcopy_body<int>(g, t0, stride);
+  else qcopy_body<unsigned char>(g, t0, stride);
 }
 inline std::atomic<bool>& qcopy_same_va() {
   static std::atomic<bool> ok{true};
   return ok;
 }
-inline hipError_t qcopy(void* dst, const void* src, size_t bytes, hipStream_t s) {
-  if (bytes == 0) return hipSuccess;
-  if (!qcopy_same_va().load(std::memory_order_relaxed)) return hipMemcpyAsync(dst, src, bytes, hipMemcpyDefault, s);
-  const size_t blocks = std::min<size_t>(1024, (bytes / 16 + 255) / 256 + 1);
-  hipLaunchKernelGGL(route_copy_kernel, dim3((unsigned)blocks), dim3(256), 0, s, (unsigned char*)dst,
-                     (const unsigned char*)src, bytes);
-  return hipGetLastError();
-}
-inline hipError_t qcopy2d(void* dst, size_t dpitch, const void* src, size_t spitch, size_t width, size_t height,
-                          hipStream_t s) {
-  if (width == 0 || height == 0) return hipSuccess;
-  if (!qcopy_same_va().load(std::memory_order_relaxed))
-    return hipMemcpy2DAsync(dst, dpitch, src, spitch, width, height, hipMemcpyDefault, s);
-  const size_t blocks = std::min<size_t>(1024, (width * height + 255) / 256);
-  hipLaunchKernelGGL(route_copy2d_kernel, dim3((unsigned)blocks), dim3(256), 0, s, (unsigned char*)dst, dpitch,
-                     (const unsigned char*)src, spitch, width, height);
-  return hipGetLastError();
-}
+
+struct QCopyList {
+  QCopyArgs a;
+  int n = 0;
+  size_t big = 0;
+  hipError_t err = hipSuccess;
+  hipStream_t stream = nullptr;
+  std::atomic<long long>* launches = nullptr;
+  QCopyList(hipStream_t s, std::atomic<long long>* count) : stream(s), launches(count) {}
+  void reset(hipStream_t s) {
+    n = 0;
+    big = 0;
+    err = hipSuccess;
+    stream = s;
+  }
+  void add2d(void* dst, size_t dpitch, const void* src, size_t spitch, size_t width, size_t rows) {
+    if (width == 0 || rows == 0) return;
+    if (n == QCOPY_CAP) (void)flush(stream);
+    QCopySeg& g = a.s[n++];
+    g.dst = (unsigned char*)dst;
+    g.src = (const unsigned char*)src;
+    g.width = width;
+    g.dpitch = dpitch;
+    g.spitch = spitch;
+    g.rows = (unsigned)rows;
+    g.pad = 0;
+    big = std::max(big, width * rows);
+  }
+  void add(void* dst, const void* src, size_t bytes) { add2d(dst, bytes, src, bytes, bytes, 1); }
+  hipError_t flush(hipStream_t s) {
+    if (n == 0 || err != hipSuccess) {
+      n = 0;
+      big = 0;
+      return err;
+    }
+    if (!qcopy_same_va().load(std::memory_order_relaxed)) {
+      for (int i = 0; i < n && err == hipSuccess; ++i) {
+        const QCopySeg& g = a.s[i];
+        err = g.rows == 1 ? hipMemcpyAsync(g.dst, g.src, g.width, hipMemcpyDefault, s)
+                          : hipMemcpy2DAsync(g.dst, g.dpitch, g.src, g.spitch, g.width, g.rows, hipMemcpyDefault, s);
+        if (launches) launches->fetch_add(1, std::memory_order_relaxed);
+      }
+    } else {
+      const size_t blocks = std::min<size_t>(1024, (big / 16 + 255) / 256 + 1);
+      hipLaunchKernelGGL(route_copy_list_kernel, dim3((unsigned)blocks, (unsigned)n), dim3(256), 0, s, a);
+      err = hipGetLastError();
+      if (launches) launches->fetch_add(1, std::memory_order_relaxed);
+    }
+    n = 0;
+    big = 0;
+    return err;
+  }
+};
 
 template <class T>
 struct DevBuf {
diff --git a/csrc/route_service_impl.h b/csrc/route_service_impl.h
--- a/csrc/route_service_impl.h
+++ b/csrc/route_service_impl.h
@@ -90,19 +90,19 @@
   DevBuf<int> d_lgrp, d_lr, d_li, d_lj;
   bool reserve(size_t Q, size_t QA, size_t MP, bool cch) {
     if (!cch)
-      return !(h_src.need(Q) || h_dst.need(Q) || h_len.need(Q) || h_st.need(Q) || h_cost.need(Q) || h_off.need(Q) ||
+      return !(h_src.need(Q) || h_dst.need(Q) || h_len.need(Q) || h_st.need(Q) || h_cost.need(Q) || h_off.need(Q + 1) ||
                h_qidx.need(Q) || d_src.need(Q) || d_dst.need(Q) || d_len.need(Q) || d_st.need(Q) || d_cost.need(Q) ||
-               d_off.need(Q) || d_qidx.need(Q + 1) || d_iters.need(Q) || d_path.need(Q * MP));
+               d_off.need(Q + 1) || d_qidx.need(Q + 1) || d_iters.need(Q) || d_path.need(Q * MP));
     if (h_src.need(Q) || h_dst.need(Q) || h_len.need(Q) || h_st.need(Q) || h_cost.need(Q) || h_met.need(Q) ||
-        h_off.need(Q) || d_src.need(Q) || d_dst.need(Q) || d_len.need(Q) || d_st.need(Q) || d_cost.need(Q) ||
-        d_met.need(Q) || d_off.need(Q) || d_path.need(Q * MP) || d_edge.need(Q * MP) || h_lgrp.need(Q) ||
+        h_off.need(Q + 1) || d_src.need(Q) || d_dst.need(Q) || d_len.need(Q) || d_st.need(Q) || d_cost.need(Q) ||
+        d_met.need(Q) || d_off.need(Q + 1) || d_path.need(Q * MP) || d_edge.need(Q * MP) || h_lgrp.need(Q) ||
         d_lgrp.need(Q))
       return false;
     return QA == 0 ||
            !(h_lr.need(QA) || h_li.need(QA) || h_lj.need(QA) || d_lr.need(QA) || d_li.need(QA) || d_lj.need(QA));
   }
-  bool reserve_flat(size_t total) { return !(h_flat.need(total) || d_flat.need(total)); }
-  bool reserve_flat_e(size_t total) { return !(h_flat_e.need(total) || d_flat_e.need(total)); }
+  bool reserve_flat(size_t total, bool dev) { return !(h_flat.need(total) || (dev && d_flat.need(total))); }
+  bool reserve_flat_e(size_t total, bool dev) { return !(h_flat_e.need(total) || (dev && d_flat_e.need(total))); }
 };
 
 struct CchBufs {
@@ -161,9 +161,9 @@
   CchBufs cb;
   EtaBufs eb;
   ModelWs eta_ws;
-  void cp(hipError_t& e, void* dst, const void* src, size_t bytes) {
-    if (e == hipSuccess) e = qcopy(dst, src, bytes, stream);
-  }
+  std::atomic<long long> n_copy_launches{0}, n_gpu_syncs{0}, n_flat_regrows{0};
+  QCopyList copies() { return QCopyList(stream, &n_copy_launches); }
+  QCopyList up{nullptr, &n_copy_launches};
   CchScratch csc;
   CchScratch msc;
   uint64_t mtag = 0;
@@ -246,10 +246,12 @@
   bool cch_groups(Batch& b);
   bool plan_multi(std::vector<RouteJob*>& jobs);
   bool plan_multi_road(Batch& b);
-  hipError_t improve_rows(bool any, const int* d_npts, int R, int NM);
+  void trips_up(bool any, int R);
+  hipError_t improve_rows(bool any, const int* d_npts, int R, int NM, QCopyList& down);
+  hipError_t trips_down(hipError_t e, size_t R, size_t NM, QCopyList& down, const char* what);
   void unpack_plan(RouteJob* j, int n, int NM, int k, bool improved);
   std::vector<RouteJob*> snap_jobs(Batch& b);
-  bool compact_out(Batch& b, int Q, bool edges, const char* what);
+  bool legs_out(Batch& b, hipError_t e, int Q, bool cch, double t0, const char* what);
   bool search_legs_cch(Batch& b);
   bool search_legs(Batch& b);
   void choose_alternatives(Batch& b, RouteJob* j);
diff --git a/csrc/route_service_legs.hip b/csrc/route_service_legs.hip
--- a/csrc/route_service_legs.hip
+++ b/csrc/route_service_legs.hip
@@ -9,14 +9,71 @@
 
 namespace {
 
-__global__ void compact_paths_kernel(const int* __restrict__ rows, int max_path, const int* __restrict__ len,
-                                     const int* __restrict__ status, const long long* __restrict__ off, int Q,
-                                     int* __restrict__ flat) {
+__global__ __launch_bounds__(256) void leg_offsets_kernel(const int* __restrict__ status, const int* __restrict__ len,
+                                                          int max_path, int Q, long long* __restrict__ off) {
+  constexpr int IT = 4;
+  __shared__ long long wsum[4];
+  const int lane = threadIdx.x & 63, wave = threadIdx.x >> 6;
+  long long carry = 0;
+  for (int base = 0; base < Q; base += 256 * IT) {
+    const int q0 = base + (int)threadIdx.x * IT;
+    int v[IT];
+    long long s = 0;
+#pragma unroll
+    for (int k = 0; k < IT; ++k) {
+      const int q = q0 + k;
+      v[k] = (q < Q && status[q] == 0) ? min(len[q], max_path) : 0;
+      s += v[k];
+    }
+    long long inc = s;
+#pragma unroll
+    for (int d = 1; d < 64; d <<= 1) {
+      const long long t = __shfl_up(inc, d, 64);
+      if (lane >= d) inc += t;
+    }
+    if (lane == 63) wsum[wave] = inc;
+    __syncthreads();
+    long long o = carry + inc - s;
+    for (int w = 0; w < wave; ++w) o += wsum[w];
+    carry += wsum[0] + wsum[1] + wsum[2] + wsum[3];
+#pragma unroll
+    for (int k = 0; k < IT; ++k) {
+      if (q0 + k < Q) off[q0 + k] = o;
+      o += v[k];
+    }
+    __syncthreads();
+  }
+  if (threadIdx.x == 0) off[Q] = carry;
+}
+
+__global__ __launch_bounds__(64) void compact_paths_kernel(const int* __restrict__ rows, int max_path,
+                                                           const int* __restrict__ len, const int* __restrict__ status,
+                                                           const long long* __restrict__ off, int Q, int* __restrict__ flat,
+                                                           long long capacity) {
   const int q = blockIdx.x;
-  if (q >= Q || status[q] != 0) return;
-  const int n = min(len[q], max_path);
-  const long long o = off[q];
-  for (int i = threadIdx.x; i < n; i += blockDim.x) flat[o + i] = rows[(size_t)q * max_path + i];
+  if (q >= Q || status[q] != 0 || off[Q] > capacity) return;
+  const int n = min(len[q], max_path), t = threadIdx.x;
+  const int* __restrict__ src = rows + (size_t)q * max_path;
+  int* __restrict__ dst = flat + off[q];
+  const int head = min(n, (int)(((16 - ((uintptr_t)dst & 15)) & 15) >> 2));
+  if (t < head) dst[t] = src[t];
+  const int nv = (n - head) >> 2;
+  for (int i = t; i < nv; i += 64) {
+    const int* s = src + head + 4 * i;
+    reinterpret_cast<int4*>(dst + head)[i] = make_int4(s[0], s[1], s[2], s[3]);
+  }
+  const int rest = head + 4 * nv + t;
+  if (rest < n) dst[rest] = src[rest];
+}
+
+hipError_t launch_offsets(const int* st, const int* len, int MP, int Q, long long* off, hipStream_t s) {
+  hipLaunchKernelGGL(leg_offsets_kernel, dim3(1), dim3(256), 0, s, st, len, MP, Q, off);
+  return hipGetLastError();
+}
+hipError_t launch_compact(const int* rows, int MP, const int* len, const int* st, const long long* off, int Q, int* flat,
+                          long long capacity, hipStream_t s) {
+  hipLaunchKernelGGL(compact_paths_kernel, dim3(Q), dim3(64), 0, s, rows, MP, len, st, off, Q, flat, capacity);
+  return hipGetLastError();
 }
 
 bool host_dijkstra(const int* indptr, const int* indices, const float* cost, int N, int s, int t, int max_path,
@@ -56,6 +113,23 @@
 
 }
 
+hipError_t route_copy_list_run(const std::vector<std::array<long long, 6>>& segs, hipStream_t s, long long* launches) {
+  std::atomic<long long> count{0};
+  QCopyList l(s, &count);
+  for (const auto& g : segs)
+    l.add2d((void*)(uintptr_t)g[0], (size_t)g[4], (const void*)(uintptr_t)g[1], (size_t)g[5], (size_t)g[2], (size_t)g[3]);
+  const hipError_t e = l.flush(s);
+  *launches = count.load();
+  return e;
+}
+
+hipError_t route_leg_offsets_compact(const int* rows, int max_path, const int* len, const int* status, int Q,
+                                     long long* off, int* flat, long long capacity, hipStream_t s) {
+  hipError_t e = launch_offsets(status, len, max_path, Q, off, s);
+  if (e == hipSuccess) e = launch_compact(rows, max_path, len, status, off, Q, flat, capacity, s);
+  return e;
+}
+
 std::vector<RouteJob*> RouteService::Impl::snap_jobs(Batch& b) {
   const double t0 = now_us();
   std::vector<RouteJob*> g;
@@ -73,35 +147,52 @@
   return g;
 }
 
-bool RouteService::Impl::compact_out(Batch& b, int Q, bool edges, const char* what) {
+bool RouteService::Impl::legs_out(Batch& b, hipError_t e, int Q, bool cch, double t0, const char* what) {
   const int MP = cfg.max_path;
-  long long total = 0;
-  for (int i = 0; i < Q; ++i) {
-    lb.h_off.h[i] = total;
-    if (lb.h_st.h[i] == 0) total += std::min(lb.h_len.h[i], MP);
-  }
-  if (total == 0) return true;
-  if (!lb.reserve_flat((size_t)total)) return false;
-  hipError_t e = qcopy(lb.d_off.d, lb.h_off.h, (size_t)Q * 8, stream);
-  if (e == hipSuccess) {
-    hipLaunchKernelGGL(compact_paths_kernel, dim3(Q), dim3(256), 0, stream, lb.d_path.d, MP, lb.d_len.d, lb.d_st.d,
-                       lb.d_off.d, Q, lb.d_flat.d);
-    e = hipGetLastError();
-  }
-  if (edges) {
-    if (e == hipSuccess && !lb.reserve_flat_e((size_t)total)) e = hipErrorOutOfMemory;
-    if (e == hipSuccess) {
-      hipLaunchKernelGGL(compact_paths_kernel, dim3(Q), dim3(256), 0, stream, lb.d_edge.d, MP, lb.d_len.d, lb.d_st.d,
-                         lb.d_off.d, Q, lb.d_flat_e.d);
-      e = hipGetLastError();
-    }
-  }
-  if (e == hipSuccess) e = qcopy(lb.h_flat.h, lb.d_flat.d, (size_t)total * 4, stream);
-  if (edges && e == hipSuccess) e = qcopy(lb.h_flat_e.h, lb.d_flat_e.d, (size_t)total * 4, stream);
+  const bool direct = qcopy_same_va().load(std::memory_order_relaxed);
+  auto cap = [&]() {
+    size_t c = std::min(lb.h_flat.n, direct ? lb.h_flat.n : lb.d_flat.n);
+    if (cch) c = std::min(c, std::min(lb.h_flat_e.n, direct ? lb.h_flat_e.n : lb.d_flat_e.n));
+    return (long long)c;
+  };
+  auto compact = [&](long long capacity) {
+    if (e == hipSuccess)
+      e = launch_compact(lb.d_path.d, MP, lb.d_len.d, lb.d_st.d, lb.d_off.d, Q, direct ? lb.h_flat.h : lb.d_flat.d, capacity,
+                         stream);
+    if (cch && e == hipSuccess)
+      e = launch_compact(lb.d_edge.d, MP, lb.d_len.d, lb.d_st.d, lb.d_off.d, Q, direct ? lb.h_flat_e.h : lb.d_flat_e.d,
+                         capacity, stream);
+  };
+  if (e == hipSuccess) e = launch_offsets(lb.d_st.d, lb.d_len.d, MP, Q, lb.d_off.d, stream);
+  const long long cap0 = cap();
+  compact(cap0);
+  QCopyList down = copies();
+  down.add(lb.h_st.h, lb.d_st.d, (size_t)Q * 4);
+  down.add(lb.h_len.h, lb.d_len.d, (size_t)Q * 4);
+  down.add(lb.h_cost.h, lb.d_cost.d, (size_t)Q * 4);
+  if (cch) down.add(lb.h_met.h, lb.d_met.d, (size_t)Q * 4);
+  down.add(lb.h_off.h, lb.d_off.d, ((size_t)Q + 1) * 8);
+  if (e == hipSuccess) e = down.flush(stream);
   if (e == hipSuccess) e = sync(stream, ev_gpu, what);
+  add_t(3, t0);
+  t0 = now_us();
+  if (e != hipSuccess) return false;
+  const long long total = lb.h_off.h[Q];
+  if (total > cap0) {
+    if (!lb.reserve_flat((size_t)total, !direct) || (cch && !lb.reserve_flat_e((size_t)total, !direct))) return false;
+    n_flat_regrows.fetch_add(1, std::memory_order_relaxed);
+    compact(cap());
+  }
+  if (!direct && total > 0) {
+    down.add(lb.h_flat.h, lb.d_flat.d, (size_t)total * 4);
+    if (cch) down.add(lb.h_flat_e.h, lb.d_flat_e.d, (size_t)total * 4);
+    if (e == hipSuccess) e = down.flush(stream);
+  }
+  if (e == hipSuccess && (total > cap0 || (!direct && total > 0))) e = sync(stream, ev_gpu, "paths-regrown");
   if (e != hipSuccess) return false;
   b.flat.assign(lb.h_flat.h, lb.h_flat.h + total);
-  if (edges) b.flat_e.assign(lb.h_flat_e.h, lb.h_flat_e.h + total);
+  if (cch) b.flat_e.assign(lb.h_flat_e.h, lb.h_flat_e.h + total);
+  add_t(4, t0);
   return true;
 }
 
@@ -205,14 +296,13 @@
       }
     }
   }
-  hipError_t e = qcopy(lb.d_src.d, lb.h_src.h, (size_t)Q * 4, stream);
-  if (e == hipSuccess) e = qcopy(lb.d_dst.d, lb.h_dst.h, (size_t)Q * 4, stream);
-  if (e == hipSuccess) e = qcopy(lb.d_lgrp.d, lb.h_lgrp.h, (size_t)Q * 4, stream);
-  if (QA > 0) {
-    if (e == hipSuccess) e = qcopy(lb.d_lr.d, lb.h_lr.h, (size_t)QA * 4, stream);
-    if (e == hipSuccess) e = qcopy(lb.d_li.d, lb.h_li.h, (size_t)QA * 4, stream);
-    if (e == hipSuccess) e = qcopy(lb.d_lj.d, lb.h_lj.h, (size_t)QA * 4, stream);
-  }
+  up.add(lb.d_src.d, lb.h_src.h, (size_t)Q * 4);
+  up.add(lb.d_dst.d, lb.h_dst.h, (size_t)Q * 4);
+  up.add(lb.d_lgrp.d, lb.h_lgrp.h, (size_t)Q * 4);
+  up.add(lb.d_lr.d, lb.h_lr.h, (size_t)QA * 4);
+  up.add(lb.d_li.d, lb.h_li.h, (size_t)QA * 4);
+  up.add(lb.d_lj.d, lb.h_lj.h, (size_t)QA * 4);
+  hipError_t e = up.flush(stream);
   auto out_at = [&](int q) {
     CchRouteOut o;
     o.sec = lb.d_cost.d + q;
@@ -230,16 +320,7 @@
   if (e == hipSuccess && QR > 0)
     e = cfg.cch->route_multi(cb.d_mv.d, lb.d_lgrp.d + QA, lb.d_src.d + QA, lb.d_dst.d + QA, QR, out_at(QA), csc, stream);
   n_legs_reused.fetch_add(QA, std::memory_order_relaxed);
-  if (e == hipSuccess) e = qcopy(lb.h_st.h, lb.d_st.d, (size_t)Q * 4, stream);
-  if (e == hipSuccess) e = qcopy(lb.h_len.h, lb.d_len.d, (size_t)Q * 4, stream);
-  if (e == hipSuccess) e = qcopy(lb.h_cost.h, lb.d_cost.d, (size_t)Q * 4, stream);
-  if (e == hipSuccess) e = qcopy(lb.h_met.h, lb.d_met.d, (size_t)Q * 4, stream);
-  if (e == hipSuccess) e = sync(stream, ev_gpu, "cch-legs");
-  add_t(3, t0);
-  t0 = now_us();
-  if (e != hipSuccess) return false;
-  if (!compact_out(b, Q, true, "cch-paths")) return false;
-  add_t(4, t0);
+  if (!legs_out(b, e, Q, true, t0, "cch-legs+paths")) return false;
   int nbad = 0;
   for (int i = 0; i < Q; ++i) nbad += lb.h_st.h[i] == 4;
   b.host_paths.resize(Q);
@@ -303,8 +384,10 @@
     lb.h_src.h[i] = pairs[i].first;
     lb.h_dst.h[i] = pairs[i].second;
   }
-  hipError_t e = qcopy(lb.d_src.d, lb.h_src.h, (size_t)Q * 4, stream);
-  if (e == hipSuccess) e = qcopy(lb.d_dst.d, lb.h_dst.h, (size_t)Q * 4, stream);
+  QCopyList in = copies();
+  in.add(lb.d_src.d, lb.h_src.h, (size_t)Q * 4);
+  in.add(lb.d_dst.d, lb.h_dst.h, (size_t)Q * 4);
+  hipError_t e = in.flush(stream);
   AstarGraphDev gd;
   gd.indptr = cfg.indptr;
   gd.indices = cfg.indices;
@@ -334,16 +417,7 @@
                      cfg.wave_ws.slots > 0 ? &cfg.wave_ws : nullptr, cfg.big_ws.slots > 0 ? &cfg.big_ws : nullptr,
                      ao, pl, lb.d_qidx.d, stream, &rs, cfg.arena.base ? &cfg.arena : nullptr);
   n_escalated.fetch_add(rs.escalated, std::memory_order_relaxed);
-  if (e == hipSuccess) e = qcopy(lb.h_st.h, lb.d_st.d, (size_t)Q * 4, stream);
-  if (e == hipSuccess) e = sync(stream, ev_gpu, "astar");
-  add_t(3, t0);
-  t0 = now_us();
-  if (e == hipSuccess) e = qcopy(lb.h_len.h, lb.d_len.d, (size_t)Q * 4, stream);
-  if (e == hipSuccess) e = qcopy(lb.h_cost.h, lb.d_cost.d, (size_t)Q * 4, stream);
-  if (e == hipSuccess) e = sync(stream, ev_gpu, "astar-escalate");
-  if (e != hipSuccess) return false;
-  if (!compact_out(b, Q, false, "astar-paths")) return false;
-  add_t(4, t0);
+  if (!legs_out(b, e, Q, false, t0, "astar+paths")) return false;
   int nbad = 0;
   for (int i = 0; i < Q; ++i) nbad += (lb.h_st.h[i] == 2 || lb.h_st.h[i] == 3);
   host_paths.resize(Q);
diff --git a/csrc/route_service_plan.hip b/csrc/route_service_plan.hip
--- a/csrc/route_service_plan.hip
+++ b/csrc/route_service_plan.hip
@@ -17,9 +17,10 @@
     }
   }
   auto v = std::make_shared<std::vector<float>>((size_t)cfg.cch->topo().E);
-  if (cb.h_hcost.need(v->size()) != hipSuccess || qcopy(cb.h_hcost.h, m->cost, v->size() * 4, stream) != hipSuccess ||
-      sync(stream, ev_gpu, "host-costs") != hipSuccess)
-    return nullptr;
+  QCopyList down = copies();
+  if (cb.h_hcost.need(v->size()) != hipSuccess) return nullptr;
+  down.add(cb.h_hcost.h, m->cost, v->size() * 4);
+  if (down.flush(stream) != hipSuccess || sync(stream, ev_gpu, "host-costs") != hipSuccess) return nullptr;
   std::memcpy(v->data(), cb.h_hcost.h, v->size() * 4);
   std::lock_guard<std::mutex> lk(hc_mu);
   if (hc_index.count(m->key)) return v;
@@ -34,6 +35,7 @@
 
 bool RouteService::Impl::cch_groups(Batch& b) {
   if (cfg.cch != nullptr) cfg.cch->note_queries();
+  up.reset(stream);
   const rtc::Stamp now = local_now(clock_skew_s);
   const int64_t days = (int64_t)std::floor((double)now.secs / 86400.0);
   const int64_t sec_of_day = now.secs - days * 86400;
@@ -144,7 +146,7 @@
   if (G > 0) {
     if (!cb.reserve(G)) return false;
     for (size_t g = 0; g < G; ++g) cb.h_mv.h[g] = CchGpu::view(*b.metrics[g]);
-    if (qcopy(cb.d_mv.d, cb.h_mv.h, G * sizeof(CchMView), stream) != hipSuccess) return false;
+    up.add(cb.d_mv.d, cb.h_mv.h, G * sizeof(CchMView));
   }
   return true;
 }
@@ -186,26 +188,22 @@
     tb.imp.h_xflag.h[k] = r.exchange ? 1 : 0;
   }
   const bool any_imp = std::any_of(m.begin(), m.end(), [](const RouteJob* j) { return j->req.improve || j->req.exchange; });
-  hipError_t e = hipSuccess;
-  cp(e, tb.d_lat.d, tb.h_lat.h, RN * 8);
-  cp(e, tb.d_lon.d, tb.h_lon.h, RN * 8);
-  cp(e, tb.d_dem.d, tb.h_dem.h, RN * 8);
-  cp(e, tb.d_npts.d, tb.h_npts.h, (size_t)R * 4);
-  cp(e, tb.d_cap.d, tb.h_cap.h, (size_t)R * 8);
-  cp(e, tb.d_maxd.d, tb.h_maxd.h, (size_t)R * 8);
+  up.reset(stream);
+  up.add(tb.d_lat.d, tb.h_lat.h, RN * 8);
+  up.add(tb.d_lon.d, tb.h_lon.h, RN * 8);
+  up.add(tb.d_dem.d, tb.h_dem.h, RN * 8);
+  up.add(tb.d_npts.d, tb.h_npts.h, (size_t)R * 4);
+  up.add(tb.d_cap.d, tb.h_cap.h, (size_t)R * 8);
+  up.add(tb.d_maxd.d, tb.h_maxd.h, (size_t)R * 8);
+  trips_up(any_imp, R);
+  hipError_t e = up.flush(stream);
+  QCopyList down = copies();
   if (e == hipSuccess) e = launch_haversine_matrix(tb.d_lat.d, tb.d_lon.d, tb.d_npts.d, R, NM, cfg.circuity, tb.d_D.d, stream);
   if (e == hipSuccess)
     e = launch_greedy_cvrp(tb.d_D.d, tb.d_npts.d, tb.d_dem.d, tb.d_cap.d, tb.d_maxd.d, R, NM, tb.d_visit.d, tb.d_trip.d, tb.d_ntrips.d,
                            tb.d_status.d, stream);
-  if (e == hipSuccess) e = improve_rows(any_imp, tb.d_npts.d, R, NM);
-  cp(e, tb.h_visit.h, tb.d_visit.d, RN * 4);
-  cp(e, tb.h_trip.h, tb.d_trip.d, RN * 4);
-  cp(e, tb.h_ntrips.h, tb.d_ntrips.d, (size_t)R * 4);
-  cp(e, tb.h_status.h, tb.d_status.d, (size_t)R * 4);
-  if (e == hipSuccess)
-    e = qcopy2d(tb.h_row0.h, (size_t)NM * 8, tb.d_D.d, (size_t)NM * NM * 8, (size_t)NM * 8, (size_t)R, stream);
-  if (e == hipSuccess) e = sync(stream, ev_gpu, "k5k6-matrix");
-  if (e != hipSuccess) return false;
+  if (e == hipSuccess) e = improve_rows(any_imp, tb.d_npts.d, R, NM, down);
+  if (trips_down(e, (size_t)R, (size_t)NM, down, "k5k6-matrix") != hipSuccess) return false;
   for (int k = 0; k < R; ++k) unpack_plan(m[k], tb.h_npts.h[k], NM, k, any_imp);
   return true;
 }
@@ -259,13 +257,15 @@
     }
   });
   const bool any_imp = std::any_of(m.begin(), m.end(), [](const RouteJob* j) { return j->req.improve || j->req.exchange; });
-  hipError_t e = hipSuccess;
-  cp(e, tb.d_pts.d, tb.h_pts.h, RN * 4);
-  cp(e, tb.d_npts2.d, tb.h_npts2.h, (size_t)R * 4);
-  cp(e, tb.d_dem.d, tb.h_dem.h, RN * 8);
-  cp(e, tb.d_cap.d, tb.h_cap.h, (size_t)R * 8);
-  cp(e, tb.d_maxd.d, tb.h_maxd.h, (size_t)R * 8);
-  cp(e, tb.d_rowg.d, tb.h_rowg.h, (size_t)R * 4);
+  up.add(tb.d_pts.d, tb.h_pts.h, RN * 4);
+  up.add(tb.d_npts2.d, tb.h_npts2.h, (size_t)R * 4);
+  up.add(tb.d_dem.d, tb.h_dem.h, RN * 8);
+  up.add(tb.d_cap.d, tb.h_cap.h, (size_t)R * 8);
+  up.add(tb.d_maxd.d, tb.h_maxd.h, (size_t)R * 8);
+  up.add(tb.d_rowg.d, tb.h_rowg.h, (size_t)R * 4);
+  trips_up(any_imp, R);
+  hipError_t e = up.flush(stream);
+  QCopyList down = copies();
   if (e == hipSuccess)
     e = cfg.cch->matrix_multi(cb.d_mv.d, tb.d_rowg.d, tb.d_pts.d, tb.d_npts2.d, R, NM, tb.d_msec.d, tb.d_mmet.d, tb.d_D.d, msc, stream);
   mtag = e == hipSuccess ? msc.chain_tag : 0;
@@ -273,32 +273,29 @@
   if (e == hipSuccess)
     e = launch_greedy_cvrp(tb.d_D.d, tb.d_npts2.d, tb.d_dem.d, tb.d_cap.d, tb.d_maxd.d, R, NM, tb.d_visit.d, tb.d_trip.d, tb.d_ntrips.d,
                            tb.d_status.d, stream);
-  if (e == hipSuccess) e = improve_rows(any_imp, tb.d_npts2.d, R, NM);
-  cp(e, tb.h_visit.h, tb.d_visit.d, RN * 4);
-  cp(e, tb.h_trip.h, tb.d_trip.d, RN * 4);
-  cp(e, tb.h_ntrips.h, tb.d_ntrips.d, (size_t)R * 4);
-  cp(e, tb.h_status.h, tb.d_status.d, (size_t)R * 4);
-  if (e == hipSuccess)
-    e = qcopy2d(tb.h_row0.h, (size_t)NM * 8, tb.d_D.d, (size_t)NM * NM * 8, (size_t)NM * 8, (size_t)R, stream);
-  if (e == hipSuccess) e = sync(stream, ev_gpu, "cch-matrix+greedy");
-  if (e != hipSuccess) return false;
+  if (e == hipSuccess) e = improve_rows(any_imp, tb.d_npts2.d, R, NM, down);
+  if (trips_down(e, (size_t)R, (size_t)NM, down, "cch-matrix+greedy") != hipSuccess) return false;
   for (int k = 0; k < R; ++k) unpack_plan(m[k], tb.h_npts2.h[k], NM, k, any_imp);
   return true;
 }
 
-hipError_t RouteService::Impl::improve_rows(bool any, const int* d_npts, int R, int NM) {
+void RouteService::Impl::trips_up(bool any, int R) {
+  if (!any) return;
+  up.add(tb.imp.d_flag.d, tb.imp.h_flag.h, (size_t)R);
+  if (std::any_of(tb.imp.h_xflag.h, tb.imp.h_xflag.h + R, [](unsigned char f) { return f != 0; }))
+    up.add(tb.imp.d_xflag.d, tb.imp.h_xflag.h, (size_t)R);
+}
+
+hipError_t RouteService::Impl::improve_rows(bool any, const int* d_npts, int R, int NM, QCopyList& down) {
   if (!any) return hipSuccess;
-  hipError_t e = hipSuccess;
-  cp(e, tb.imp.d_flag.d, tb.imp.h_flag.h, (size_t)R);
-  if (e == hipSuccess)
-    e = launch_improve_trips(tb.d_D.d, d_npts, tb.d_maxd.d, tb.imp.d_flag.d, tb.d_status.d, R, NM, tb.d_visit.d, tb.d_trip.d,
-                             tb.imp.d_moves.d, tb.imp.d_changed.d, tb.imp.d_before.d, tb.imp.d_after.d, stream);
-  cp(e, tb.imp.h_moves.h, tb.imp.d_moves.d, (size_t)R * 4);
-  cp(e, tb.imp.h_changed.h, tb.imp.d_changed.d, (size_t)R * 4);
-  cp(e, tb.imp.h_before.h, tb.imp.d_before.d, (size_t)R * 8);
-  cp(e, tb.imp.h_after.h, tb.imp.d_after.d, (size_t)R * 8);
+  hipError_t e = launch_improve_trips(tb.d_D.d, d_npts, tb.d_maxd.d, tb.imp.d_flag.d, tb.d_status.d, R, NM, tb.d_visit.d,
+                                      tb.d_trip.d, tb.imp.d_moves.d, tb.imp.d_changed.d, tb.imp.d_before.d,
+                                      tb.imp.d_after.d, stream);
+  down.add(tb.imp.h_moves.h, tb.imp.d_moves.d, (size_t)R * 4);
+  down.add(tb.imp.h_changed.h, tb.imp.d_changed.d, (size_t)R * 4);
+  down.add(tb.imp.h_before.h, tb.imp.d_before.d, (size_t)R * 8);
+  down.add(tb.imp.h_after.h, tb.imp.d_after.d, (size_t)R * 8);
   if (!std::any_of(tb.imp.h_xflag.h, tb.imp.h_xflag.h + R, [](unsigned char f) { return f != 0; })) return e;
-  cp(e, tb.imp.d_xflag.d, tb.imp.h_xflag.h, (size_t)R);
   if (e == hipSuccess)
     e = launch_exchange_trips(tb.d_D.d, d_npts, tb.d_dem.d, tb.d_cap.d, tb.d_maxd.d, tb.imp.d_xflag.d, tb.d_status.d, R, NM, -1,
                               tb.d_visit.d, tb.d_trip.d, tb.d_ntrips.d, tb.imp.d_xmoves.d, tb.imp.d_xrej.d, tb.imp.d_xtb.d,
@@ -306,12 +303,23 @@
   if (e == hipSuccess)
     e = launch_improve_trips(tb.d_D.d, d_npts, tb.d_maxd.d, tb.imp.d_xflag.d, tb.d_status.d, R, NM, tb.d_visit.d, tb.d_trip.d,
                              tb.imp.d_moves2.d, tb.imp.d_changed2.d, tb.imp.d_before2.d, tb.imp.d_after2.d, stream);
-  cp(e, tb.imp.h_xmoves.h, tb.imp.d_xmoves.d, (size_t)R * 4);
-  cp(e, tb.imp.h_xtb.h, tb.imp.d_xtb.d, (size_t)R * 4);
-  cp(e, tb.imp.h_xta.h, tb.imp.d_xta.d, (size_t)R * 4);
-  cp(e, tb.imp.h_moves2.h, tb.imp.d_moves2.d, (size_t)R * 4);
-  cp(e, tb.imp.h_after2.h, tb.imp.d_after2.d, (size_t)R * 8);
+  down.add(tb.imp.h_xmoves.h, tb.imp.d_xmoves.d, (size_t)R * 4);
+  down.add(tb.imp.h_xtb.h, tb.imp.d_xtb.d, (size_t)R * 4);
+  down.add(tb.imp.h_xta.h, tb.imp.d_xta.d, (size_t)R * 4);
+  down.add(tb.imp.h_moves2.h, tb.imp.d_moves2.d, (size_t)R * 4);
+  down.add(tb.imp.h_after2.h, tb.imp.d_after2.d, (size_t)R * 8);
   return e;
+}
+
+hipError_t RouteService::Impl::trips_down(hipError_t e, size_t R, size_t NM, QCopyList& down, const char* what) {
+  if (e != hipSuccess) return e;
+  down.add(tb.h_visit.h, tb.d_visit.d, R * NM * 4);
+  down.add(tb.h_trip.h, tb.d_trip.d, R * NM * 4);
+  down.add(tb.h_ntrips.h, tb.d_ntrips.d, R * 4);
+  down.add(tb.h_status.h, tb.d_status.d, R * 4);
+  down.add2d(tb.h_row0.h, NM * 8, tb.d_D.d, NM * NM * 8, NM * 8, R);
+  e = down.flush(stream);
+  return e == hipSuccess ? sync(stream, ev_gpu, what) : e;
 }
 
 void RouteService::Impl::unpack_plan(RouteJob* j, int n, int NM, int k, bool improved) {
diff --git a/routest_amd/serve/native_server.py b/routest_amd/serve/native_server.py
--- a/routest_amd/serve/native_server.py
+++ b/routest_amd/serve/native_server.py
@@ -126,7 +126,8 @@
                  "route_ctx_deferred", "route_us_ctx_wait", "route_ctx_prefetched",
                  "route_failed_over", "timeouts",
                  "route_records", "route_record_bytes",
-                 "route_us_collect", "route_us_handoff")
+                 "route_us_collect", "route_us_handoff",
+                 "route_copy_launches", "route_gpu_syncs", "route_flat_regrows")
         return dict(zip(names, v))
 
     def close(self) -> None:
```

Result: no change. 6.567 billion (-0.0%).
